# silencht/SG-SLAM

Hardware: AMD Instinct MI355X
Metric: tracked frames/sec (640x480 RGB-D) (higher is better)
Workload: dtype u8/f32(bf16x3 matrix products)/f64

## Files before the change

### include/sgx.h

```cpp
#ifndef SGX_H
#define SGX_H
#include <stdint.h>
#include <stddef.h>
#ifdef __cplusplus
extern "C" {
#endif

typedef enum sgx_status {
    SGX_OK = 0,
    SGX_ERR_INVALID = -1,
    SGX_ERR_UNSUPPORTED = -2,
    SGX_ERR_NOMEM = -3,
    SGX_ERR_DEVICE = -4,
    SGX_ERR_OVERFLOW = -5
} sgx_status;

const char *sgx_version(void);
const char *sgx_status_string(int status);

typedef struct sgx_keypoint {
    float x, y;
    float size;
    float angle;
    float response;
    int32_t octave;
    int32_t class_id;
} sgx_keypoint;

typedef struct sgx_orb_config {
    int32_t nfeatures;
    float scale_factor;
    int32_t nlevels;
    int32_t ini_th_fast;
    int32_t min_th_fast;
    int32_t width, height;
    int32_t max_batch;
} sgx_orb_config;

typedef struct sgx_orb sgx_orb;

int sgx_orb_create(const sgx_orb_config *cfg, sgx_orb **out);
void sgx_orb_destroy(sgx_orb *h);
int sgx_orb_keypoint_capacity(const sgx_orb *h);
int sgx_orb_get_tables(const sgx_orb *h, float *scale, float *inv_scale, float *sigma2, float *inv_sigma2,
                       int32_t *features_per_level);
int sgx_orb_extract_batch_dev(sgx_orb *h, const uint8_t *d_gray, int pitch, int batch,
                              sgx_keypoint *d_kps, uint8_t *d_desc, int32_t *d_count, int cap, void *stream);
int sgx_orb_extract(sgx_orb *h, const uint8_t *gray, int stride, sgx_keypoint *kps, uint8_t *desc, int cap, int *n);
int sgx_orb_last_status(sgx_orb *h, void *stream);

typedef struct sgx_camera {
    float fx, fy, cx, cy, bf;
    float min_x, max_x, min_y, max_y;
} sgx_camera;

int sgx_match_project_frame_batch_dev(
    int batch, int cap,
    const sgx_keypoint *d_ckeys, const uint8_t *d_cdesc, const float *d_curight, const int32_t *d_cn, const float *d_cTcw,
    const sgx_keypoint *d_lkeys, const int32_t *d_ln, const uint8_t *d_l_has_mp, const uint8_t *d_l_outlier, const float *d_l_xw,
    const int32_t *d_l_obs, const uint8_t *d_l_mpdesc, const float *d_lTcw,
    const sgx_camera *cam, const float *scale_factors, int nlevels, float th, int b_mono, int check_orientation,
    int32_t *d_cur_match, int32_t *d_nmatches, void *stream);
int sgx_match_project_frame(
    int nc, const sgx_keypoint *ckeys, const uint8_t *cdesc, const float *curight, const float *cTcw,
    int nl, const sgx_keypoint *lkeys, const uint8_t *l_has_mp, const uint8_t *l_outlier, const float *l_xw,
    const int32_t *l_obs, const uint8_t *l_mpdesc, const float *lTcw,
    const sgx_camera *cam, const float *scale_factors, int nlevels, float th, int b_mono, int check_orientation,
    int32_t *cur_match, int32_t *nmatches);

int sgx_match_project_local_batch_dev(
    int batch, int cap, const sgx_keypoint *d_ckeys, const uint8_t *d_cdesc, const float *d_curight, const int32_t *d_cn, const float *d_cTcw, const int32_t *d_cur_mp_obs,
    int mcap, const int32_t *d_mn, const float *d_m_xw, const float *d_m_normal, const float *d_m_min_dist, const float *d_m_max_dist, const uint8_t *d_m_desc,
    const int32_t *d_m_obs, const uint8_t *d_m_skip,
    const sgx_camera *cam, const float *scale_factors, int nlevels, float log_scale_factor, float th, float nnratio, float viewing_cos_limit,
    int32_t *d_cur_match, int32_t *d_nmatches, uint8_t *d_in_view, void *stream);

int sgx_match_project_local(
    int nc, const sgx_keypoint *ckeys, const uint8_t *cdesc, const float *curight, const float *cTcw, const int32_t *cur_mp_obs,
    int nm, const float *m_xw, const float *m_normal, const float *m_min_dist, const float *m_max_dist, const uint8_t *m_desc, const int32_t *m_obs, const uint8_t *m_skip,
    const sgx_camera *cam, const float *scale_factors, int nlevels, float log_scale_factor, float th, float nnratio, float viewing_cos_limit,
    int32_t *cur_match, int32_t *nmatches, uint8_t *in_view);

int sgx_hamming_matrix(const uint8_t *desc_a, int na, const uint8_t *desc_b, int nb, uint16_t *out);
int sgx_hamming_matrix_dev(const uint8_t *d_desc_a, int na, const uint8_t *d_desc_b, int nb, uint16_t *d_out, void *stream);
int sgx_match_search_for_triangulation(
    int n1, const sgx_keypoint *keys1_un, const uint8_t *desc1, const float *uright1, const uint8_t *has_mp1, const int32_t *feat_node1, const float *cam_center1,
    int n2, const sgx_keypoint *keys2_un, const uint8_t *desc2, const float *uright2, const uint8_t *has_mp2, const int32_t *feat_node2, const float *Tcw2,
    const float *F12, const sgx_camera *cam2, const float *scale_factors2, const float *level_sigma2_2, int nlevels, int only_stereo, int check_orientation,
    int32_t *pairs, int32_t *npairs);
int sgx_match_search_by_bow(
    int nk, const sgx_keypoint *keys_kf_un, const uint8_t *desc_kf, const uint8_t *kf_good_mp, const int32_t *feat_node_kf,
    int nf, const sgx_keypoint *keys_f_un, const uint8_t *desc_f, const int32_t *feat_node_f, float nnratio, int check_orientation,
    int32_t *match_f, int32_t *nmatches);
int sgx_match_search_by_bow_kf(
    int n1, const sgx_keypoint *keys1_un, const uint8_t *desc1, const uint8_t *good1, const int32_t *feat_node1,
    int n2, const sgx_keypoint *keys2_un, const uint8_t *desc2, const uint8_t *good2, const int32_t *feat_node2, float nnratio, int check_orientation,
    int32_t *match12, int32_t *nmatches);
int sgx_match_fuse_search(
    int nk, const sgx_keypoint *keys_un, const uint8_t *desc, const float *uright, const float *Tcw,
    int nm, const float *m_xw, const float *m_normal, const float *m_min_dist, const float *m_max_dist, const uint8_t *m_desc, const uint8_t *m_skip,
    const sgx_camera *cam, const float *scale_factors, const float *inv_level_sigma2, int nlevels, float log_scale_factor, float th,
    int32_t *best_idx, int32_t *best_dist, int32_t *nfused);

int sgx_match_project_keyframe(
    int nc, const sgx_keypoint *ckeys_un, const uint8_t *cdesc, const uint8_t *c_has_mp, const float *cTcw,
    int nk, const sgx_keypoint *kf_keys_un, const uint8_t *kf_ok, const float *m_xw, const float *m_min_dist, const float *m_max_dist, const uint8_t *m_desc,
    const sgx_camera *cam, const float *scale_factors, int nlevels, float log_scale_factor, float th, int orb_dist, int check_orientation,
    int32_t *cur_match, int32_t *nmatches);

int sgx_match_fuse_search_sim3(
    int nk, const sgx_keypoint *keys_un, const uint8_t *desc, const float *Scw,
    int nm, const float *m_xw, const float *m_normal, const float *m_min_dist, const float *m_max_dist, const uint8_t *m_desc, const uint8_t *m_skip,
    const sgx_camera *cam, const float *scale_factors, int nlevels, float log_scale_factor, float th,
    int32_t *best_idx, int32_t *best_dist, int32_t *nfused);
int sgx_match_project_sim3(
    int nk, const sgx_keypoint *keys_un, const uint8_t *desc, const uint8_t *matched_in, const float *Scw,
    int nm, const float *m_xw, const float *m_normal, const float *m_min_dist, const float *m_max_dist, const uint8_t *m_desc, const uint8_t *m_skip,
    const sgx_camera *cam, const float *scale_factors, int nlevels, float log_scale_factor, int th,
    int32_t *matched_out, int32_t *nmatches);
int sgx_match_search_by_sim3(
    int n1, const sgx_keypoint *keys1_un, const uint8_t *desc1, const float *Tcw1, const uint8_t *mp_ok1, const float *m_xw1, const float *m_min_dist1, const float *m_max_dist1, const uint8_t *m_desc1,
    int n2, const sgx_keypoint *keys2_un, const uint8_t *desc2, const float *Tcw2, const uint8_t *mp_ok2, const float *m_xw2, const float *m_min_dist2, const float *m_max_dist2, const uint8_t *m_desc2,
    const sgx_camera *cam, const float *scale_factors, int nlevels, float log_scale_factor, float s12, const float *R12, const float *t12, float th,
    int32_t *match12, int32_t *nfound);

int sgx_match_search_for_initialization(
    int n1, const sgx_keypoint *keys1_un, const uint8_t *desc1, int n2, const sgx_keypoint *keys2_un, const uint8_t *desc2,
    float *prev_matched, int window_size, float nnratio, int check_orientation, const sgx_camera *cam, int32_t *matches12, int32_t *nmatches);

int sgx_triangulate_new_map_points(
// ... 84 lines not shown
int sgx_voc_transform(sgx_voc *v, int n, const uint8_t *desc, int levelsup, int32_t *bow_ids, double *bow_weights, int32_t *nbow, int32_t *feat_node, int32_t *feat_word);
int sgx_voc_transform_batch_dev(sgx_voc *v, const uint8_t *d_desc, size_t desc_pitch, const int32_t *d_n, int batch, int cap, int levelsup,
                                int32_t *d_word_id, double *d_weight, int32_t *d_feat_node, void *stream);
int sgx_voc_score(const sgx_voc *v, int n1, const int32_t *ids1, const double *w1, int n2, const int32_t *ids2, const double *w2, double *score);

int sgx_frame_gray_from_color_batch_dev(int batch, int width, int height, const uint8_t *d_src, int src_pitch, int channels, int blue_first,
                                        uint8_t *d_gray, int gray_pitch, void *stream);
int sgx_frame_stereo_from_rgbd_batch_dev(int batch, int cap, const sgx_keypoint *d_keys, const int32_t *d_n,
                                         const uint16_t *d_depth, int width, int height, float depth_map_factor,
                                         float bf, float *d_uright, float *d_zdepth, void *stream);
int sgx_undistort_points(int n, const float *pts, const float *K4, const float *dist, int ndist, float *out);
int sgx_frame_undistort_stereo_rgbd_batch_dev(int batch, int cap, const sgx_keypoint *d_keys, const int32_t *d_n, const float *dist, int ndist,
                                              const sgx_camera *cam, const uint16_t *d_depth, int width, int height, float depth_map_factor,
                                              sgx_keypoint *d_keys_un, float *d_uright, float *d_zdepth, void *stream);
int sgx_frame_image_bounds(int width, int height, const float *K4, const float *dist, int ndist, sgx_camera *cam);

int sgx_frame_unproject_batch_dev(int batch, int cap, const sgx_keypoint *d_keys, const int32_t *d_n, const float *d_zdepth,
                                  const float *d_Tcw, const sgx_camera *cam, float *d_xw, uint8_t *d_has, void *stream);

int sgx_frame_motion_model_batch_dev(int batch, const float *d_Tcw_cur, const float *d_Tcw_prev, const uint8_t *d_valid,
                                     float *d_Tcw_pred, void *stream);

int sgx_frame_make_map_points_batch_dev(int batch, int cap, int half, const sgx_keypoint *d_keys, const int32_t *d_n, const float *d_xw, const uint8_t *d_has,
                                        const uint8_t *d_desc, const float *d_Tcw, const float *scale_factors, int nlevels,
                                        float *d_m_xw, float *d_m_normal, float *d_m_min_dist, float *d_m_max_dist, uint8_t *d_m_desc, uint8_t *d_m_skip, void *stream);
int sgx_frame_merge_matches_batch_dev(int batch, int cap, const int32_t *d_n, const int32_t *d_match_last, const uint8_t *d_outlier_last, const int32_t *d_match_local,
                                      const float *d_xw_last, const float *d_m_xw, int32_t *d_merged, int32_t *d_cur_mp_obs, float *d_xw_all, void *stream);

int sgx_pose_optimization_batch_dev(int batch, int cap, const sgx_keypoint *d_keys_un, const float *d_uright, const int32_t *d_n,
                                    const int32_t *d_mp_index, const uint8_t *d_has_mp, const float *d_mp_xw, int xw_pitch,
                                    const float *inv_level_sigma2, int nlevels, const sgx_camera *cam,
                                    float *d_Tcw, uint8_t *d_outlier, int32_t *d_n_inliers, void *stream);
int sgx_pose_optimization(int n, const sgx_keypoint *keys_un, const float *uright, const uint8_t *has_mp, const float *mp_xw,
                          const float *inv_level_sigma2, int nlevels, const sgx_camera *cam,
                          float *Tcw, uint8_t *outlier, int32_t *n_inliers);

typedef struct sgx_ba_problem {
    int32_t n_poses, n_points, n_edges;
    float *poses;
    const uint8_t *pose_fixed;
    float *points;
    const int32_t *edge_pose;
    const int32_t *edge_point;
    const float *edge_obs;
    const float *edge_info;
} sgx_ba_problem;
typedef struct sgx_ba_stats { int32_t iterations_first, iterations_second, free_poses, reserved; double chi2_first, chi2_second; } sgx_ba_stats;
int sgx_local_bundle_adjustment(const sgx_ba_problem *problem, const sgx_camera *cam, const volatile int32_t *stop_flag,
                                uint8_t *edge_erase, sgx_ba_stats *stats);
int sgx_bundle_adjustment(const sgx_ba_problem *problem, const sgx_camera *cam, int n_iterations, const volatile int32_t *stop_flag, int robust, sgx_ba_stats *stats);

int sgx_optimize_sim3(int n, const float *p1c, const float *p2c, const float *obs1, const float *obs2, const float *info1, const float *info2,
                      const float *K1, const float *K2, double *S12, float th2, int fix_scale, uint8_t *inlier, int32_t *iterations, int32_t *n_inliers);

int sgx_optimize_essential_graph(int nv, const double *S_in, const uint8_t *fixed, int ne, const int32_t *e_i, const int32_t *e_j, const double *e_meas,
                                 int fix_scale, int iterations, double *S_out, double *stats);
int sgx_correct_map_points(int n, const float *xw, const int32_t *ref, int nv, const double *Srw, const double *corrected_Swr, float *xw_out);

#define SGX_DET_MAX 100
typedef struct sgx_detection { float label, score, xmin, ymin, xmax, ymax; } sgx_detection;
typedef struct sgx_object2d { int32_t id; float prob, x, y, w, h; } sgx_object2d;
typedef struct sgx_det_result {
    int32_t n_raw; sgx_detection raw[SGX_DET_MAX];
    int32_t n_objects; sgx_object2d objects[SGX_DET_MAX];
    int32_t have_dynamic_for_mapping, have_dynamic_for_rm_feature;
    int32_t n_map_boxes; sgx_object2d map_boxes[SGX_DET_MAX];
    int32_t n_rm_boxes; sgx_object2d rm_boxes[SGX_DET_MAX];
} sgx_det_result;
typedef struct sgx_det sgx_det;
int sgx_det_create(const char *param_text, const void *bin, size_t bin_bytes, int width, int height, int max_batch,
                   float detection_confidence_threshold, float dynamic_detection_confidence_threshold, sgx_det **out);
void sgx_det_destroy(sgx_det *h);
int sgx_det_info(const sgx_det *h, int32_t *num_priors, int32_t *num_class, int32_t *num_kernels, double *gmac);
int sgx_det_detect(sgx_det *h, const uint8_t *images, int pitch, int batch, sgx_det_result *results);
int sgx_det_detect_batch_dev(sgx_det *h, const uint8_t *d_img, int pitch, int batch, sgx_det_result *d_results,
                             float *d_boxes, int32_t *d_nboxes, int max_boxes, int32_t *d_have_dynamic, void *stream);
int sgx_det_forward_batch_dev(sgx_det *h, const uint8_t *d_img, int pitch, int batch, const float **d_loc, const float **d_conf, void *stream);
int sgx_det_gemm_mode(const sgx_det *h);
int sgx_det_plan_step(const sgx_det *h, int i, char *buf, int cap);
int sgx_dynamic_mask_batch_dev(int batch, int cap, const sgx_keypoint *d_keys, const int32_t *d_n, const float *d_prev_xy, const double *d_F,
                               const float *d_boxes, const int32_t *d_nboxes, int max_boxes, uint8_t *d_keep, void *stream);
int sgx_frame_compact_keys_batch_dev(int batch, int cap, const sgx_keypoint *d_keys, const uint8_t *d_desc, const int32_t *d_n, const uint8_t *d_keep,
                                     const int32_t *d_have_dynamic, int nfeatures, sgx_keypoint *d_keys_out, uint8_t *d_desc_out, int32_t *d_n_out, void *stream);


typedef struct sgx_flow_config {
    int32_t width, height, max_batch;
    int32_t win_size;
    int32_t max_level;
    int32_t max_count;
    double epsilon;
} sgx_flow_config;
typedef struct sgx_flow sgx_flow;
int sgx_flow_create(const sgx_flow_config *cfg, sgx_flow **out);
void sgx_flow_destroy(sgx_flow *h);
int sgx_flow_reset(sgx_flow *h);
int sgx_flow_levels(const sgx_flow *h);
int sgx_flow_lk_batch_dev(sgx_flow *h, const uint8_t *d_gray, int pitch, int batch, const sgx_keypoint *d_keys, const int32_t *d_n, int cap,
                          float *d_prev_xy, uint8_t *d_status, int32_t *have_prev, void *stream);
int sgx_flow_lk(sgx_flow *h, const uint8_t *gray_from, const uint8_t *gray_to, int stride, const float *pts, int n, float *next_pts, uint8_t *status);
int sgx_fundamental_ransac_batch_dev(int batch, int cap, const sgx_keypoint *d_keys, const int32_t *d_n, const float *d_prev_xy,
                                     const int32_t *d_pre_have_dynamic, const float *d_pre_boxes, const int32_t *d_pre_nboxes, int max_boxes,
                                     double threshold, double confidence, double *d_F, int32_t *d_ok, int32_t *d_stats, void *stream);
int sgx_find_fundamental_mat(const float *pts1, const float *pts2, int n, double threshold, double confidence, double *F, int32_t *ok, int32_t *stats);

typedef struct sgx_tracker_config {
    int32_t streams, width, height;
    int32_t nfeatures; float scale_factor; int32_t nlevels, ini_th_fast, min_th_fast;
    sgx_camera cam; float depth_map_factor;
    float th_projection;
    int32_t local_map;
    int32_t dynamic_mask;
    int32_t max_boxes;
    int32_t pipelined;
} sgx_tracker_config;
typedef struct sgx_tracker sgx_tracker;
int sgx_tracker_create(const sgx_tracker_config *cfg, sgx_det *detector , sgx_tracker **out);
void sgx_tracker_destroy(sgx_tracker *t);
int sgx_tracker_keypoint_capacity(const sgx_tracker *t);
int sgx_tracker_record_bytes(const sgx_tracker *t);
int sgx_tracker_set_initial_pose(sgx_tracker *t, const float *Tcw );
int sgx_tracker_set_distortion(sgx_tracker *t, const float *dist, int ndist, sgx_camera *out_cam);
int sgx_tracker_step_dev(sgx_tracker *t, const uint8_t *d_gray, int gray_pitch, const uint16_t *d_depth, const uint8_t *d_bgr, int bgr_pitch, void *caller_stream);
int sgx_tracker_host_buffers(sgx_tracker *t, int slot, uint8_t **bgr, int *bgr_pitch, uint16_t **depth);
int sgx_tracker_step_host(sgx_tracker *t, int slot, int rgb_order);
int sgx_tracker_wait_inputs(sgx_tracker *t, int steps_back);
int sgx_tracker_sync(sgx_tracker *t);
int sgx_tracker_read(sgx_tracker *t, float *Tcw, int32_t *nkeys, int32_t *nmatches, int32_t *ninliers, int32_t *nmatches_local, int32_t *ninliers2, int32_t *nkeys_raw,
                     int32_t *f_ok, int32_t *f_stats);
int sgx_tracker_snapshot_pose_dev(sgx_tracker *t, float *d_out );
int sgx_tracker_snapshot_boxes_dev(sgx_tracker *t, int stream_index, float *d_boxes , int32_t *d_nboxes);
int sgx_tracker_pack_records_dev(sgx_tracker *t, uint8_t *d_records, void *stream);
typedef struct sgx_dist sgx_dist;
int sgx_dist_unique_id(void *id128 );
int sgx_dist_create(const void *id128, int world, int rank, sgx_dist **out);
void sgx_dist_destroy(sgx_dist *d);
int sgx_dist_world(const sgx_dist *d, int32_t *world, int32_t *rank);
int sgx_dist_gather_records(sgx_dist *d, const void *d_send, size_t bytes_per_rank, void *d_recv, int root, void *stream);
int sgx_tracker_frame_dev(sgx_tracker *t, const int32_t **d_n, const sgx_keypoint **d_keys, const uint8_t **d_desc, const float **d_Tcw, const float **d_xw, const uint8_t **d_has);
int sgx_tracker_frame_keys_un_dev(sgx_tracker *t, const sgx_keypoint **d_keys_un);
sgx_orb *sgx_tracker_extractor(sgx_tracker *t);

int sgx_profile_enable(int on);
int sgx_profile_num_classes(void);
const char *sgx_profile_class_name(int k);
int sgx_profile_read(float *ms, int32_t *launches, int reset);

#ifdef __cplusplus
}
#endif
#endif
```

### include/sgx_debug.h

```cpp
#ifndef SGX_DEBUG_H
#define SGX_DEBUG_H
#include "sgx.h"
#ifdef __cplusplus
extern "C" {
#endif

int sgx_orb_debug_level_geometry(const sgx_orb *h, int level, int32_t *w, int32_t *hgt, int32_t *stride);
int sgx_orb_debug_set_unfused_pyramid(int on);
int sgx_orb_debug_read_level(sgx_orb *h, int frame, int level, uint8_t *dst );
int sgx_orb_debug_read_candidates(sgx_orb *h, int frame, int level, int32_t *x, int32_t *y, int32_t *score, int cap, int *n);
int sgx_debug_flow_affine_batch_dev(int batch, int cap, const sgx_keypoint *d_keys, const int32_t *d_n, const float *d_A, const float *d_shift, const float *d_boxes,
                                    int max_boxes, float *d_prev_xy, void *stream);
int sgx_pose_opt_debug_set_threads(int threads_per_frame);
int sgx_ba_debug_last_plan(int32_t plan[4]);
int sgx_ba_debug_set_init(int mode);
int sgx_ba_debug_set_jobs(int host);
int sgx_ba_debug_set_solver(int mode);
int sgx_det_debug_read_blob(sgx_det *h, const char *blob_name, int image, float *dst, int cap, int *n);
int sgx_flow_debug_read_level(sgx_flow *h, int slot, int frame, int level, uint8_t *img);
int sgx_flow_debug_read_slot(sgx_flow *h, int slot, int frame, int level, uint8_t *img, int32_t *pitch);
int sgx_flow_debug_level_size(const sgx_flow *h, int level, int32_t *w, int32_t *hgt);
int sgx_pnp_debug_betas(int which, const double *L, const double *rho, double *betas);
int sgx_obj3d_debug_read(sgx_obj3d *h, int job, uint8_t *kept, int32_t *labels, int cap, int *n);
int sgx_debug_corun_bf16(int blocks, int iters, int launches, void *stream);
int sgx_det_debug_detection_output(sgx_det *h, const float *loc, const float *conf, int batch, sgx_det_result *results);
int sgx_det_debug_continued(sgx_det *h, int *count);
int sgx_det_debug_set_fusion(int on);
int sgx_det_debug_set_irb(int on);
int sgx_det_debug_set_block_fusion(int on);
int sgx_det_debug_set_gemm(int mode);
int sgx_det_debug_set_legacy_kernels(int on);
int sgx_det_debug_time_ops(sgx_det *h, const uint8_t *d_img, int pitch, int batch, int reps, float *ms, int cap, int *nops);
int sgx_det_debug_run_step(sgx_det *h, const uint8_t *d_img, int pitch, int batch, int step, int reps, void *stream);
int sgx_orb_debug_run_octree(sgx_orb *h, int level, const uint32_t *packed, int n, uint32_t *out_sel, int cap, int *nsel);

#ifdef __cplusplus
}
#endif
#endif
```

### sg_slam_amd/capi.py

```python
import ctypes as C
import numpy as np

KP_DTYPE = np.dtype([('x', 'f4'), ('y', 'f4'), ('size', 'f4'), ('angle', 'f4'), ('response', 'f4'),
                     ('octave', 'i4'), ('class_id', 'i4')])


class SgxError(RuntimeError):
    pass


class Camera(C.Structure):
    _fields_ = [('fx', C.c_float), ('fy', C.c_float), ('cx', C.c_float), ('cy', C.c_float), ('bf', C.c_float),
                ('min_x', C.c_float), ('max_x', C.c_float), ('min_y', C.c_float), ('max_y', C.c_float)]


class BaProblem(C.Structure):
    _fields_ = [('n_poses', C.c_int32), ('n_points', C.c_int32), ('n_edges', C.c_int32), ('poses', C.c_void_p), ('pose_fixed', C.c_void_p),
                ('points', C.c_void_p), ('edge_pose', C.c_void_p), ('edge_point', C.c_void_p), ('edge_obs', C.c_void_p), ('edge_info', C.c_void_p)]


class BaStats(C.Structure):
    _fields_ = [('iterations_first', C.c_int32), ('iterations_second', C.c_int32), ('free_poses', C.c_int32), ('reserved', C.c_int32),
                ('chi2_first', C.c_double), ('chi2_second', C.c_double)]

# ... 2 lines not shown


class Detection(C.Structure):
    _fields_ = [(k, C.c_float) for k in ('label', 'score', 'xmin', 'ymin', 'xmax', 'ymax')]


class Object2D(C.Structure):
    _fields_ = [('id', C.c_int32)] + [(k, C.c_float) for k in ('prob', 'x', 'y', 'w', 'h')]


class DetResult(C.Structure):
    _fields_ = [('n_raw', C.c_int32), ('raw', Detection * SGX_DET_MAX), ('n_objects', C.c_int32), ('objects', Object2D * SGX_DET_MAX),
                ('have_dynamic_for_mapping', C.c_int32), ('have_dynamic_for_rm_feature', C.c_int32),
                ('n_map_boxes', C.c_int32), ('map_boxes', Object2D * SGX_DET_MAX), ('n_rm_boxes', C.c_int32), ('rm_boxes', Object2D * SGX_DET_MAX)]


class FlowConfig(C.Structure):
    _fields_ = [('width', C.c_int32), ('height', C.c_int32), ('max_batch', C.c_int32), ('win_size', C.c_int32), ('max_level', C.c_int32),
                ('max_count', C.c_int32), ('epsilon', C.c_double)]


class TrackerConfig(C.Structure):
    _fields_ = [('streams', C.c_int32), ('width', C.c_int32), ('height', C.c_int32), ('nfeatures', C.c_int32), ('scale_factor', C.c_float), ('nlevels', C.c_int32),
                ('ini_th_fast', C.c_int32), ('min_th_fast', C.c_int32), ('cam', Camera), ('depth_map_factor', C.c_float), ('th_projection', C.c_float),
                ('local_map', C.c_int32), ('dynamic_mask', C.c_int32), ('max_boxes', C.c_int32), ('pipelined', C.c_int32)]


class Obj3dParams(C.Structure):
    _fields_ = [('sor_stddev_mul', C.c_double), ('sor_mean_k', C.c_int32), ('cluster_min_size', C.c_int32), ('cluster_max_size', C.c_int32),
                ('voxel_leaf_size', C.c_float), ('cluster_tolerance', C.c_float), ('similar_compare_ratio', C.c_float),
                ('camera_valid_depth_min', C.c_float), ('camera_valid_depth_max', C.c_float)]


class Obj3dJob(C.Structure):
    _fields_ = [('image', C.c_int32), ('class_id', C.c_int32)] + [(k, C.c_float) for k in ('prob', 'x', 'y', 'w', 'h')]


OBJ3D_RESULT_DTYPE = np.dtype([('found', 'i4'), ('class_id', 'i4'), ('prob', 'f4'), ('centroid', 'f4', 3), ('size', 'f4', 3), ('crop_points', 'i4'), ('kept_points', 'i4'),
                               ('components', 'i4'), ('clusters', 'i4'), ('best_cluster_size', 'i4'), ('larger_window_points', 'i4'), ('best_similar1', 'f4'),
                               ('best_similar2', 'f4'), ('best_roi', 'f4', 4)])


class SemanticObjectRecord(C.Structure):
    _fields_ = [('class_id', C.c_int32), ('object_id', C.c_int32), ('prob', C.c_float), ('centroid', C.c_float * 3), ('size', C.c_float * 3)]


class InitReport(C.Structure):
    _fields_ = [('SH', C.c_float), ('SF', C.c_float), ('RH', C.c_float), ('model', C.c_int32), ('n_matches', C.c_int32), ('n_inliers_h', C.c_int32),
                ('n_inliers_f', C.c_int32), ('n_hyp', C.c_int32), ('best_hyp', C.c_int32), ('n_good', C.c_int32 * 8), ('cos_parallax', C.c_float * 8),
                ('parallax', C.c_float * 8), ('H21', C.c_float * 9), ('F21', C.c_float * 9)]


class OrbConfig(C.Structure):
    _fields_ = [('nfeatures', C.c_int32), ('scale_factor', C.c_float), ('nlevels', C.c_int32),
                ('ini_th_fast', C.c_int32), ('min_th_fast', C.c_int32), ('width', C.c_int32),
                ('height', C.c_int32), ('max_batch', C.c_int32)]


SYMBOLS = [
    'sgx_version', 'sgx_status_string', 'sgx_orb_create', 'sgx_orb_destroy', 'sgx_orb_keypoint_capacity', 'sgx_orb_get_tables',
    'sgx_orb_extract_batch_dev', 'sgx_orb_extract', 'sgx_orb_last_status', 'sgx_profile_enable', 'sgx_profile_num_classes', 'sgx_profile_class_name',
    'sgx_profile_read', 'sgx_match_project_frame_batch_dev', 'sgx_match_project_frame', 'sgx_match_project_local_batch_dev',
    'sgx_match_project_local', 'sgx_frame_stereo_from_rgbd_batch_dev', 'sgx_frame_unproject_batch_dev', 'sgx_frame_make_map_points_batch_dev',
    'sgx_frame_merge_matches_batch_dev', 'sgx_pose_optimization_batch_dev', 'sgx_pose_optimization', 'sgx_frame_motion_model_batch_dev',
    'sgx_local_bundle_adjustment', 'sgx_bundle_adjustment', 'sgx_det_create', 'sgx_det_destroy', 'sgx_det_info', 'sgx_det_detect',
    'sgx_det_detect_batch_dev', 'sgx_det_forward_batch_dev', 'sgx_frame_compact_keys_batch_dev', 'sgx_frame_gray_from_color_batch_dev',
    'sgx_det_gemm_mode', 'sgx_det_plan_step', 'sgx_dynamic_mask_batch_dev', 'sgx_tracker_create', 'sgx_tracker_destroy',
    'sgx_tracker_keypoint_capacity', 'sgx_tracker_record_bytes', 'sgx_tracker_set_initial_pose', 'sgx_tracker_step_dev', 'sgx_tracker_host_buffers',
    'sgx_tracker_step_host', 'sgx_tracker_wait_inputs', 'sgx_tracker_sync', 'sgx_tracker_read', 'sgx_tracker_snapshot_pose_dev',
    'sgx_tracker_snapshot_boxes_dev', 'sgx_tracker_pack_records_dev', 'sgx_tracker_frame_dev', 'sgx_tracker_extractor', 'sgx_flow_create',
    'sgx_dist_unique_id', 'sgx_dist_create', 'sgx_dist_destroy', 'sgx_dist_world', 'sgx_dist_gather_records',
    'sgx_flow_destroy', 'sgx_flow_reset', 'sgx_flow_levels', 'sgx_flow_lk_batch_dev', 'sgx_flow_lk', 'sgx_fundamental_ransac_batch_dev',
    'sgx_find_fundamental_mat', 'sgx_hamming_matrix', 'sgx_hamming_matrix_dev', 'sgx_match_search_for_triangulation', 'sgx_match_search_by_bow',
    'sgx_match_search_by_bow_kf', 'sgx_match_fuse_search', 'sgx_match_project_keyframe', 'sgx_match_fuse_search_sim3',
    'sgx_triangulate_new_map_points', 'sgx_mappoint_update_normal_and_depth', 'sgx_mappoint_distinctive_descriptors', 'sgx_sim3_solver_create',
    'sgx_sim3_solver_set_ransac_parameters', 'sgx_sim3_solver_iterate', 'sgx_sim3_solver_get_estimate', 'sgx_sim3_solver_destroy',
    'sgx_match_search_for_initialization', 'sgx_voc_load', 'sgx_voc_create', 'sgx_voc_info', 'sgx_voc_destroy', 'sgx_voc_transform',
    'sgx_voc_transform_batch_dev', 'sgx_voc_score', 'sgx_match_project_sim3', 'sgx_match_search_by_sim3', 'sgx_optimize_sim3',
    'sgx_optimize_essential_graph', 'sgx_correct_map_points', 'sgx_undistort_points', 'sgx_frame_undistort_stereo_rgbd_batch_dev', 'sgx_frame_image_bounds',
    'sgx_tracker_set_distortion', 'sgx_tracker_frame_keys_un_dev', 'sgx_pnp_solver_create', 'sgx_pnp_solver_set_ransac_parameters', 'sgx_pnp_solver_iterate',
    'sgx_pnp_solver_get_estimate', 'sgx_pnp_solver_destroy', 'sgx_pnp_batch_create', 'sgx_pnp_batch_set_dev', 'sgx_pnp_batch_iterate_dev', 'sgx_pnp_batch_destroy',
    'sgx_obj3d_create', 'sgx_obj3d_destroy', 'sgx_obj3d_detect_batch_dev', 'sgx_obj3d_detect', 'sgx_objdb_create', 'sgx_objdb_destroy', 'sgx_objdb_add', 'sgx_objdb_size',
    'sgx_objdb_get', 'sgx_initializer_create', 'sgx_initializer_initialize', 'sgx_initializer_destroy', 'sgx_init_batch_create', 'sgx_init_batch_run_dev',
    'sgx_init_batch_destroy',
]
TAP_SYMBOLS = [
    'sgx_orb_debug_level_geometry', 'sgx_orb_debug_set_unfused_pyramid', 'sgx_orb_debug_read_level', 'sgx_orb_debug_read_candidates',
    'sgx_orb_debug_run_octree', 'sgx_pose_opt_debug_set_threads', 'sgx_ba_debug_set_solver', 'sgx_ba_debug_set_jobs', 'sgx_ba_debug_set_init', 'sgx_ba_debug_last_plan', 'sgx_det_debug_read_blob',
    'sgx_det_debug_detection_output', 'sgx_det_debug_continued', 'sgx_debug_flow_affine_batch_dev', 'sgx_det_debug_set_fusion', 'sgx_det_debug_set_legacy_kernels',
    'sgx_det_debug_set_block_fusion', 'sgx_det_debug_set_irb', 'sgx_det_debug_set_gemm', 'sgx_det_debug_time_ops', 'sgx_det_debug_run_step', 'sgx_flow_debug_read_level',
    'sgx_flow_debug_level_size', 'sgx_flow_debug_read_slot', 'sgx_debug_corun_bf16', 'sgx_pnp_debug_betas', 'sgx_obj3d_debug_read',
]


def _vp(x):
    if x is None:
        return None
    if isinstance(x, int):
        return C.c_void_p(x)
    if hasattr(x, 'data_ptr'):
        return C.c_void_p(x.data_ptr())
    return x.ctypes.data_as(C.c_void_p)


class SgxLib:
    def __init__(self, path):
        self.path = path
        self.dll = C.CDLL(path)
        d = self.dll
        d.sgx_version.restype = C.c_char_p
        d.sgx_status_string.restype = C.c_char_p
        d.sgx_status_string.argtypes = [C.c_int]
        d.sgx_orb_create.argtypes = [C.POINTER(OrbConfig), C.POINTER(C.c_void_p)]
        d.sgx_orb_destroy.argtypes = [C.c_void_p]
        d.sgx_orb_destroy.restype = None
        d.sgx_orb_keypoint_capacity.argtypes = [C.c_void_p]
        d.sgx_orb_get_tables.argtypes = [C.c_void_p] + [C.c_void_p] * 5
        d.sgx_orb_extract_batch_dev.argtypes = [C.c_void_p, C.c_void_p, C.c_int, C.c_int, C.c_void_p, C.c_void_p,
                                                C.c_void_p, C.c_int, C.c_void_p]
        d.sgx_orb_extract.argtypes = [C.c_void_p, C.c_void_p, C.c_int, C.c_void_p, C.c_void_p, C.c_int, C.POINTER(C.c_int)]
        d.sgx_orb_last_status.argtypes = [C.c_void_p, C.c_void_p]

        d.sgx_profile_enable.argtypes = [C.c_int]
        d.sgx_profile_class_name.restype = C.c_char_p
        d.sgx_profile_class_name.argtypes = [C.c_int]
        d.sgx_profile_read.argtypes = [C.c_void_p, C.c_void_p, C.c_int]

        vp = C.c_void_p
        d.sgx_match_project_frame_batch_dev.argtypes = [C.c_int, C.c_int] + [vp] * 13 + [C.POINTER(Camera), vp, C.c_int, C.c_float, C.c_int, C.c_int, vp, vp, vp]
        d.sgx_match_project_frame.argtypes = [C.c_int] + [vp] * 4 + [C.c_int] + [vp] * 7 + [C.POINTER(Camera), vp, C.c_int, C.c_float, C.c_int, C.c_int, vp, vp]
        d.sgx_frame_stereo_from_rgbd_batch_dev.argtypes = [C.c_int, C.c_int, vp, vp, vp, C.c_int, C.c_int, C.c_float, C.c_float, vp, vp, vp]
        d.sgx_frame_unproject_batch_dev.argtypes = [C.c_int, C.c_int, vp, vp, vp, vp, C.POINTER(Camera), vp, vp, vp]
        d.sgx_pose_optimization_batch_dev.argtypes = [C.c_int, C.c_int, vp, vp, vp, vp, vp, vp, C.c_int, vp, C.c_int, C.POINTER(Camera), vp, vp, vp, vp]
        d.sgx_pose_optimization.argtypes = [C.c_int, vp, vp, vp, vp, vp, C.c_int, C.POINTER(Camera), vp, vp, vp]
        d.sgx_frame_motion_model_batch_dev.argtypes = [C.c_int, vp, vp, vp, vp, vp]
        d.sgx_local_bundle_adjustment.argtypes = [C.POINTER(BaProblem), C.POINTER(Camera), vp, vp, C.POINTER(BaStats)]
        d.sgx_bundle_adjustment.argtypes = [C.POINTER(BaProblem), C.POINTER(Camera), C.c_int, vp, C.c_int, C.POINTER(BaStats)]
        d.sgx_det_create.argtypes = [C.c_char_p, vp, C.c_size_t, C.c_int, C.c_int, C.c_int, C.c_float, C.c_float, C.POINTER(vp)]
        d.sgx_det_destroy.argtypes = [vp]; d.sgx_det_destroy.restype = None
        d.sgx_det_info.argtypes = [vp, C.POINTER(C.c_int32), C.POINTER(C.c_int32), C.POINTER(C.c_int32), C.POINTER(C.c_double)]
        d.sgx_det_detect.argtypes = [vp, vp, C.c_int, C.c_int, C.POINTER(DetResult)]
        d.sgx_det_detect_batch_dev.argtypes = [vp, vp, C.c_int, C.c_int, vp, vp, vp, C.c_int, vp, vp]
        d.sgx_det_forward_batch_dev.argtypes = [vp, vp, C.c_int, C.c_int, C.POINTER(vp), C.POINTER(vp), vp]
        d.sgx_det_gemm_mode.argtypes = [vp]
        d.sgx_tracker_create.argtypes = [C.POINTER(TrackerConfig), vp, C.POINTER(vp)]
        d.sgx_tracker_destroy.argtypes = [vp]; d.sgx_tracker_destroy.restype = None
        d.sgx_tracker_keypoint_capacity.argtypes = [vp]
        d.sgx_tracker_record_bytes.argtypes = [vp]
        d.sgx_tracker_set_initial_pose.argtypes = [vp, vp]
        d.sgx_tracker_step_dev.argtypes = [vp, vp, C.c_int, vp, vp, C.c_int, vp]
        d.sgx_tracker_host_buffers.argtypes = [vp, C.c_int, C.POINTER(vp), C.POINTER(C.c_int), C.POINTER(vp)]
        d.sgx_tracker_step_host.argtypes = [vp, C.c_int, C.c_int]
        d.sgx_tracker_sync.argtypes = [vp]
        d.sgx_tracker_wait_inputs.argtypes = [vp, C.c_int]
        d.sgx_tracker_read.argtypes = [vp] * 10
        d.sgx_tracker_snapshot_pose_dev.argtypes = [vp, vp]
        d.sgx_tracker_snapshot_boxes_dev.argtypes = [vp, C.c_int, vp, vp]
        d.sgx_tracker_pack_records_dev.argtypes = [vp, vp, vp]
        d.sgx_dist_unique_id.argtypes = [vp]
        d.sgx_dist_create.argtypes = [vp, C.c_int, C.c_int, C.POINTER(vp)]
        d.sgx_dist_destroy.argtypes = [vp]; d.sgx_dist_destroy.restype = None
        d.sgx_dist_world.argtypes = [vp, C.POINTER(C.c_int32), C.POINTER(C.c_int32)]
        d.sgx_dist_gather_records.argtypes = [vp, vp, C.c_size_t, vp, C.c_int, vp]
        d.sgx_tracker_frame_dev.argtypes = [vp] + [C.POINTER(vp)] * 6
        d.sgx_tracker_extractor.argtypes = [vp]; d.sgx_tracker_extractor.restype = vp
        d.sgx_det_plan_step.argtypes = [vp, C.c_int, C.c_char_p, C.c_int]
        d.sgx_dynamic_mask_batch_dev.argtypes = [C.c_int, C.c_int, vp, vp, vp, vp, vp, vp, C.c_int, vp, vp]
        d.sgx_frame_gray_from_color_batch_dev.argtypes = [C.c_int, C.c_int, C.c_int, vp, C.c_int, C.c_int, C.c_int, vp, C.c_int, vp]
        d.sgx_frame_compact_keys_batch_dev.argtypes = [C.c_int, C.c_int, vp, vp, vp, vp, vp, C.c_int, vp, vp, vp, vp]
        d.sgx_match_project_local.argtypes = [C.c_int] + [vp] * 5 + [C.c_int] + [vp] * 7 + [C.POINTER(Camera), vp, C.c_int, C.c_float, C.c_float, C.c_float, C.c_float, vp, vp, vp]
        d.sgx_match_project_local_batch_dev.argtypes = [C.c_int, C.c_int] + [vp] * 6 + [C.c_int] + [vp] * 8 + [C.POINTER(Camera), vp, C.c_int, C.c_float, C.c_float, C.c_float, C.c_float, vp, vp, vp, vp]
        d.sgx_undistort_points.argtypes = [C.c_int, vp, vp, vp, C.c_int, vp]
        d.sgx_frame_undistort_stereo_rgbd_batch_dev.argtypes = [C.c_int, C.c_int, vp, vp, vp, C.c_int, C.POINTER(Camera), vp, C.c_int, C.c_int, C.c_float, vp, vp, vp, vp]
        d.sgx_frame_image_bounds.argtypes = [C.c_int, C.c_int, vp, vp, C.c_int, C.POINTER(Camera)]
        d.sgx_tracker_set_distortion.argtypes = [vp, vp, C.c_int, C.POINTER(Camera)]
        d.sgx_tracker_frame_keys_un_dev.argtypes = [vp, C.POINTER(vp)]
        d.sgx_frame_make_map_points_batch_dev.argtypes = [C.c_int, C.c_int, C.c_int] + [vp] * 7 + [C.c_int] + [vp] * 7
        d.sgx_frame_merge_matches_batch_dev.argtypes = [C.c_int, C.c_int] + [vp] * 10
        d.sgx_flow_create.argtypes = [C.POINTER(FlowConfig), C.POINTER(vp)]
        d.sgx_flow_destroy.argtypes = [vp]; d.sgx_flow_destroy.restype = None
        d.sgx_flow_reset.argtypes = [vp]
        d.sgx_flow_levels.argtypes = [vp]
        d.sgx_flow_lk_batch_dev.argtypes = [vp, vp, C.c_int, C.c_int, vp, vp, C.c_int, vp, vp, C.POINTER(C.c_int32), vp]
        d.sgx_flow_lk.argtypes = [vp, vp, vp, C.c_int, vp, C.c_int, vp, vp]
        d.sgx_fundamental_ransac_batch_dev.argtypes = [C.c_int, C.c_int] + [vp] * 6 + [C.c_int, C.c_double, C.c_double, vp, vp, vp, vp]
        d.sgx_find_fundamental_mat.argtypes = [vp, vp, C.c_int, C.c_double, C.c_double, vp, vp, vp]
        d.sgx_hamming_matrix.argtypes = [vp, C.c_int, vp, C.c_int, vp]
        d.sgx_optimize_essential_graph.argtypes = [C.c_int, vp, vp, C.c_int, vp, vp, vp, C.c_int, C.c_int, vp, vp]
        d.sgx_correct_map_points.argtypes = [C.c_int, vp, vp, C.c_int, vp, vp, vp]
        d.sgx_optimize_sim3.argtypes = [C.c_int] + [vp] * 9 + [C.c_float, C.c_int, vp, vp, vp]
        d.sgx_match_project_keyframe.argtypes = [C.c_int] + [vp] * 4 + [C.c_int] + [vp] * 6 + [C.POINTER(Camera), vp, C.c_int, C.c_float, C.c_float, C.c_int, C.c_int, vp, vp]
        d.sgx_match_search_by_bow.argtypes = [C.c_int] + [vp] * 4 + [C.c_int] + [vp] * 3 + [C.c_float, C.c_int, vp, vp]
        d.sgx_match_fuse_search_sim3.argtypes = [C.c_int, vp, vp, vp, C.c_int] + [vp] * 6 + [vp, vp, C.c_int, C.c_float, C.c_float, vp, vp, vp]
        d.sgx_match_project_sim3.argtypes = [C.c_int, vp, vp, vp, vp, C.c_int] + [vp] * 6 + [vp, vp, C.c_int, C.c_float, C.c_int, vp, vp]
        d.sgx_match_search_by_sim3.argtypes = ([C.c_int] + [vp] * 8) * 2 + [vp, vp, C.c_int, C.c_float, C.c_float, vp, vp, C.c_float, vp, vp]
        d.sgx_match_search_for_initialization.argtypes = [C.c_int, vp, vp, C.c_int, vp, vp, vp, C.c_int, C.c_float, C.c_int, vp, vp, vp]
        d.sgx_sim3_solver_create.argtypes = [C.c_int] + [vp] * 6 + [C.c_int, C.c_uint, vp]
        d.sgx_sim3_solver_set_ransac_parameters.argtypes = [vp, C.c_double, C.c_int, C.c_int]
        d.sgx_sim3_solver_iterate.argtypes = [vp, C.c_int] + [vp] * 7
        d.sgx_sim3_solver_get_estimate.argtypes = [vp] * 5
        d.sgx_sim3_solver_destroy.argtypes = [vp]; d.sgx_sim3_solver_destroy.restype = None
        d.sgx_pnp_solver_create.argtypes = [C.c_int] + [vp] * 4 + [C.c_uint, vp]
        d.sgx_pnp_solver_set_ransac_parameters.argtypes = [vp, C.c_double, C.c_int, C.c_int, C.c_int, C.c_float, C.c_float]
        d.sgx_pnp_solver_iterate.argtypes = [vp, C.c_int] + [vp] * 7
        d.sgx_pnp_solver_get_estimate.argtypes = [vp] * 6
        d.sgx_pnp_solver_destroy.argtypes = [vp]; d.sgx_pnp_solver_destroy.restype = None
        d.sgx_pnp_batch_create.argtypes = [C.c_int, C.c_int, vp]
        d.sgx_pnp_batch_set_dev.argtypes = [vp, C.c_int] + [vp] * 8
        d.sgx_pnp_batch_iterate_dev.argtypes = [vp, C.c_int, vp, C.c_int, vp, vp, vp, vp]
        d.sgx_pnp_batch_destroy.argtypes = [vp]; d.sgx_pnp_batch_destroy.restype = None
        d.sgx_initializer_create.argtypes = [C.c_int, vp, vp, C.c_float, C.c_int, C.c_uint, vp]
        d.sgx_initializer_initialize.argtypes = [vp, C.c_int] + [vp] * 10
        d.sgx_initializer_destroy.argtypes = [vp]; d.sgx_initializer_destroy.restype = None
        d.sgx_init_batch_create.argtypes = [C.c_int] * 4 + [vp]
        d.sgx_init_batch_run_dev.argtypes = [vp, C.c_int] + [vp] * 9 + [C.c_int] + [vp] * 8
        d.sgx_init_batch_destroy.argtypes = [vp]; d.sgx_init_batch_destroy.restype = None
        d.sgx_obj3d_create.argtypes = [C.c_int] * 5 + [C.POINTER(Obj3dParams), C.POINTER(vp)]
        d.sgx_obj3d_destroy.argtypes = [vp]; d.sgx_obj3d_destroy.restype = None
        d.sgx_obj3d_detect_batch_dev.argtypes = [vp, vp, C.c_int, C.c_int, vp, vp, vp, C.c_int, vp, vp]
        d.sgx_obj3d_detect.argtypes = [vp, vp, vp, vp, C.POINTER(Obj3dJob), vp]
        d.sgx_objdb_create.argtypes = [C.POINTER(vp)]
        d.sgx_objdb_destroy.argtypes = [vp]; d.sgx_objdb_destroy.restype = None
        d.sgx_objdb_add.argtypes = [vp, C.POINTER(SemanticObjectRecord), C.POINTER(C.c_int32), C.POINTER(C.c_int32)]
        d.sgx_objdb_size.argtypes = [vp]
        d.sgx_objdb_get.argtypes = [vp, C.c_int, C.POINTER(SemanticObjectRecord)]
        d.sgx_mappoint_update_normal_and_depth.argtypes = [C.c_int] + [vp] * 6 + [C.c_int, vp, vp, vp]
        d.sgx_mappoint_distinctive_descriptors.argtypes = [C.c_int, vp, vp, vp, vp]
        d.sgx_triangulate_new_map_points.argtypes = [C.c_int, vp] + [C.c_int] + [vp] * 5 + [C.c_int] + [vp] * 5 + [vp, vp, vp, C.c_int, vp, vp, vp]
        d.sgx_voc_load.argtypes = [C.c_char_p, vp]
        d.sgx_voc_create.argtypes = [C.c_int] * 5 + [vp] * 5
        d.sgx_voc_info.argtypes = [vp] * 7
        d.sgx_voc_destroy.argtypes = [vp]; d.sgx_voc_destroy.restype = None
        d.sgx_voc_transform.argtypes = [vp, C.c_int, vp, C.c_int, vp, vp, vp, vp, vp]
        d.sgx_voc_transform_batch_dev.argtypes = [vp, vp, C.c_size_t, vp, C.c_int, C.c_int, C.c_int, vp, vp, vp, vp]
        d.sgx_voc_score.argtypes = [vp, C.c_int, vp, vp, C.c_int, vp, vp, vp]
        d.sgx_match_search_by_bow_kf.argtypes = [C.c_int] + [vp] * 4 + [C.c_int] + [vp] * 4 + [C.c_float, C.c_int, vp, vp]
        d.sgx_match_fuse_search.argtypes = [C.c_int] + [vp] * 4 + [C.c_int] + [vp] * 6 + [C.POINTER(Camera), vp, vp, C.c_int, C.c_float, C.c_float, vp, vp, vp]
        d.sgx_hamming_matrix_dev.argtypes = [vp, C.c_int, vp, C.c_int, vp, vp]
        d.sgx_match_search_for_triangulation.argtypes = [C.c_int] + [vp] * 6 + [C.c_int] + [vp] * 6 + [vp, C.POINTER(Camera), vp, vp, C.c_int, C.c_int, C.c_int, vp, vp]

        self.has_taps = hasattr(d, 'sgx_det_debug_read_blob')
        if self.has_taps:
            d.sgx_orb_debug_level_geometry.argtypes = [C.c_void_p, C.c_int] + [C.POINTER(C.c_int32)] * 3
            d.sgx_orb_debug_read_level.argtypes = [C.c_void_p, C.c_int, C.c_int, C.c_void_p]
            d.sgx_orb_debug_read_candidates.argtypes = [C.c_void_p, C.c_int, C.c_int, C.c_void_p, C.c_void_p, C.c_void_p, C.c_int, C.POINTER(C.c_int)]
            d.sgx_orb_debug_run_octree.argtypes = [C.c_void_p, C.c_int, C.c_void_p, C.c_int, C.c_void_p, C.c_int, C.POINTER(C.c_int)]
            d.sgx_orb_debug_set_unfused_pyramid.argtypes = [C.c_int]
            d.sgx_pose_opt_debug_set_threads.argtypes = [C.c_int]
            d.sgx_ba_debug_set_solver.argtypes = [C.c_int]
            d.sgx_ba_debug_set_jobs.argtypes = [C.c_int]
            d.sgx_ba_debug_set_init.argtypes = [C.c_int]
            d.sgx_ba_debug_last_plan.argtypes = [C.c_void_p]
            d.sgx_det_debug_detection_output.argtypes = [vp, vp, vp, C.c_int, C.POINTER(DetResult)]
            d.sgx_det_debug_continued.argtypes = [vp, C.POINTER(C.c_int)]
            d.sgx_det_debug_read_blob.argtypes = [vp, C.c_char_p, C.c_int, vp, C.c_int, C.POINTER(C.c_int)]
            for nm in ('fusion', 'legacy_kernels', 'block_fusion', 'irb', 'gemm'):
                getattr(d, 'sgx_det_debug_set_' + nm).argtypes = [C.c_int]
            d.sgx_det_debug_time_ops.argtypes = [vp, vp, C.c_int, C.c_int, C.c_int, vp, C.c_int, C.POINTER(C.c_int)]
            d.sgx_det_debug_run_step.argtypes = [vp, vp, C.c_int, C.c_int, C.c_int, C.c_int, vp]
            d.sgx_debug_flow_affine_batch_dev.argtypes = [C.c_int, C.c_int, vp, vp, vp, vp, vp, C.c_int, vp, vp]
            d.sgx_flow_debug_read_level.argtypes = [vp, C.c_int, C.c_int, C.c_int, vp]
            d.sgx_debug_corun_bf16.argtypes = [C.c_int, C.c_int, C.c_int, vp]
            d.sgx_pnp_debug_betas.argtypes = [C.c_int, vp, vp, vp]
            d.sgx_obj3d_debug_read.argtypes = [vp, C.c_int, vp, vp, C.c_int, C.POINTER(C.c_int)]
            d.sgx_flow_debug_level_size.argtypes = [vp, C.c_int, C.POINTER(C.c_int32), C.POINTER(C.c_int32)]
            d.sgx_flow_debug_read_slot.argtypes = [vp, C.c_int, C.c_int, C.c_int, vp, C.POINTER(C.c_int32)]

    def tap(self, name):
        if not self.has_taps:
            raise SgxError(f'{name}: {self.path} is the product build and has no test taps; use tests/taps/libsgx_taps.so (make -C sg_slam_amd/csrc taps)')
        return getattr(self.dll, name)

    def version(self):
        return self.dll.sgx_version().decode()

    def check(self, rc, what=''):
        if rc != 0:
            raise SgxError(f'{what}: {self.dll.sgx_status_string(rc).decode()} ({rc})')

    def profile_enable(self, on=True):
        self.check(self.dll.sgx_profile_enable(int(on)))

    def profile_read(self, reset=True):
        n = self.dll.sgx_profile_num_classes()
        ms = np.zeros(n, 'f4'); cnt = np.zeros(n, 'i4')
        self.check(self.dll.sgx_profile_read(_vp(ms), _vp(cnt), int(reset)), 'sgx_profile_read')
        return {self.dll.sgx_profile_class_name(k).decode(): (float(ms[k]), int(cnt[k])) for k in range(n)}
```

### sg_slam_amd/csrc/sgx_det.cpp

```cpp
#include "sgx_block.h"
#include "sgx_det_block.h"
#include "sgx_det_irb.h"
#include "sgx_det_bf16.h"
#include "sgx_det_hrb.h"
#include "sgx_prof.h"
#include "../../include/sgx.h"
#ifdef SGX_DEBUG_TAPS
#include "../../include/sgx_debug.h"
#endif
#include <math.h>
#include <stdio.h>
#include <stdlib.h>
#include <string.h>
#include <algorithm>
#include <map>
#include <memory>
#include <sstream>
#include <string>
#include <vector>


namespace {
struct Layer {
    std::string type, name;
// ... 1206 lines not shown
                                        float *d_boxes, int32_t *d_nboxes, int max_boxes, int32_t *d_have_dynamic, void *stream_)
{
    if (!h || !d_results || ((d_boxes != nullptr) != (d_nboxes != nullptr)) || (d_boxes && max_boxes < 1)) return SGX_ERR_INVALID;
    const float *dl = nullptr, *dc = nullptr;
    int rc = sgx_det_forward_batch_dev(h, d_img, pitch, batch, &dl, &dc, stream_);
    if (rc != SGX_OK) return rc;
    return run_detection_output(h, batch, d_results, d_boxes, d_nboxes, max_boxes, d_have_dynamic, (sgx_stream_t)stream_);
}

static int run_detection_output(sgx_det *h, int batch, sgx_det_result *d_results, float *d_boxes, int32_t *d_nboxes, int max_boxes, int32_t *d_have_dynamic, sgx_stream_t st)
{
    SgxDetOut P; P.n = h->num_priors; P.nc = h->num_class; P.nms_top_k = h->nms_top_k; P.keep_top_k = h->keep_top_k; P.nms_th = h->nms_th; P.conf_th = h->conf_th;
    P.var0 = h->dvar[0]; P.var1 = h->dvar[1]; P.var2 = h->dvar[2]; P.var3 = h->dvar[3];
    if (h->sw.skip_output) return SGX_OK;
    sgx_prof_begin(SGX_K_DET_OUT, st);
    const dim3 grid(h->num_class - 1, batch);
    const size_t lds_full = (size_t)std::max(h->num_priors, 7 * SGX_DO_TOPK) * 4 + 16, lds_first = (size_t)std::max(h->num_priors, 7 * (SGX_DO_FIRST + 1)) * 4 + 16;
    const float *loc = h->blobs[h->loc_blob].d, *conf = h->blobs[h->conf_blob].d;
    const int *no_cont = nullptr; const uint32_t *no_sstar = nullptr; int *no_ncut = nullptr; uint32_t *no_next = nullptr;
    if (h->sw.out_single) {
        SGX_LAUNCH_DYN(k_det_class_nms<0>, grid, dim3(256), lds_full, st, P, loc, conf, h->d_priors, h->d_cls_rows, h->d_cls_count, no_ncut, no_next, no_cont, no_sstar);
    } else {
        SGX_LAUNCH_DYN(k_det_class_nms<SGX_DO_FIRST>, grid, dim3(256), lds_first, st, P, loc, conf, h->d_priors, h->d_cls_rows, h->d_cls_count, h->d_cls_ncut, h->d_cls_next, no_cont, no_sstar);
        SGX_LAUNCH(k_det_cut, dim3(batch), dim3(256), st, P, h->d_cls_rows, h->d_cls_count, h->d_cls_ncut, h->d_cls_next, h->d_sstar, h->d_cls_cont);
        SGX_LAUNCH_DYN(k_det_class_nms<0>, grid, dim3(256), lds_full, st, P, loc, conf, h->d_priors, h->d_cls_rows, h->d_cls_count, no_ncut, no_next, h->d_cls_cont, h->d_sstar);
    }
    h->last_out_batch = h->sw.out_single ? 0 : batch;
    SGX_LAUNCH(k_det_merge, dim3(batch), dim3(256), st, P, h->d_cls_rows, h->d_cls_count, h->det_th, h->dyn_th, h->W, h->H, h->T, d_results, d_boxes, d_nboxes, max_boxes, d_have_dynamic);
    sgx_prof_end(SGX_K_DET_OUT, st);
    SGX_CHECK_HIP(hipGetLastError());
    return SGX_OK;
}

SGX_TAP int sgx_det_debug_detection_output(sgx_det *h, const float *loc, const float *conf, int batch, sgx_det_result *results)
{
    if (!h || !loc || !conf || !results || batch < 1 || batch > h->max_batch) return SGX_ERR_INVALID;
    SGX_CHECK_HIP(hipMemcpy(h->blobs[h->loc_blob].d, loc, sizeof(float) * 4 * (size_t)h->num_priors * batch, hipMemcpyHostToDevice));
    SGX_CHECK_HIP(hipMemcpy(h->blobs[h->conf_blob].d, conf, sizeof(float) * (size_t)h->num_priors * h->num_class * batch, hipMemcpyHostToDevice));
    int rc = run_detection_output(h, batch, h->d_results, nullptr, nullptr, 0, nullptr, (sgx_stream_t)0);
    if (rc != SGX_OK) return rc;
    SGX_CHECK_HIP(hipMemcpy(results, h->d_results, sizeof(sgx_det_result) * batch, hipMemcpyDeviceToHost));
    return SGX_OK;
}

SGX_TAP int sgx_det_debug_continued(sgx_det *h, int *count)
{
    if (!h || !count) return SGX_ERR_INVALID;
    std::vector<int> cont((size_t)h->last_out_batch * (h->num_class - 1));
    if (!cont.empty()) SGX_CHECK_HIP(hipMemcpy(cont.data(), h->d_cls_cont, cont.size() * sizeof(int), hipMemcpyDeviceToHost));
    *count = 0; for (int v : cont) *count += v;
    return SGX_OK;
}

extern "C" int sgx_det_detect(sgx_det *h, const uint8_t *images, int pitch, int batch, sgx_det_result *results)
{
    if (!h || !images || !results || batch < 1 || batch > h->max_batch || pitch < 3 * h->W) return SGX_ERR_INVALID;
    const int ipitch = (3 * h->W + 3) & ~3;
    for (int b = 0; b < batch; b++)
        for (int y = 0; y < h->H; y++)
            SGX_CHECK_HIP(hipMemcpyAsync(h->d_img + ((size_t)b * h->H + y) * ipitch, images + ((size_t)b * h->H + y) * pitch, (size_t)3 * h->W, hipMemcpyHostToDevice, 0));
    int rc = sgx_det_detect_batch_dev(h, h->d_img, ipitch, batch, h->d_results, nullptr, nullptr, 0, nullptr, nullptr);
    if (rc != SGX_OK) return rc;
    SGX_CHECK_HIP(hipMemcpy(results, h->d_results, sizeof(sgx_det_result) * batch, hipMemcpyDeviceToHost));
    return SGX_OK;
}

extern "C" int sgx_dynamic_mask_batch_dev(int batch, int cap, const sgx_keypoint *d_keys, const int32_t *d_n, const float *d_prev_xy, const double *d_F,
                                          const float *d_boxes, const int32_t *d_nboxes, int max_boxes, uint8_t *d_keep, void *stream)
{
    if (batch < 1 || cap < 1 || !d_keys || !d_n || !d_prev_xy || !d_F || !d_boxes || !d_nboxes || !d_keep || max_boxes < 0) return SGX_ERR_INVALID;
    sgx_prof_begin(SGX_K_MASK, (sgx_stream_t)stream);
    SGX_LAUNCH(k_dynamic_mask, dim3((cap + 255) / 256, batch), dim3(256), (sgx_stream_t)stream, cap, (const uint8_t *)d_keys, d_n, d_prev_xy, d_F, d_boxes, d_nboxes, max_boxes, d_keep);
    sgx_prof_end(SGX_K_MASK, (sgx_stream_t)stream);
    SGX_CHECK_HIP(hipGetLastError());
    return SGX_OK;
}

extern "C" int sgx_frame_compact_keys_batch_dev(int batch, int cap, const sgx_keypoint *d_keys, const uint8_t *d_desc, const int32_t *d_n, const uint8_t *d_keep,
                                                const int32_t *d_have_dynamic, int nfeatures, sgx_keypoint *d_keys_out, uint8_t *d_desc_out, int32_t *d_n_out, void *stream)
{
    if (batch < 1 || cap < 1 || !d_keys || !d_desc || !d_n || !d_keep || !d_keys_out || !d_desc_out || !d_n_out || (const void *)d_keys == (const void *)d_keys_out) return SGX_ERR_INVALID;
    sgx_prof_begin(SGX_K_MASK, (sgx_stream_t)stream);
    SGX_LAUNCH(k_compact_keys, dim3(batch), dim3(256), (sgx_stream_t)stream, cap, (const uint8_t *)d_keys, d_desc, d_n, d_keep, d_have_dynamic, (float)nfeatures * 0.1f,
               (uint8_t *)d_keys_out, d_desc_out, d_n_out);
    sgx_prof_end(SGX_K_MASK, (sgx_stream_t)stream);
    SGX_CHECK_HIP(hipGetLastError());
    return SGX_OK;
}
```

### sg_slam_amd/csrc/sgx_det_kernels.h

```cpp
#pragma once
#include "sgx_rt.h"
#include "../../include/sgx.h"
#ifdef SGX_DEBUG_TAPS
#include "../../include/sgx_debug.h"
#endif

#ifndef SGX_EMU
__device__ int sgx_det_xcd_order = 1;
#else
static int sgx_det_xcd_order = 1;
#endif
SGX_DEV void sgx_xcd_order(int id, int per_frame, int batch, int *frame, int *item)
{
    const int b8 = batch & ~7;
    if (sgx_det_xcd_order && id < b8 * per_frame) {
        const int x = id & 7, i = id >> 3, q = i / per_frame;
        *item = i - q * per_frame; *frame = q * 8 + x;
    } else { const int f = id / per_frame; *frame = f; *item = id - f * per_frame; }
}

#define SGX_ACT_NONE 0
#define SGX_ACT_RELU 1
#define SGX_ACT_CLIP 2

// ... 800 lines not shown
    SGX_THREADS_END
}

SGX_KERNEL(256) k_unary(size_t n, int act, float lo, float hi, const float *a, float *out)
{
    SGX_THREADS_BEGIN(tid)
    for (size_t i = (size_t)blockIdx.x * 256 + tid; i < n; i += (size_t)gridDim.x * 256) out[i] = sgx_act(a[i], act, lo, hi);
    SGX_THREADS_END
}

SGX_KERNEL(256) k_permute_hwc_into(int C, int HW, const float *src, size_t src_pitch, float *dst, size_t dst_pitch, int off)
{
    SGX_THREADS_BEGIN(tid)
    const int idx = (int)blockIdx.x * 256 + tid, b = (int)blockIdx.y;
    if (idx < C * HW) { const int hw = idx / C, c = idx - hw * C; dst[(size_t)b * dst_pitch + off + idx] = src[(size_t)b * src_pitch + (size_t)c * HW + hw]; }
    SGX_THREADS_END
}

SGX_KERNEL(256) k_copy_into(int n, const float *src, size_t src_pitch, float *dst, size_t dst_pitch, int off)
{
    SGX_THREADS_BEGIN(tid)
    const int idx = (int)blockIdx.x * 256 + tid, b = (int)blockIdx.y;
    if (idx < n) dst[(size_t)b * dst_pitch + off + idx] = src[(size_t)b * src_pitch + idx];
    SGX_THREADS_END
}

#define SGX_SOFTMAX_MAXC 32
SGX_KERNEL(256) k_softmax_rows(int rows, int C, const float *in, size_t in_pitch, float *out, size_t out_pitch)
{
    SGX_LDS float buf[256 * SGX_SOFTMAX_MAXC + 1];
    const int r0 = (int)blockIdx.x * 256, b = (int)blockIdx.y;
    const int nr = min(256, rows - r0), tot = nr * C;
    const float *src = in + (size_t)b * in_pitch + (size_t)r0 * C;
    float *dst = out + (size_t)b * out_pitch + (size_t)r0 * C;
    SGX_THREADS_BEGIN(tid)
    for (int t = tid; t < tot; t += 256) buf[t] = src[t];
    SGX_THREADS_END
    SGX_SYNC();
    SGX_THREADS_BEGIN(tid)
    if (tid < nr) {
        float *x = buf + tid * C;
        float m = x[0];
        for (int c = 1; c < C; c++) m = fmaxf(m, x[c]);
        float s = 0.f;
        for (int c = 0; c < C; c++) { const float e = expf(x[c] - m); x[c] = e; s += e; }
        for (int c = 0; c < C; c++) x[c] = x[c] / s;
    }
    SGX_THREADS_END
    SGX_SYNC();
    SGX_THREADS_BEGIN(tid)
    for (int t = tid; t < tot; t += 256) dst[t] = buf[t];
    SGX_THREADS_END
}

SGX_KERNEL(256) k_dynamic_mask(int cap, const uint8_t *keys_raw, const int *n, const float *prev_xy, const double *F, const float *boxes, const int *nboxes,
                               int max_boxes, uint8_t *keep)
{
    SGX_THREADS_BEGIN(tid)
    const int f = (int)blockIdx.y, i = (int)blockIdx.x * 256 + tid;
    if (i < cap) {
        uint8_t k = 0;
        if (i < n[f]) {
            const float *kp = (const float *)(keys_raw + ((size_t)f * cap + i) * 28);
            const float x = kp[0], y = kp[1];
            const double *Fm = F + 9 * (size_t)f;
            const double a = x * Fm[0] + y * Fm[1] + Fm[2], b = x * Fm[3] + y * Fm[4] + Fm[5], c = x * Fm[6] + y * Fm[7] + Fm[8];
            const float px = prev_xy[2 * ((size_t)f * cap + i)], py = prev_xy[2 * ((size_t)f * cap + i) + 1];
            const double dist = fabs(a * px + b * py + c) / sqrt(a * a + b * b);
            const bool noF = Fm[0] == 0. && Fm[1] == 0. && Fm[2] == 0. && Fm[3] == 0. && Fm[4] == 0. && Fm[5] == 0. && Fm[6] == 0. && Fm[7] == 0. && Fm[8] == 0.;
            bool inbox = false;
            const int nb = nboxes[f];
            for (int q = 0; q < nb && q < max_boxes; q++) {
                const float *r = boxes + 4 * ((size_t)f * max_boxes + q);
                if (x > r[0] && x < r[0] + r[2] && y > r[1] && y < r[1] + r[3]) { inbox = true; break; }
            }
            k = (noF || dist < (inbox ? 0.2 : 1.0)) ? 1 : 0;
        }
        keep[(size_t)f * cap + i] = k;
    }
    SGX_THREADS_END
}

SGX_KERNEL(256) k_compact_keys(int cap, const uint8_t *keys, const uint8_t *desc, const int *n, const uint8_t *keep, const int *have_dynamic, float restore_below,
                               uint8_t *keys_out, uint8_t *desc_out, int *n_out)
{
    SGX_LDS int scan[256];
    SGX_LDS int s_total;
    const int f = (int)blockIdx.x, N = min(n[f], cap), CH = (N + 255) / 256;
    SGX_THREADS_BEGIN(tid)
    int c = 0;
    for (int i = tid * CH; i < min(N, (tid + 1) * CH); i++) c += keep[(size_t)f * cap + i] ? 1 : 0;
    scan[tid] = c;
    SGX_THREADS_END
    SGX_SYNC();
    SGX_THREADS_BEGIN(tid)
    sgx_block_exclusive_scan_i32(scan, 256, &s_total, tid);
    SGX_THREADS_END
    SGX_SYNC();
    const bool restore = (have_dynamic && have_dynamic[f]) && (float)s_total < restore_below;
    SGX_THREADS_BEGIN(tid)
    int pos = restore ? tid * CH : scan[tid];
    for (int i = tid * CH; i < min(N, (tid + 1) * CH); i++) {
        if (!restore && !keep[(size_t)f * cap + i]) continue;
        const uint32_t *ks = (const uint32_t *)(keys + ((size_t)f * cap + i) * 28), *ds = (const uint32_t *)(desc + ((size_t)f * cap + i) * 32);
        uint32_t *kd = (uint32_t *)(keys_out + ((size_t)f * cap + pos) * 28), *dd = (uint32_t *)(desc_out + ((size_t)f * cap + pos) * 32);
#pragma unroll
        for (int w = 0; w < 7; w++) kd[w] = ks[w];
#pragma unroll
        for (int w = 0; w < 8; w++) dd[w] = ds[w];
        pos++;
    }
    if (tid == 0) n_out[f] = restore ? N : s_total;
    SGX_THREADS_END
}

#define SGX_DO_SORT 4096
#define SGX_DO_TOPK 320
#define SGX_DO_WORDS (SGX_DO_TOPK / 64)
#define SGX_DO_MERGE 8192
#define SGX_DO_FIRST 64
struct SgxDetOut { int n, nc, nms_top_k, keep_top_k; float nms_th, conf_th, var0, var1, var2, var3; };

#define SGX_BITONIC_DESC(keys, size, NT)                                                                             \
    for (int k_ = 2; k_ <= (size); k_ <<= 1)                                                                         \
        for (int j_ = k_ >> 1; j_ > 0; j_ >>= 1) {                                                                   \
            SGX_THREADS_BEGIN(tid)                                                                                   \
            for (int t_ = tid; t_ < (size) / 2; t_ += (NT)) {                                                        \
                const int lo_ = ((t_ & ~(j_ - 1)) << 1) | (t_ & (j_ - 1)), hi_ = lo_ | j_;                           \
                const unsigned long long a_ = keys[lo_], b_ = keys[hi_];                                             \
                const bool desc_ = (lo_ & k_) == 0;                                                                  \
                if (desc_ ? a_ < b_ : a_ > b_) { keys[lo_] = b_; keys[hi_] = a_; }                                   \
            }                                                                                                        \
            SGX_THREADS_END                                                                                          \
            SGX_SYNC();                                                                                              \
        }

#define SGX_TOPK_SELECT(keys, size, K, hist, cum, sel, s_tot)                                                        \
    SGX_THREADS_BEGIN(tid) if (tid == 0) { sel[0] = 0; sel[1] = (K); sel[2] = 0; sel[3] = 0; } SGX_THREADS_END       \
    SGX_SYNC();                                                                                                      \
    for (int sh_ = 24; sh_ >= 0; sh_ -= 8) {                                                                         \
        SGX_THREADS_BEGIN(tid) hist[tid] = 0; SGX_THREADS_END                                                        \
        SGX_SYNC();                                                                                                  \
        SGX_THREADS_BEGIN(tid)                                                                                       \
        const uint32_t pre_ = (uint32_t)sel[0];                                                                      \
        for (int i_ = tid; i_ < (size); i_ += 256) {                                                                 \
            const unsigned long long k_ = keys[i_]; const uint32_t h_ = (uint32_t)(k_ >> 32);                        \
            if (k_ != 0 && (sh_ == 24 || ((h_ ^ pre_) >> ((sh_ + 8) & 31)) == 0)) sgx_atomic_add(&hist[255 - (int)((h_ >> sh_) & 255u)], 1); \
        }                                                                                                            \
        SGX_THREADS_END                                                                                              \
        SGX_SYNC();                                                                                                  \
        SGX_THREADS_BEGIN(tid) cum[tid] = hist[tid]; SGX_THREADS_END                                                 \
        SGX_SYNC();                                                                                                  \
        SGX_THREADS_BEGIN(tid) sgx_block_exclusive_scan_i32(cum, 256, &s_tot, tid); SGX_THREADS_END                  \
        SGX_SYNC();                                                                                                  \
        SGX_THREADS_BEGIN(tid) { const int need_ = sel[1]; if (cum[tid] < need_ && need_ <= cum[tid] + hist[tid]) sel[2] = tid; } SGX_THREADS_END \
        SGX_SYNC();                                                                                                  \
        SGX_THREADS_BEGIN(tid) if (tid == 0) { const int b_ = sel[2]; sel[1] -= cum[b_]; sel[3] = hist[b_]; sel[0] = (int)((uint32_t)sel[0] | ((uint32_t)(255 - b_) << sh_)); } SGX_THREADS_END \
        SGX_SYNC();                                                                                                  \
    }

#define SGX_RANK_SORT_DESC(src, n, dst)                                                                              \
    SGX_THREADS_BEGIN(tid)                                                                                           \
    for (int r_ = tid; r_ < (n); r_ += 256) {                                                                        \
        const unsigned long long k_ = src[r_]; int rank_ = 0;                                                        \
        _Pragma("unroll 8")                                                                                          \
        for (int q_ = 0; q_ < (n); q_++) rank_ += src[q_] > k_ ? 1 : 0;                                              \
        dst[rank_] = k_;                                                                                             \
    }                                                                                                                \
    SGX_THREADS_END                                                                                                  \
    SGX_SYNC();

#ifdef SGX_EMU
SGX_DEV void sgx_topk_resolve(int *hist, int *sel, int sh, int tid)
{
    if (tid != 0) return;
    int run = 0; const int need = sel[1];
    for (int rb = 0; rb < 256; rb++) {
        const int hcur = hist[rb];
        if (run < need && need <= run + hcur) { sel[1] = need - run; sel[3] = hcur; sel[0] = (int)((uint32_t)sel[0] | ((uint32_t)(255 - rb) << sh)); }
        run += hcur;
    }
    for (int rb = 0; rb < 256; rb++) hist[rb] = 0;
}
#else
SGX_DEV void sgx_topk_resolve(int *hist, int *sel, int sh, int tid)
{
    if (tid >= 64) return;
    const int need = sel[1]; const uint32_t pre = (uint32_t)sel[0];
    int hv[4]; int sum = 0;
#pragma unroll
    for (int j = 0; j < 4; j++) { hv[j] = hist[4 * tid + j]; sum += hv[j]; }
    int inc = sum;
// ... 332 lines not shown
```

### sg_slam_amd/csrc/sgx_orb.cpp

```cpp
#include "sgx_orb_kernels.h"
#include "sgx_prof.h"
#include "../../include/sgx.h"
#ifdef SGX_DEBUG_TAPS
#include "../../include/sgx_debug.h"
#endif
#include "../../include/sgx_orb_pattern.h"
#include <math.h>
#include <stdio.h>
#include <stdlib.h>
#include <string.h>
#include <vector>

#ifdef SGX_EMU
thread_local sgx_dim3 blockIdx, blockDim, gridDim;
#endif


struct sgx_orb {
    sgx_orb_config cfg;
    SgxOrbGeom g;
    float scale[SGX_MAX_LEVELS], inv_scale[SGX_MAX_LEVELS], sigma2[SGX_MAX_LEVELS], inv_sigma2[SGX_MAX_LEVELS];
    int umax_h[16];
    SgxCell *d_cells = nullptr;
    SgxXTab *d_xt[SGX_MAX_LEVELS] = {};
    SgxYTab *d_yt[SGX_MAX_LEVELS] = {};
    SgxXGroup *d_xg_all = nullptr; SgxYTab *d_yt_all = nullptr; SgxPyrRect *d_pyr_rects = nullptr; SgxPyrTabs pyr_tabs; int pyr_tiles = 0, pyr_lds = 0;
    int *d_umax = nullptr;
    signed char *d_pattern = nullptr;
    uint8_t *d_pyr = nullptr;
    uint8_t *d_blur = nullptr; SgxBlurTile *d_blur_tiles = nullptr;
    uint32_t *d_cand = nullptr;
    int *d_cand_count = nullptr;
    uint16_t *d_node_scratch = nullptr;
    uint32_t *d_sel = nullptr;
    int *d_sel_count = nullptr;
    uint32_t *d_status = nullptr;
    uint8_t *d_gray1 = nullptr; uint8_t *d_kps1 = nullptr; uint8_t *d_desc1 = nullptr; int *d_count1 = nullptr;
    int last_batch = 0;
    int oct_maxlim = 0;
};

static thread_local int g_orb_unfused_pyramid = 0;
SGX_TAP int sgx_orb_debug_set_unfused_pyramid(int on) { g_orb_unfused_pyramid = on ? 1 : 0; return SGX_OK; }

static inline int cvround_f(float v) { return (int)lrintf(v); }
static inline int cvround_d(double v) { return (int)lrint(v); }

static void build_tables(sgx_orb *h)
{
    const sgx_orb_config &c = h->cfg;
    const double sf = (double)c.scale_factor;
    const int nl = c.nlevels;
    h->scale[0] = 1.0f; h->sigma2[0] = 1.0f;
    for (int i = 1; i < nl; i++) { h->scale[i] = (float)((double)h->scale[i - 1] * sf); h->sigma2[i] = h->scale[i] * h->scale[i]; }
    for (int i = 0; i < nl; i++) { h->inv_scale[i] = 1.0f / h->scale[i]; h->inv_sigma2[i] = 1.0f / h->sigma2[i]; }
    const float factor = (float)(1.0f / sf);
    float want = c.nfeatures * (1 - factor) / (1 - (float)pow((double)factor, (double)nl));
    int sum = 0;
    for (int l = 0; l < nl - 1; l++) { h->g.lv[l].quota = cvround_f(want); sum += h->g.lv[l].quota; want *= factor; }
    h->g.lv[nl - 1].quota = c.nfeatures - sum > 0 ? c.nfeatures - sum : 0;
    int umax[17] = {0};
    const int HP = 15;
    const int vmax = (int)floor(HP * sqrtf(2.f) / 2 + 1), vmin = (int)ceil(HP * sqrtf(2.f) / 2);
    for (int v = 0; v <= vmax; ++v) umax[v] = cvround_d(sqrt((double)HP * HP - v * v));
    for (int v = HP, v0 = 0; v >= vmin; --v) { while (umax[v0] == umax[v0 + 1]) ++v0; umax[v] = v0; ++v0; }
    for (int i = 0; i < 16; i++) h->umax_h[i] = umax[i];
}

static void build_resize_tables(int sw, int sh, int dw, int dh, std::vector<SgxXTab> &xt, std::vector<SgxYTab> &yt)
{
    const double scale_x = 1. / ((double)dw / sw), scale_y = 1. / ((double)dh / sh);
    xt.resize(dw); yt.resize(dh);
    for (int dx = 0; dx < dw; dx++) {
        float fx = (float)((dx + 0.5) * scale_x - 0.5);
        int sx = (int)floorf(fx);
        fx -= sx;
        if (sx < 0) { fx = 0; sx = 0; }
        if (sx >= sw - 1) { fx = 0; sx = sw - 1; }
        xt[dx].sx = (short)sx; xt[dx].sx1 = (short)(sx + 1 < sw ? sx + 1 : sx);
        xt[dx].a0 = (short)cvround_f((1.f - fx) * 2048); xt[dx].a1 = (short)cvround_f(fx * 2048);
    }
    for (int dy = 0; dy < dh; dy++) {
        float fy = (float)((dy + 0.5) * scale_y - 0.5);
        int sy = (int)floorf(fy);
        fy -= sy;
        int r0 = sy, r1 = sy + 1;
        if (r0 < 0) r0 = 0; if (r0 > sh - 1) r0 = sh - 1;
        if (r1 < 0) r1 = 0; if (r1 > sh - 1) r1 = sh - 1;
        yt[dy].sy0 = (short)r0; yt[dy].sy1 = (short)r1;
        yt[dy].b0 = (short)cvround_f((1.f - fy) * 2048); yt[dy].b1 = (short)cvround_f(fy * 2048);
    }
}

extern "C" const char *sgx_version(void) {
#ifdef SGX_EMU
    return "sgx 0.1 (EMULATOR - tests only)";
#else
    return "sgx 0.1 (gfx950)";
#endif
}

extern "C" const char *sgx_status_string(int s)
{
    switch (s) {
    case SGX_OK: return "ok";
    case SGX_ERR_INVALID: return "invalid argument";
    case SGX_ERR_UNSUPPORTED: return "unsupported geometry";
    case SGX_ERR_NOMEM: return "out of memory";
    case SGX_ERR_DEVICE: return "HIP runtime error";
    case SGX_ERR_OVERFLOW: return "device buffer overflow";
    default: return "unknown";
    }
}

extern "C" void sgx_orb_destroy(sgx_orb *h)
{
    if (!h) return;
    (void)hipFree(h->d_cells); (void)hipFree(h->d_umax); (void)hipFree(h->d_pattern); (void)hipFree(h->d_pyr); (void)hipFree(h->d_cand);
    (void)hipFree(h->d_cand_count); (void)hipFree(h->d_node_scratch); (void)hipFree(h->d_sel); (void)hipFree(h->d_sel_count); (void)hipFree(h->d_status);
    (void)hipFree(h->d_gray1); (void)hipFree(h->d_kps1); (void)hipFree(h->d_desc1); (void)hipFree(h->d_count1);
    for (int l = 0; l < SGX_MAX_LEVELS; l++) { (void)hipFree(h->d_xt[l]); (void)hipFree(h->d_yt[l]); }
// ... 142 lines not shown
                    G.a01[i] = (uint32_t)t.a0 | ((uint32_t)t.a1 << 16);
                }
                xall.push_back(G);
            }
        }
        const int T = 32, ntx = (g.lv[nl - 1].w + T - 1) / T, nty = (g.lv[nl - 1].h + T - 1) / T;
        std::vector<SgxPyrRect> rects((size_t)ntx * nty * nl);
        int max_a = 0, max_b = 0, max_y = 0;
        for (int j = 0; j < nty; j++) for (int i = 0; i < ntx; i++) {
            SgxPyrRect *R = &rects[((size_t)j * ntx + i) * nl];
            int nx0 = 0, nx1 = 0, ny0 = 0, ny1 = 0;
            for (int l = nl - 1; l >= 0; l--) {
                const int Wl = g.lv[l].w, Hl = g.lv[l].h;
                int ax0 = Wl, ax1 = 0, ay0 = Hl, ay1 = 0;
                if (l >= 1) {
                    ax0 = i == 0 ? 0 : (int)(((long)i * Wl / ntx) & ~3L); ax1 = i == ntx - 1 ? Wl : (int)(((long)(i + 1) * Wl / ntx) & ~3L);
                    ay0 = (int)((long)j * Hl / nty); ay1 = j == nty - 1 ? Hl : (int)((long)(j + 1) * Hl / nty);
                }
                SgxPyrRect &r = R[l];
                r.ox0 = (short)ax0; r.ox1 = (short)ax1; r.oy0 = (short)ay0; r.oy1 = (short)ay1;
                if (l < nl - 1) {
                    for (int x = nx0; x < std::min(nx1, g.lv[l + 1].w); x++) { ax0 = std::min(ax0, (int)xts[l + 1][x].sx); ax1 = std::max(ax1, (int)xts[l + 1][x].sx1 + 1); }
                    for (int y = ny0; y < ny1; y++) { ay0 = std::min(ay0, (int)yts[l + 1][y].sy0); ay1 = std::max(ay1, (int)yts[l + 1][y].sy1 + 1); }
                }
                ax0 &= ~3; ax1 = (ax1 + 3) & ~3;
                r.nx0 = (short)ax0; r.ny0 = (short)ay0; r.nw = (short)(ax1 - ax0); r.nh = (short)(ay1 - ay0);
                const int q = r.nw / 4; r.qmagic = q <= 1 ? 0u : (unsigned)((0x100000000ull + (unsigned)q - 1) / (unsigned)q); r.pad0 = r.pad1 = 0;
                const int bytes = (int)r.nw * r.nh;
                if (l & 1) max_b = std::max(max_b, bytes); else max_a = std::max(max_a, bytes);
                nx0 = ax0; nx1 = ax1; ny0 = ay0; ny1 = ay1;
            }
            int yo = 0;
            for (int l = 1; l < nl; l++) { R[l].yo = yo; yo += R[l].nh; }
            R[0].yo = 0;
            max_y = std::max(max_y, yo);
        }
        h->pyr_tabs.lds_a = (max_a + SGX_PYR_SPAN + 15) & ~15; h->pyr_tabs.lds_b = (max_b + SGX_PYR_SPAN + 15) & ~15;
        h->pyr_lds = h->pyr_tabs.lds_a + h->pyr_tabs.lds_b + max_y * (int)sizeof(SgxYTab);
        h->pyr_tiles = ntx * nty;
        if (h->pyr_lds > 64 * 1024 || !span_ok) h->pyr_tiles = 0;
        SGX_ALLOC(h->d_xg_all, xall.size() * sizeof(SgxXGroup)); SGX_ALLOC(h->d_yt_all, yall.size() * sizeof(SgxYTab)); SGX_ALLOC(h->d_pyr_rects, rects.size() * sizeof(SgxPyrRect));
        SGX_CHECK_HIP(hipMemcpy(h->d_xg_all, xall.data(), xall.size() * sizeof(SgxXGroup), hipMemcpyHostToDevice));
        SGX_CHECK_HIP(hipMemcpy(h->d_yt_all, yall.data(), yall.size() * sizeof(SgxYTab), hipMemcpyHostToDevice));
        SGX_CHECK_HIP(hipMemcpy(h->d_pyr_rects, rects.data(), rects.size() * sizeof(SgxPyrRect), hipMemcpyHostToDevice));
    }
#undef SGX_ALLOC
    *out = h;
    return SGX_OK;
}

extern "C" int sgx_orb_keypoint_capacity(const sgx_orb *h) { return h ? h->g.kp_cap : SGX_ERR_INVALID; }

extern "C" int sgx_orb_get_tables(const sgx_orb *h, float *scale, float *inv_scale, float *sigma2, float *inv_sigma2, int32_t *per_level)
{
    if (!h) return SGX_ERR_INVALID;
    for (int l = 0; l < h->g.nlevels; l++) {
        if (scale) scale[l] = h->scale[l];
        if (inv_scale) inv_scale[l] = h->inv_scale[l];
        if (sigma2) sigma2[l] = h->sigma2[l];
        if (inv_sigma2) inv_sigma2[l] = h->inv_sigma2[l];
        if (per_level) per_level[l] = h->g.lv[l].quota;
    }
    return SGX_OK;
}

static void launch_octree(sgx_orb *h, int batch, sgx_stream_t stream)
{
    const SgxOrbGeom &g = h->g; const int nl = g.nlevels;
    static const int oct_threads = sgx_getenv("SGX_TUNE_OCT_THREADS") ? atoi(sgx_getenv("SGX_TUNE_OCT_THREADS")) : SGX_OCT_THREADS;
    static const bool frame_fast = sgx_getenv("SGX_TUNE_OCT_FRAME_FAST") != nullptr;
    const dim3 ogrid = frame_fast ? dim3(batch, nl) : dim3(nl, batch);
    if (h->oct_maxlim <= 256) {
        auto ka = k_octree<true, 256, 2048>; auto kb = k_octree<true, 256, SGX_CAND_LDS>; auto kc = k_octree<false, 256, 1>;
        SGX_LAUNCH(ka, ogrid, dim3(oct_threads), stream, g, h->d_cand, h->d_cand_count, h->d_node_scratch, h->d_sel, h->d_sel_count, h->d_status, -1);
        SGX_LAUNCH(kb, ogrid, dim3(oct_threads), stream, g, h->d_cand, h->d_cand_count, h->d_node_scratch, h->d_sel, h->d_sel_count, h->d_status, 2048);
        SGX_LAUNCH(kc, ogrid, dim3(oct_threads), stream, g, h->d_cand, h->d_cand_count, h->d_node_scratch, h->d_sel, h->d_sel_count, h->d_status, SGX_CAND_LDS);
    } else {
        auto kb = k_octree<true, SGX_OCT_MAXN, SGX_CAND_LDS>; auto kc = k_octree<false, SGX_OCT_MAXN, 1>;
        SGX_LAUNCH(kb, ogrid, dim3(oct_threads), stream, g, h->d_cand, h->d_cand_count, h->d_node_scratch, h->d_sel, h->d_sel_count, h->d_status, -1);
        SGX_LAUNCH(kc, ogrid, dim3(oct_threads), stream, g, h->d_cand, h->d_cand_count, h->d_node_scratch, h->d_sel, h->d_sel_count, h->d_status, SGX_CAND_LDS);
    }
}

extern "C" int sgx_orb_extract_batch_dev(sgx_orb *h, const uint8_t *d_gray, int pitch, int batch,
                                         sgx_keypoint *d_kps, uint8_t *d_desc, int32_t *d_count, int cap, void *stream_)
{
    if (!h || !d_gray || !d_kps || !d_desc || !d_count) return SGX_ERR_INVALID;
    if (batch < 1 || batch > h->cfg.max_batch || pitch < h->g.W || (pitch & 3) || ((uintptr_t)d_gray & 3) || cap < h->g.kp_cap) return SGX_ERR_INVALID;
    sgx_stream_t stream = (sgx_stream_t)stream_;
    const SgxOrbGeom &g = h->g;
    const int nl = g.nlevels;
    h->last_batch = batch;
    SGX_CHECK_HIP(hipMemsetAsync(h->d_cand_count, 0, (size_t)batch * nl * 4, stream));
    sgx_prof_begin(SGX_K_RESIZE, stream);
    static const int pyr_threads = sgx_getenv("SGX_TUNE_PYR_THREADS") ? atoi(sgx_getenv("SGX_TUNE_PYR_THREADS")) : 512;
    if (h->pyr_tiles > 0 && !g_orb_unfused_pyramid)
        SGX_LAUNCH_DYN(k_pyramid, dim3(h->pyr_tiles, batch), dim3(pyr_threads), h->pyr_lds, stream, g, h->pyr_tabs, d_gray, pitch, h->d_pyr, h->d_xg_all, h->d_yt_all, h->d_pyr_rects);
    else
        for (int l = 1; l < nl; l++) {
            dim3 grid((g.lv[l].w + 255) / 256, (g.lv[l].h + 3) / 4, batch);
            SGX_LAUNCH(k_resize, grid, dim3(256), stream, g, l, d_gray, pitch, h->d_pyr, h->d_xt[l], h->d_yt[l]);
        }
    sgx_prof_end(SGX_K_RESIZE, stream);
    sgx_prof_begin(SGX_K_FAST, stream);
    static const int fast_threads = sgx_getenv("SGX_TUNE_FAST_THREADS") ? atoi(sgx_getenv("SGX_TUNE_FAST_THREADS")) : 128;
    static const int e_extra = sgx_getenv("SGX_TUNE_E_EXTRA_LDS") ? atoi(sgx_getenv("SGX_TUNE_E_EXTRA_LDS")) : 0;
    SGX_LAUNCH_DYN(k_fast_cells, dim3(g.ncells * batch), dim3(fast_threads), g.fast_lds_bytes + e_extra, stream, g, h->d_cells, d_gray, pitch, h->d_pyr, batch,
               h->d_cand, h->d_cand_count, h->d_status);
    sgx_prof_end(SGX_K_FAST, stream);
    sgx_prof_begin(SGX_K_OCTREE, stream);
    launch_octree(h, batch, stream);
    sgx_prof_end(SGX_K_OCTREE, stream);
    sgx_prof_begin(SGX_K_ORIENT_DESC, stream);
    unsigned long long umax_packed = 0;
    for (int i = 0; i < 16; i++) umax_packed |= (unsigned long long)(h->umax_h[i] & 15) << (4 * i);
#ifdef SGX_DEBUG_TAPS
    static const bool patch_blur = sgx_getenv("SGX_TUNE_ORB_PATCH_BLUR") != nullptr;
    if (patch_blur) {
        SGX_LAUNCH_DYN(k_orient_desc, dim3(g.kp_cap * batch), dim3(64), e_extra / 2, stream, g, d_gray, pitch, h->d_pyr, h->d_sel, h->d_sel_count,
                       umax_packed, h->d_pattern, (uint8_t *)d_kps, d_desc, d_count, cap, batch, h->d_status);
    } else
#endif
    {
        static const int blur_threads = sgx_getenv("SGX_TUNE_BLUR_THREADS") ? atoi(sgx_getenv("SGX_TUNE_BLUR_THREADS")) : 256;
        {
            const int blur_grid = sgx_getenv("SGX_TUNE_ORB_BLUR_GRID") ? atoi(sgx_getenv("SGX_TUNE_ORB_BLUR_GRID")) : 4096;
            const int parts = std::min(g.nblur_tiles, std::max(1, blur_grid / batch));
            SGX_LAUNCH(k_blur_levels, dim3(parts * batch), dim3(std::min(512, std::max(256, blur_threads))), stream, g, h->d_blur_tiles, d_gray, pitch, h->d_pyr, h->d_blur, batch);
        }
#ifdef SGX_DEBUG_TAPS
        static const bool one_per_wave = sgx_getenv("SGX_TUNE_ORB_DESC_ONE_PER_WAVE") != nullptr;
        if (one_per_wave)
            SGX_LAUNCH(k_orient_desc2, dim3(g.kp_cap * batch), dim3(64), stream, g, d_gray, pitch, h->d_pyr, h->d_blur, h->d_sel, h->d_sel_count,
                       umax_packed, h->d_pattern, (uint8_t *)d_kps, d_desc, d_count, cap, batch, h->d_status);
        else
#endif
            SGX_LAUNCH(k_orient_desc4, dim3(((g.kp_cap + 3) / 4) * batch), dim3(64), stream, g, d_gray, pitch, h->d_pyr, h->d_blur, h->d_sel, h->d_sel_count,
                       umax_packed, h->d_pattern, (uint8_t *)d_kps, d_desc, d_count, cap, batch, h->d_status);
    }
    sgx_prof_end(SGX_K_ORIENT_DESC, stream);
    SGX_CHECK_HIP(hipGetLastError());
    return SGX_OK;
}

extern "C" int sgx_orb_last_status(sgx_orb *h, void *stream_)
{
    if (!h) return SGX_ERR_INVALID;
    uint32_t st = 0;
    SGX_CHECK_HIP(hipMemcpyAsync(&st, h->d_status, 4, hipMemcpyDeviceToHost, (sgx_stream_t)stream_));
    SGX_CHECK_HIP(hipStreamSynchronize((sgx_stream_t)stream_));
    if (st) { SGX_CHECK_HIP(hipMemsetAsync(h->d_status, 0, 4, (sgx_stream_t)stream_)); return SGX_ERR_OVERFLOW; }
    return SGX_OK;
}

extern "C" int sgx_orb_extract(sgx_orb *h, const uint8_t *gray, int stride, sgx_keypoint *kps, uint8_t *desc, int cap, int *n)
{
    if (!h || !gray || !kps || !desc || !n || stride < h->g.W || cap < 0) return SGX_ERR_INVALID;
    const int W = h->g.W, H = h->g.H, kc = h->g.kp_cap, P = (W + 3) & ~3;
    if (stride == P) SGX_CHECK_HIP(hipMemcpyAsync(h->d_gray1, gray, (size_t)P * (H - 1) + W, hipMemcpyHostToDevice, 0));
    else for (int y = 0; y < H; y++)
        SGX_CHECK_HIP(hipMemcpyAsync(h->d_gray1 + (size_t)y * P, gray + (size_t)y * stride, W, hipMemcpyHostToDevice, 0));
    int rc = sgx_orb_extract_batch_dev(h, h->d_gray1, P, 1, (sgx_keypoint *)h->d_kps1, h->d_desc1, h->d_count1, kc, 0);
    if (rc != SGX_OK) return rc;
    int cnt = 0;
    SGX_CHECK_HIP(hipMemcpyAsync(&cnt, h->d_count1, 4, hipMemcpyDeviceToHost, 0));
    SGX_CHECK_HIP(hipStreamSynchronize(0));
    rc = sgx_orb_last_status(h, 0);
    if (rc != SGX_OK) return rc;
    if (cnt > cap) return SGX_ERR_OVERFLOW;
    SGX_CHECK_HIP(hipMemcpyAsync(kps, h->d_kps1, (size_t)cnt * 28, hipMemcpyDeviceToHost, 0));
    SGX_CHECK_HIP(hipMemcpyAsync(desc, h->d_desc1, (size_t)cnt * 32, hipMemcpyDeviceToHost, 0));
    SGX_CHECK_HIP(hipStreamSynchronize(0));
    *n = cnt;
    return SGX_OK;
}

SGX_TAP int sgx_orb_debug_level_geometry(const sgx_orb *h, int level, int32_t *w, int32_t *hgt, int32_t *stride)
{
    if (!h || level < 0 || level >= h->g.nlevels) return SGX_ERR_INVALID;
    if (w) *w = h->g.lv[level].w; if (hgt) *hgt = h->g.lv[level].h; if (stride) *stride = h->g.lv[level].stride;
    return SGX_OK;
}

SGX_TAP int sgx_orb_debug_read_level(sgx_orb *h, int frame, int level, uint8_t *dst)
{
    if (!h || !dst || level < 1 || level >= h->g.nlevels || frame < 0 || frame >= h->cfg.max_batch) return SGX_ERR_INVALID;
    const SgxLevel &L = h->g.lv[level];
    for (int y = 0; y < L.h; y++)
        SGX_CHECK_HIP(hipMemcpyAsync(dst + (size_t)y * L.w, h->d_pyr + (size_t)frame * h->g.pyr_pitch + L.off + (size_t)y * L.stride, L.w, hipMemcpyDeviceToHost, 0));
    SGX_CHECK_HIP(hipStreamSynchronize(0));
    return SGX_OK;
}

SGX_TAP int sgx_orb_debug_read_candidates(sgx_orb *h, int frame, int level, int32_t *x, int32_t *y, int32_t *score, int cap, int *n)
{
    if (!h || !n || level < 0 || level >= h->g.nlevels || frame < 0 || frame >= h->cfg.max_batch) return SGX_ERR_INVALID;
    int cnt = 0;
    SGX_CHECK_HIP(hipMemcpyAsync(&cnt, h->d_cand_count + frame * h->g.nlevels + level, 4, hipMemcpyDeviceToHost, 0));
    SGX_CHECK_HIP(hipStreamSynchronize(0));
    if (cnt > h->g.lv[level].cand_cap) cnt = h->g.lv[level].cand_cap;
    std::vector<uint32_t> buf(cnt > 0 ? cnt : 1);
    SGX_CHECK_HIP(hipMemcpyAsync(buf.data(), h->d_cand + (size_t)frame * h->g.cand_pitch + h->g.lv[level].cand_off, (size_t)cnt * 4, hipMemcpyDeviceToHost, 0));
    SGX_CHECK_HIP(hipStreamSynchronize(0));
    for (int i = 0; i < cnt && i < cap; i++) { x[i] = buf[i] & 0xFFF; y[i] = (buf[i] >> 12) & 0xFFF; score[i] = buf[i] >> 24; }
    *n = cnt;
    return SGX_OK;
}

SGX_TAP int sgx_orb_debug_run_octree(sgx_orb *h, int level, const uint32_t *packed, int n, uint32_t *out_sel, int cap, int *nsel)
{
    if (!h || !packed || !out_sel || !nsel || level < 0 || level >= h->g.nlevels || n < 0 || n > h->g.lv[level].cand_cap) return SGX_ERR_INVALID;
    const int nl = h->g.nlevels;
    std::vector<int> cnt(nl, 0); cnt[level] = n;
    SGX_CHECK_HIP(hipMemcpyAsync(h->d_cand_count, cnt.data(), nl * 4, hipMemcpyHostToDevice, 0));
    SGX_CHECK_HIP(hipMemcpyAsync(h->d_cand + h->g.lv[level].cand_off, packed, (size_t)n * 4, hipMemcpyHostToDevice, 0));
    launch_octree(h, 1, (sgx_stream_t)0);
    int ns = 0;
    SGX_CHECK_HIP(hipMemcpyAsync(&ns, h->d_sel_count + level, 4, hipMemcpyDeviceToHost, 0));
    SGX_CHECK_HIP(hipStreamSynchronize(0));
    if (ns > cap) return SGX_ERR_OVERFLOW;
    SGX_CHECK_HIP(hipMemcpyAsync(out_sel, h->d_sel + (size_t)level * SGX_OCT_MAXN, (size_t)ns * 4, hipMemcpyDeviceToHost, 0));
    SGX_CHECK_HIP(hipStreamSynchronize(0));
// ... 4 lines not shown
```

### sg_slam_amd/csrc/sgx_orb_kernels.h

```cpp
#pragma once
#include "sgx_rt.h"
#include "sgx_block.h"
#include "sgx_lane.h"

#define SGX_MAX_LEVELS 12
#define SGX_EDGE 19
#define SGX_BORDER 16
#define SGX_TILE_MAX 68
#define SGX_TILE_STRIDE 72
#define SGX_CAND_LDS 8192
#define SGX_OCT_MAXN 1280
#define SGX_OCT_THREADS 512

struct SgxLevel {
    int w, h, stride;
    int off;
    int quota;
    int ncols, nrows, wcell, hcell;
    int cell0;
    int patch_size;
    int cand_off, cand_cap;
    int boff, bstride;
    float scale;
};
// ... 954 lines not shown
        else { frame = n / kc; slot = n % kc; }
    }
    int level = -1, base = 0, total = 0;
    for (int l = 0; l < g.nlevels; l++) {
        const int n = sel_count[frame * g.nlevels + l];
        if (level < 0 && slot < total + n) { level = l; base = total; }
        total += n;
    }
    if (slot == 0) {
        SGX_THREADS_BEGIN(tid)
        if (tid == 0) { count[frame] = total < cap ? total : cap; if (total > cap) sgx_atomic_or(status, SGX_ST_KP_OVERFLOW); }
        SGX_THREADS_END
    }
    if (level < 0 || slot >= cap) return;
    const SgxLevel L = g.lv[level];
    const uint32_t e = sel[((size_t)frame * g.nlevels + level) * SGX_OCT_MAXN + (slot - base)];
    const int kx = (int)(e & 0xFFF) + SGX_BORDER, ky = (int)((e >> 12) & 0xFFF) + SGX_BORDER;
    int stride;
    const uint8_t *img = sgx_level_ptr(g, gray, gray_pitch, pyr, frame, level, &stride);
    const int px0 = kx - 15, py0 = ky - 15, lead = px0 & 3, xa = px0 - lead;
    SGX_THREADS_BEGIN(tid)
    if (tid == 0) { s_m01 = 0; s_m10 = 0; }
#pragma unroll
    for (int it_ = 0; it_ < (31 * (SGX_MS / 4) + 63) / 64; it_++) { const int i = tid + 64 * it_; if (i >= 31 * (SGX_MS / 4)) break;
        const int r = i / (SGX_MS / 4), q = i - r * (SGX_MS / 4);
        patch_dw[i] = *(const uint32_t *)(img + (size_t)(py0 + r) * stride + xa + 4 * q);
    }
    SGX_THREADS_END
    SGX_SYNC();
    SGX_THREADS_BEGIN(tid)
    int m10 = 0, m01 = 0;
#pragma unroll
    for (int it_ = 0; it_ < (31 * 31 + 63) / 64; it_++) { const int i = tid + 64 * it_; if (i >= 31 * 31) break;
        const int v = i / 31 - 15, u = i - (v + 15) * 31 - 15;
        const int av = v < 0 ? -v : v, au = u < 0 ? -u : u;
        if (au <= (int)((umax_packed >> (4 * av)) & 15ull)) {
            const int I = patch[(15 + v) * SGX_MS + lead + 15 + u];
            m10 += u * I; m01 += v * I;
        }
    }
    sgx_atomic_add(&s_m10, m10); sgx_atomic_add(&s_m01, m01);
    SGX_THREADS_END
    SGX_SYNC();
    SGX_THREADS_BEGIN(tid)
    if (tid == 0) {
        const float angle = sgx_fast_atan2((float)s_m01, (float)s_m10);
        const float factorPI = (float)(3.1415926535897932384626433832795 / 180.f);
        float sn, cs;
        sgx_sincosf(angle * factorPI, &sn, &cs);
        s_a = cs; s_b = sn;
        float *kp = (float *)(kps_raw + ((size_t)frame * cap + slot) * 28);
        float fx = (float)kx, fy = (float)ky;
        if (level != 0) { fx = fx * L.scale; fy = fy * L.scale; }
        kp[0] = fx; kp[1] = fy; kp[2] = (float)L.patch_size; kp[3] = angle; kp[4] = (float)(e >> 24);
        ((int *)kp)[5] = level; ((int *)kp)[6] = -1;
    }
    SGX_THREADS_END
    SGX_SYNC();
    SGX_THREADS_BEGIN(tid)
    const float a = s_a, b = s_b;
    const uint8_t *bl = blur + (size_t)frame * g.blur_pitch + L.boff + (size_t)ky * L.bstride + kx;
#pragma unroll
    for (int it_ = 0; it_ < 4; it_++) { const int t = tid + 64 * it_;
        const uint32_t pw = *(const uint32_t *)(pattern + 4 * t);
        const float x0 = (float)(signed char)(pw & 255u), y0 = (float)(signed char)((pw >> 8) & 255u), x1 = (float)(signed char)((pw >> 16) & 255u), y1 = (float)(signed char)(pw >> 24);
        const int r0 = sgx_cvround(x0 * b + y0 * a), c0 = sgx_cvround(x0 * a - y0 * b);
        const int r1 = sgx_cvround(x1 * b + y1 * a), c1 = sgx_cvround(x1 * a - y1 * b);
        const int t0 = bl[r0 * L.bstride + c0], t1 = bl[r1 * L.bstride + c1];
        bits[t] = (uint8_t)(t0 < t1);
    }
    SGX_THREADS_END
    SGX_SYNC();
    SGX_THREADS_BEGIN(tid)
    if (tid < 32) {
        int v = 0;
#pragma unroll
        for (int j = 0; j < 8; j++) v |= bits[8 * tid + j] << j;
        desc[((size_t)frame * cap + slot) * 32 + tid] = (uint8_t)v;
    }
    SGX_THREADS_END
}
#endif

SGX_KERNEL(64) k_orient_desc4(SgxOrbGeom g, const uint8_t *gray, int gray_pitch, const uint8_t *pyr, const uint8_t *blur,
                              const uint32_t *sel, const int *sel_count, unsigned long long umax_packed, const signed char *pattern,
                              uint8_t *kps_raw, uint8_t *desc, int *count, int cap, int batch, uint32_t *status)
{
    SGX_LDS uint32_t patch_dw[4][31 * SGX_MS / 4];
    SGX_LDS uint8_t bits[4][256];
    SGX_LDS int s_m01[4], s_m10[4];
    SGX_LDS float s_a[4], s_b[4];
    int slot4, frame;
    {
        const int n = (int)blockIdx.x, kc = (g.kp_cap + 3) >> 2;
        if ((batch & 7) == 0) { const int xcd = n & 7, j = n >> 3; frame = xcd + 8 * (j / kc); slot4 = j % kc; }
        else { frame = n / kc; slot4 = n % kc; }
    }
    int total = 0;
    for (int l = 0; l < g.nlevels; l++) total += sel_count[frame * g.nlevels + l];
    if (slot4 == 0) {
        SGX_THREADS_BEGIN(tid)
        if (tid == 0) { count[frame] = total < cap ? total : cap; if (total > cap) sgx_atomic_or(status, SGX_ST_KP_OVERFLOW); }
        SGX_THREADS_END
    }
    if (4 * slot4 >= total || 4 * slot4 >= cap) return;

    SGX_THREADS_BEGIN(tid)
    if (tid < 4) { s_m01[tid] = 0; s_m10[tid] = 0; }
    const int grp = tid >> 4, l16 = tid & 15, slot = 4 * slot4 + grp;
    int level = -1, base = 0, acc_ = 0;
    for (int l = 0; l < g.nlevels; l++) {
        const int n = sel_count[frame * g.nlevels + l];
        if (level < 0 && slot < acc_ + n) { level = l; base = acc_; }
        acc_ += n;
    }
    if (level >= 0 && slot < cap) {
        const uint32_t e = sel[((size_t)frame * g.nlevels + level) * SGX_OCT_MAXN + (slot - base)];
        const int kx = (int)(e & 0xFFF) + SGX_BORDER, ky = (int)((e >> 12) & 0xFFF) + SGX_BORDER;
        int stride;
        const uint8_t *img = sgx_level_ptr(g, gray, gray_pitch, pyr, frame, level, &stride);
        const int px0 = kx - 15, py0 = ky - 15, lead = px0 & 3, xa = px0 - lead;
        for (int i = l16; i < 31 * (SGX_MS / 4); i += 16) {
            const int r = i / (SGX_MS / 4), q = i - r * (SGX_MS / 4);
            patch_dw[grp][i] = *(const uint32_t *)(img + (size_t)(py0 + r) * stride + xa + 4 * q);
        }
    }
    SGX_THREADS_END
    SGX_SYNC();
    SGX_THREADS_BEGIN(tid)
    const int grp = tid >> 4, l16 = tid & 15, slot = 4 * slot4 + grp;
    int level = -1, base = 0, acc_ = 0;
    for (int l = 0; l < g.nlevels; l++) {
        const int n = sel_count[frame * g.nlevels + l];
        if (level < 0 && slot < acc_ + n) { level = l; base = acc_; }
        acc_ += n;
    }
    if (level >= 0 && slot < cap) {
        const uint32_t e = sel[((size_t)frame * g.nlevels + level) * SGX_OCT_MAXN + (slot - base)];
        const int lead = ((int)(e & 0xFFF) + SGX_BORDER - 15) & 3;
        int m10 = 0, m01 = 0;
        for (int i = l16; i < 31 * (SGX_MS / 4); i += 16) {
            const int r = i / (SGX_MS / 4), q = i - r * (SGX_MS / 4);
            const int v = r - 15, av = v < 0 ? -v : v, um = (int)((umax_packed >> (4 * av)) & 15ull);
            const uint32_t w = patch_dw[grp][i];
            int rowsum = 0;
#pragma unroll
            for (int j = 0; j < 4; j++) {
                const int u = 4 * q + j - lead - 15, au = u < 0 ? -u : u;
                const int I = au <= um ? (int)((w >> (8 * j)) & 255u) : 0;
                m10 += u * I; rowsum += I;
            }
            m01 += v * rowsum;
        }
        sgx_atomic_add(&s_m10[grp], m10); sgx_atomic_add(&s_m01[grp], m01);
    }
    SGX_THREADS_END
    SGX_SYNC();
    SGX_THREADS_BEGIN(tid)
    const int grp = tid >> 4, l16 = tid & 15, slot = 4 * slot4 + grp;
    int level = -1, base = 0, acc_ = 0;
    for (int l = 0; l < g.nlevels; l++) {
        const int n = sel_count[frame * g.nlevels + l];
        if (level < 0 && slot < acc_ + n) { level = l; base = acc_; }
        acc_ += n;
    }
    if (level >= 0 && slot < cap && l16 == 0) {
        const SgxLevel L = g.lv[level];
        const uint32_t e = sel[((size_t)frame * g.nlevels + level) * SGX_OCT_MAXN + (slot - base)];
        const int kx = (int)(e & 0xFFF) + SGX_BORDER, ky = (int)((e >> 12) & 0xFFF) + SGX_BORDER;
        const float angle = sgx_fast_atan2((float)s_m01[grp], (float)s_m10[grp]);
        const float factorPI = (float)(3.1415926535897932384626433832795 / 180.f);
        float sn, cs;
        sgx_sincosf(angle * factorPI, &sn, &cs);
        s_a[grp] = cs; s_b[grp] = sn;
        float *kp = (float *)(kps_raw + ((size_t)frame * cap + slot) * 28);
        float fx = (float)kx, fy = (float)ky;
        if (level != 0) { fx = fx * L.scale; fy = fy * L.scale; }
        kp[0] = fx; kp[1] = fy; kp[2] = (float)L.patch_size; kp[3] = angle; kp[4] = (float)(e >> 24);
        ((int *)kp)[5] = level; ((int *)kp)[6] = -1;
    }
    SGX_THREADS_END
    SGX_SYNC();
    SGX_THREADS_BEGIN(tid)
    const int grp = tid >> 4, l16 = tid & 15, slot = 4 * slot4 + grp;
    int level = -1, base = 0, acc_ = 0;
    for (int l = 0; l < g.nlevels; l++) {
        const int n = sel_count[frame * g.nlevels + l];
        if (level < 0 && slot < acc_ + n) { level = l; base = acc_; }
        acc_ += n;
    }
    if (level >= 0 && slot < cap) {
        const SgxLevel L = g.lv[level];
        const uint32_t e = sel[((size_t)frame * g.nlevels + level) * SGX_OCT_MAXN + (slot - base)];
        const int kx = (int)(e & 0xFFF) + SGX_BORDER, ky = (int)((e >> 12) & 0xFFF) + SGX_BORDER;
        const float a = s_a[grp], b = s_b[grp];
        const uint8_t *bl = blur + (size_t)frame * g.blur_pitch + L.boff + (size_t)ky * L.bstride + kx;
#pragma unroll 4
        for (int it_ = 0; it_ < 16; it_++) { const int t = l16 + 16 * it_;
            const uint32_t pw = *(const uint32_t *)(pattern + 4 * t);
            const float x0 = (float)(signed char)(pw & 255u), y0 = (float)(signed char)((pw >> 8) & 255u), x1 = (float)(signed char)((pw >> 16) & 255u), y1 = (float)(signed char)(pw >> 24);
            const int r0 = sgx_cvround(x0 * b + y0 * a), c0 = sgx_cvround(x0 * a - y0 * b);
            const int r1 = sgx_cvround(x1 * b + y1 * a), c1 = sgx_cvround(x1 * a - y1 * b);
            const int t0 = bl[r0 * L.bstride + c0], t1 = bl[r1 * L.bstride + c1];
            bits[grp][t] = (uint8_t)(t0 < t1);
        }
    }
    SGX_THREADS_END
    SGX_SYNC();
    SGX_THREADS_BEGIN(tid)
    const int grp = tid >> 4, l16 = tid & 15, slot = 4 * slot4 + grp;
    if (slot < total && slot < cap) {
#pragma unroll
        for (int h2 = 0; h2 < 2; h2++) {
            const int byte = 2 * l16 + h2;
            int v = 0;
#pragma unroll
            for (int j = 0; j < 8; j++) v |= bits[grp][8 * byte + j] << j;
            desc[((size_t)frame * cap + slot) * 32 + byte] = (uint8_t)v;
        }
    }
    SGX_THREADS_END
}
```

### sg_slam_amd/csrc/sgx_tracker.cpp

```cpp
#include "sgx_rt.h"
#include "../../include/sgx.h"
#ifdef SGX_DEBUG_TAPS
#include "../../include/sgx_debug.h"
#endif
#include <math.h>
#include <stdio.h>
#include <string.h>
#include <stdlib.h>
#include <vector>

#ifndef SGX_EMU
typedef hipEvent_t sgx_ev;
typedef hipStream_t sgx_st;
static int ev_create(sgx_ev *e) { return hipEventCreateWithFlags(e, hipEventDisableTiming) == hipSuccess ? 0 : 1; }
static void ev_destroy(sgx_ev e) { if (e) (void)hipEventDestroy(e); }
static void ev_record(sgx_ev e, sgx_st s) { (void)hipEventRecord(e, s); }
static void st_wait(sgx_st s, sgx_ev e) { (void)hipStreamWaitEvent(s, e, 0); }
static int st_create(sgx_st *s, int high_priority)
{
    if (high_priority) { int lo = 0, hi = 0; (void)hipDeviceGetStreamPriorityRange(&lo, &hi); return hipStreamCreateWithPriority(s, hipStreamNonBlocking, hi) == hipSuccess ? 0 : 1; }
    return hipStreamCreateWithFlags(s, hipStreamNonBlocking) == hipSuccess ? 0 : 1;
}
static void st_destroy(sgx_st s) { if (s) (void)hipStreamDestroy(s); }
static void st_sync(sgx_st s) { if (s) (void)hipStreamSynchronize(s); }
static void ev_sync(sgx_ev e) { if (e) (void)hipEventSynchronize(e); }
static void *host_alloc(size_t n) { void *p = nullptr; return hipHostMalloc(&p, n, hipHostMallocDefault) == hipSuccess ? p : nullptr; }
static void host_free(void *p) { (void)hipHostFree(p); }
#else
typedef int sgx_ev;
typedef void *sgx_st;
static int ev_create(sgx_ev *e) { *e = 0; return 0; }
static void ev_destroy(sgx_ev) {}
static void ev_record(sgx_ev, sgx_st) {}
static void st_wait(sgx_st, sgx_ev) {}
static int st_create(sgx_st *s, int) { *s = nullptr; return 0; }
static void st_destroy(sgx_st) {}
static void st_sync(sgx_st) {}
static void ev_sync(sgx_ev) {}
static void *host_alloc(size_t n) { return calloc(1, n ? n : 1); }
static void host_free(void *p) { free(p); }
#endif

#define TRK_CHECK(expr) do { const int _rc = (expr); if (_rc != SGX_OK) return _rc; } while (0)
#define TRK_HIP(expr) do { if ((expr) != hipSuccess) return SGX_ERR_DEVICE; } while (0)

SGX_KERNEL(256) k_pack_frame_records(int cap, const int32_t *n, const uint32_t *keys, const uint32_t *desc, const uint32_t *Tcw, uint32_t *rec, int rec_words)
{
    SGX_THREADS_BEGIN(tid)
    const int f = (int)blockIdx.x;
    uint32_t *r = rec + (size_t)f * rec_words;
    const uint32_t *k = keys + (size_t)f * cap * 7, *d = desc + (size_t)f * cap * 8, *T = Tcw + (size_t)f * 16;
    if (tid < 4) r[tid] = tid == 0 ? (uint32_t)n[f] : 0u;
    for (int i = tid; i < cap * 7; i += 256) r[4 + i] = k[i];
    for (int i = tid; i < cap * 8; i += 256) r[4 + cap * 7 + i] = d[i];
    if (tid < 16) r[4 + cap * 15 + tid] = T[tid];
    SGX_THREADS_END
}

struct sgx_tracker {
    sgx_tracker_config cfg;
    int S = 0, cap = 0, nlevels = 0, MB = 0;
    sgx_orb *ex = nullptr; sgx_flow *flow = nullptr; sgx_det *det = nullptr;
    float scale[16], inv_sigma2[16]; float log_scale = 0.f;
    std::vector<void *> dev, pinned;
    sgx_keypoint *keys[3]; uint8_t *desc[3]; int32_t *n[3]; float *uright[3], *zdepth[3], *xw[3]; uint8_t *has[3];
    float *Tcw[3];
    sgx_keypoint *keys_un[3] = { nullptr, nullptr, nullptr }; float dist[8] = {}; int ndist = 0; bool undistort = false;
    int32_t *match, *nmatch, *ninl, *zero_i4; uint8_t *outlier, *zero_u8, *vel_valid;
    float *lm_xw, *lm_normal, *lm_min, *lm_max; uint8_t *lm_desc, *lm_skip; int32_t *lm_obs, *lm_n;
    int32_t *match_local, *nmatch_local, *merged, *cur_mp_obs, *ninl2; uint8_t *in_view, *outlier2; float *xw_all;
    sgx_keypoint *rkeys; uint8_t *rdesc, *keep, *lk_status; int32_t *rn; float *prev_xy; double *F; int32_t *f_ok, *f_stats;
    float *pre_boxes; int32_t *pre_nboxes, *pre_have;
    float *no_boxes; int32_t *no_nboxes, *no_have;
    sgx_det_result *det_res[2]; float *det_boxes[2]; int32_t *det_nb[2], *det_have[2];
    uint8_t *h_bgr[2] = { nullptr, nullptr }; uint16_t *h_depth[2] = { nullptr, nullptr };
    uint8_t *d_bgr[2] = { nullptr, nullptr }, *d_gray[2] = { nullptr, nullptr }; uint16_t *d_depth[2] = { nullptr, nullptr };
    int bgr_pitch = 0;
    sgx_st sE = nullptr, sT = nullptr, sD = nullptr, sU = nullptr;
    sgx_ev ev_extract[3] = {}, ev_track[3] = {}, ev_pack[3] = {}, ev_det[2] = {}, ev_up[2] = {}, ev_in = {};
    sgx_ev ev_consumed[3] = {}, ev_det_read[3] = {}, ev_step = {};
    bool consumed_valid[3] = { false, false, false }, det_read_valid[3] = { false, false, false }, up_pending[2] = { false, false };
    sgx_st last_stream = nullptr;
    bool pack_pending[3] = { false, false, false };
    int frame_idx = 0, cur = 0;
    bool pipelined = false, shared_T = false;

    template <class Tp> int alloc(Tp **p, size_t count)
    {
        void *q = nullptr;
        if (hipMalloc(&q, (count ? count : 1) * sizeof(Tp)) != hipSuccess) return SGX_ERR_NOMEM;
        if (hipMemset(q, 0, (count ? count : 1) * sizeof(Tp)) != hipSuccess) return SGX_ERR_DEVICE;
        dev.push_back(q); *p = (Tp *)q; return SGX_OK;
    }
};

extern "C" void sgx_tracker_destroy(sgx_tracker *t)
{
    if (!t) return;
    st_sync(t->sE); st_sync(t->sT); st_sync(t->sD); st_sync(t->sU);
    (void)hipDeviceSynchronize();
    if (t->ex) sgx_orb_destroy(t->ex);
    if (t->flow) sgx_flow_destroy(t->flow);
    for (void *p : t->dev) (void)hipFree(p);
    for (void *p : t->pinned) host_free(p);
    for (int i = 0; i < 3; i++) { ev_destroy(t->ev_extract[i]); ev_destroy(t->ev_track[i]); ev_destroy(t->ev_pack[i]); ev_destroy(t->ev_consumed[i]); ev_destroy(t->ev_det_read[i]); }
    ev_destroy(t->ev_step);
    for (int i = 0; i < 2; i++) { ev_destroy(t->ev_det[i]); ev_destroy(t->ev_up[i]); }
    ev_destroy(t->ev_in);
    st_destroy(t->sE); if (!t->shared_T) st_destroy(t->sT); st_destroy(t->sD); st_destroy(t->sU);
    delete t;
}

extern "C" int sgx_tracker_create(const sgx_tracker_config *cfg, sgx_det *detector, sgx_tracker **out)
{
    if (!cfg || !out || cfg->streams < 1 || cfg->width < 32 || cfg->height < 32 || cfg->nfeatures < 1 || cfg->max_boxes < 1 || cfg->max_boxes > SGX_DET_MAX) return SGX_ERR_INVALID;
    sgx_tracker *t = new sgx_tracker();
    t->cfg = *cfg; t->S = cfg->streams; t->MB = cfg->max_boxes; t->det = detector;
    sgx_orb_config oc; memset(&oc, 0, sizeof oc);
    oc.nfeatures = cfg->nfeatures; oc.scale_factor = cfg->scale_factor; oc.nlevels = cfg->nlevels; oc.ini_th_fast = cfg->ini_th_fast; oc.min_th_fast = cfg->min_th_fast;
    oc.width = cfg->width; oc.height = cfg->height; oc.max_batch = cfg->streams;
#define FAIL(rc_) do { const int _r = (rc_); sgx_tracker_destroy(t); return _r; } while (0)
    int rc = sgx_orb_create(&oc, &t->ex); if (rc != SGX_OK) FAIL(rc);
    t->cap = sgx_orb_keypoint_capacity(t->ex); t->nlevels = cfg->nlevels;
    if (t->nlevels > 16) FAIL(SGX_ERR_INVALID);
    {
        rc = sgx_orb_get_tables(t->ex, t->scale, nullptr, nullptr, t->inv_sigma2, nullptr); if (rc != SGX_OK) FAIL(rc);
        t->log_scale = logf(t->scale[1]);
    }
    const int S = t->S, cap = t->cap, MB = t->MB;
    for (int i = 0; i < 3; i++) {
        if (t->alloc(&t->keys[i], (size_t)S * cap) || t->alloc(&t->desc[i], (size_t)S * cap * 32) || t->alloc(&t->n[i], S) || t->alloc(&t->uright[i], (size_t)S * cap) ||
            t->alloc(&t->zdepth[i], (size_t)S * cap) || t->alloc(&t->xw[i], (size_t)S * cap * 3) || t->alloc(&t->has[i], (size_t)S * cap) || t->alloc(&t->Tcw[i], (size_t)S * 16)) FAIL(SGX_ERR_NOMEM);
    }
    if (t->alloc(&t->match, (size_t)S * cap) || t->alloc(&t->nmatch, S) || t->alloc(&t->ninl, S) || t->alloc(&t->zero_i4, (size_t)S * cap) || t->alloc(&t->outlier, (size_t)S * cap) ||
        t->alloc(&t->zero_u8, (size_t)S * cap) || t->alloc(&t->vel_valid, S)) FAIL(SGX_ERR_NOMEM);
    if (t->alloc(&t->lm_xw, (size_t)S * 2 * cap * 3) || t->alloc(&t->lm_normal, (size_t)S * 2 * cap * 3) || t->alloc(&t->lm_min, (size_t)S * 2 * cap) || t->alloc(&t->lm_max, (size_t)S * 2 * cap) ||
        t->alloc(&t->lm_desc, (size_t)S * 2 * cap * 32) || t->alloc(&t->lm_skip, (size_t)S * 2 * cap) || t->alloc(&t->lm_obs, (size_t)S * 2 * cap) || t->alloc(&t->lm_n, S) ||
        t->alloc(&t->match_local, (size_t)S * cap) || t->alloc(&t->nmatch_local, S) || t->alloc(&t->merged, (size_t)S * cap) || t->alloc(&t->cur_mp_obs, (size_t)S * cap) ||
        t->alloc(&t->ninl2, S) || t->alloc(&t->in_view, (size_t)S * 2 * cap) || t->alloc(&t->outlier2, (size_t)S * cap) || t->alloc(&t->xw_all, (size_t)S * 3 * cap * 3)) FAIL(SGX_ERR_NOMEM);
    {
        std::vector<uint8_t> ones((size_t)S * 2 * cap, 1); std::vector<int32_t> one((size_t)S * 2 * cap, 1), full(S, 2 * cap);
        if (hipMemcpy(t->lm_skip, ones.data(), ones.size(), hipMemcpyHostToDevice) != hipSuccess || hipMemcpy(t->lm_obs, one.data(), one.size() * 4, hipMemcpyHostToDevice) != hipSuccess ||
            hipMemcpy(t->lm_n, full.data(), full.size() * 4, hipMemcpyHostToDevice) != hipSuccess) FAIL(SGX_ERR_DEVICE);
    }
    if (t->alloc(&t->rkeys, (size_t)S * cap) || t->alloc(&t->rdesc, (size_t)S * cap * 32) || t->alloc(&t->keep, (size_t)S * cap) || t->alloc(&t->lk_status, (size_t)S * cap) ||
        t->alloc(&t->rn, S) || t->alloc(&t->prev_xy, (size_t)S * cap * 2) || t->alloc(&t->F, (size_t)S * 9) || t->alloc(&t->f_ok, S) || t->alloc(&t->f_stats, (size_t)S * 4) ||
        t->alloc(&t->pre_boxes, (size_t)S * MB * 4) || t->alloc(&t->pre_nboxes, S) || t->alloc(&t->pre_have, S) || t->alloc(&t->no_boxes, (size_t)S * MB * 4) ||
        t->alloc(&t->no_nboxes, S) || t->alloc(&t->no_have, S)) FAIL(SGX_ERR_NOMEM);
    for (int i = 0; i < 2; i++)
        if (t->alloc(&t->det_res[i], S) || t->alloc(&t->det_boxes[i], (size_t)S * MB * 4) || t->alloc(&t->det_nb[i], S) || t->alloc(&t->det_have[i], S)) FAIL(SGX_ERR_NOMEM);
    if (cfg->dynamic_mask) {
        sgx_flow_config fc; memset(&fc, 0, sizeof fc);
        fc.width = cfg->width; fc.height = cfg->height; fc.max_batch = S; fc.win_size = 21; fc.max_level = 3; fc.max_count = 30; fc.epsilon = 0.01;
        rc = sgx_flow_create(&fc, &t->flow); if (rc != SGX_OK) FAIL(rc);
    }
    t->pipelined = cfg->pipelined != 0;
    if (t->pipelined) {
        static const int prio = sgx_getenv("SGX_TRK_PRIO") ? atoi(sgx_getenv("SGX_TRK_PRIO")) : 0;
        static const int share = sgx_getenv("SGX_TRK_SHARE") ? atoi(sgx_getenv("SGX_TRK_SHARE")) : 0;
        if (st_create(&t->sE, prio & 1) || st_create(&t->sD, (prio >> 2) & 1)) FAIL(SGX_ERR_DEVICE);
        if (share == 1) { t->sT = t->sD; t->shared_T = true; } else if (share == 2) { t->sT = t->sE; t->shared_T = true; }
        else if (st_create(&t->sT, (prio >> 1) & 1)) FAIL(SGX_ERR_DEVICE);
        for (int i = 0; i < 3; i++) if (ev_create(&t->ev_extract[i]) || ev_create(&t->ev_track[i]) || ev_create(&t->ev_pack[i]) || ev_create(&t->ev_consumed[i]) || ev_create(&t->ev_det_read[i])) FAIL(SGX_ERR_DEVICE);
        for (int i = 0; i < 2; i++) if (ev_create(&t->ev_det[i])) FAIL(SGX_ERR_DEVICE);
        if (ev_create(&t->ev_in)) FAIL(SGX_ERR_DEVICE);
    } else if (ev_create(&t->ev_step)) FAIL(SGX_ERR_DEVICE);
    for (int i = 0; i < 2; i++) if (ev_create(&t->ev_up[i])) FAIL(SGX_ERR_DEVICE);
#undef FAIL
    (void)hipDeviceSynchronize();
    *out = t;
    return SGX_OK;
}

extern "C" int sgx_tracker_keypoint_capacity(const sgx_tracker *t) { return t ? t->cap : 0; }
extern "C" int sgx_tracker_record_bytes(const sgx_tracker *t) { return t ? 16 + t->cap * 28 + t->cap * 32 + 64 : 0; }

extern "C" int sgx_tracker_set_initial_pose(sgx_tracker *t, const float *Tcw)
{
    if (!t || !Tcw) return SGX_ERR_INVALID;
    for (int i = 0; i < 3; i++) TRK_HIP(hipMemcpy(t->Tcw[i], Tcw, (size_t)t->S * 16 * 4, hipMemcpyHostToDevice));
    return SGX_OK;
}

extern "C" int sgx_tracker_set_distortion(sgx_tracker *t, const float *dist, int ndist, sgx_camera *out_cam)
{
    if (!t || !dist || (ndist != 4 && ndist != 5 && ndist != 8) || t->frame_idx > 0) return SGX_ERR_INVALID;
    if (dist[0] != 0.0f) {
        const float K4[4] = { t->cfg.cam.fx, t->cfg.cam.fy, t->cfg.cam.cx, t->cfg.cam.cy };
        sgx_camera cam = t->cfg.cam;
        TRK_CHECK(sgx_frame_image_bounds(t->cfg.width, t->cfg.height, K4, dist, ndist, &cam));
        if (!t->keys_un[0]) {
            for (int i = 0; i < 3; i++) TRK_CHECK(t->alloc(&t->keys_un[i], (size_t)t->S * t->cap));
            TRK_HIP(hipDeviceSynchronize());
        }
        t->cfg.cam = cam;
        memcpy(t->dist, dist, (size_t)ndist * sizeof(float)); t->ndist = ndist; t->undistort = true;
    }
    if (out_cam) *out_cam = t->cfg.cam;
    return SGX_OK;
}

extern "C" int sgx_tracker_step_dev(sgx_tracker *t, const uint8_t *d_gray, int gray_pitch, const uint16_t *d_depth, const uint8_t *d_bgr, int bgr_pitch, void *caller_stream)
{
    if (!t || !d_gray || !d_depth || gray_pitch < t->cfg.width) return SGX_ERR_INVALID;
    const int S = t->S, cap = t->cap, MB = t->MB, i = t->frame_idx, c = i % 3, l = (i + 2) % 3;
    const sgx_tracker_config &cf = t->cfg;
    float *Tc = t->Tcw[0], *Tl = t->Tcw[1], *Tll = t->Tcw[2];
    sgx_st sE = t->pipelined ? t->sE : (sgx_st)caller_stream, sT = t->pipelined ? t->sT : (sgx_st)caller_stream, sD = t->pipelined ? t->sD : (sgx_st)caller_stream;
    if (t->pipelined) {
        ev_record(t->ev_in, (sgx_st)caller_stream);
        st_wait(sE, t->ev_in); st_wait(sD, t->ev_in);
        if (i == 0) st_wait(sT, t->ev_in);
        if (t->consumed_valid[c]) st_wait((sgx_st)caller_stream, t->ev_consumed[c]);
        if (t->det_read_valid[c]) { st_wait((sgx_st)caller_stream, t->ev_det_read[c]); t->det_read_valid[c] = false; }
        if (i >= 2) st_wait(sE, t->ev_track[(i - 2) % 3]);
        if (t->pack_pending[c]) { st_wait(sE, t->ev_pack[c]); t->pack_pending[c] = false; }
    }
    const bool with_det = t->det != nullptr && d_bgr != nullptr;
    const int b = i & 1;
    if (with_det) {
        if (t->pipelined && i >= 2) st_wait(sD, t->ev_extract[(i - 2) % 3]);
        TRK_CHECK(sgx_det_detect_batch_dev(t->det, d_bgr, bgr_pitch, S, t->det_res[b], t->det_boxes[b], t->det_nb[b], MB, t->det_have[b], sD));
        if (t->pipelined) { ev_record(t->ev_det[b], sD); ev_record(t->ev_det_read[c], sD); t->det_read_valid[c] = true; }
    }
    const float *boxes = with_det ? t->det_boxes[b] : t->no_boxes; const int32_t *nboxes = with_det ? t->det_nb[b] : t->no_nboxes, *have = with_det ? t->det_have[b] : t->no_have;
    if (cf.dynamic_mask) {
        if (i == 0) {
            TRK_CHECK(sgx_orb_extract_batch_dev(t->ex, d_gray, gray_pitch, S, t->keys[c], t->desc[c], t->n[c], cap, sE));
            TRK_CHECK(sgx_flow_lk_batch_dev(t->flow, d_gray, gray_pitch, S, nullptr, nullptr, cap, nullptr, nullptr, nullptr, sE));
        } else {
            TRK_CHECK(sgx_orb_extract_batch_dev(t->ex, d_gray, gray_pitch, S, t->rkeys, t->rdesc, t->rn, cap, sE));
            TRK_CHECK(sgx_flow_lk_batch_dev(t->flow, d_gray, gray_pitch, S, t->rkeys, t->rn, cap, t->prev_xy, t->lk_status, nullptr, sE));
            TRK_CHECK(sgx_fundamental_ransac_batch_dev(S, cap, t->rkeys, t->rn, t->prev_xy, t->pre_have, t->pre_boxes, t->pre_nboxes, MB, 1.0, 0.99, t->F, t->f_ok, t->f_stats, sE));
            if (with_det && t->pipelined) st_wait(sE, t->ev_det[b]);
            TRK_CHECK(sgx_dynamic_mask_batch_dev(S, cap, t->rkeys, t->rn, t->prev_xy, t->F, boxes, nboxes, MB, t->keep, sE));
            TRK_CHECK(sgx_frame_compact_keys_batch_dev(S, cap, t->rkeys, t->rdesc, t->rn, t->keep, have, cf.nfeatures, t->keys[c], t->desc[c], t->n[c], sE));
            TRK_HIP(hipMemcpyAsync(t->pre_boxes, boxes, (size_t)S * MB * 16, hipMemcpyDeviceToDevice, sE));
            TRK_HIP(hipMemcpyAsync(t->pre_nboxes, nboxes, (size_t)S * 4, hipMemcpyDeviceToDevice, sE));
            TRK_HIP(hipMemcpyAsync(t->pre_have, have, (size_t)S * 4, hipMemcpyDeviceToDevice, sE));
        }
    } else
        TRK_CHECK(sgx_orb_extract_batch_dev(t->ex, d_gray, gray_pitch, S, t->keys[c], t->desc[c], t->n[c], cap, sE));
    if (t->undistort)
        TRK_CHECK(sgx_frame_undistort_stereo_rgbd_batch_dev(S, cap, t->keys[c], t->n[c], t->dist, t->ndist, &cf.cam, d_depth, cf.width, cf.height, cf.depth_map_factor,
                                                            t->keys_un[c], t->uright[c], t->zdepth[c], sE));
    else
        TRK_CHECK(sgx_frame_stereo_from_rgbd_batch_dev(S, cap, t->keys[c], t->n[c], d_depth, cf.width, cf.height, cf.depth_map_factor, cf.cam.bf, t->uright[c], t->zdepth[c], sE));
    const sgx_keypoint *ku_c = t->undistort ? t->keys_un[c] : t->keys[c], *ku_l = t->undistort ? t->keys_un[l] : t->keys[l];
    if (t->pipelined) {
        ev_record(t->ev_extract[c], sE); st_wait(sT, t->ev_extract[c]);
        ev_record(t->ev_consumed[c], sE); t->consumed_valid[c] = true;
    }
    if (i > 0) {
        TRK_CHECK(sgx_frame_motion_model_batch_dev(S, Tl, Tll, t->vel_valid, Tc, sT));
        TRK_CHECK(sgx_match_project_frame_batch_dev(S, cap, ku_c, t->desc[c], t->uright[c], t->n[c], Tc, ku_l, t->n[l], t->has[l], t->zero_u8, t->xw[l], t->zero_i4,
                                                    t->desc[l], Tl, &cf.cam, t->scale, t->nlevels, cf.th_projection, 0, 1, t->match, t->nmatch, sT));
        TRK_CHECK(sgx_pose_optimization_batch_dev(S, cap, ku_c, t->uright[c], t->n[c], t->match, nullptr, t->xw[l], cap, t->inv_sigma2, t->nlevels, &cf.cam, Tc, t->outlier, t->ninl, sT));
        if (i == 1) TRK_HIP(hipMemsetAsync(t->vel_valid, 1, (size_t)S, sT));
    }
    if (i > 0 && cf.local_map) {
        TRK_CHECK(sgx_frame_merge_matches_batch_dev(S, cap, t->n[c], t->match, t->outlier, nullptr, nullptr, nullptr, nullptr, t->cur_mp_obs, nullptr, sT));
        TRK_CHECK(sgx_match_project_local_batch_dev(S, cap, ku_c, t->desc[c], t->uright[c], t->n[c], Tc, t->cur_mp_obs, 2 * cap, t->lm_n, t->lm_xw, t->lm_normal, t->lm_min, t->lm_max,
                                                    t->lm_desc, t->lm_obs, t->lm_skip, &cf.cam, t->scale, t->nlevels, t->log_scale, 3.0f, 0.8f, 0.5f, t->match_local, t->nmatch_local, t->in_view, sT));
        TRK_CHECK(sgx_frame_merge_matches_batch_dev(S, cap, t->n[c], t->match, t->outlier, t->match_local, t->xw[l], t->lm_xw, t->merged, nullptr, t->xw_all, sT));
        TRK_CHECK(sgx_pose_optimization_batch_dev(S, cap, ku_c, t->uright[c], t->n[c], t->merged, nullptr, t->xw_all, 3 * cap, t->inv_sigma2, t->nlevels, &cf.cam, Tc, t->outlier2, t->ninl2, sT));
    }
    TRK_CHECK(sgx_frame_unproject_batch_dev(S, cap, ku_c, t->n[c], t->zdepth[c], Tc, &cf.cam, t->xw[c], t->has[c], sT));
    if (i > 0 && cf.local_map)
        TRK_CHECK(sgx_frame_make_map_points_batch_dev(S, cap, (i - 1) % 2, ku_l, t->n[l], t->xw[l], t->has[l], t->desc[l], Tl, t->scale, t->nlevels, t->lm_xw, t->lm_normal, t->lm_min,
                                                      t->lm_max, t->lm_desc, t->lm_skip, sT));
    if (t->pipelined) ev_record(t->ev_track[c], sT);
    else { t->last_stream = (sgx_st)caller_stream; ev_record(t->ev_step, t->last_stream); }
    t->Tcw[0] = Tll; t->Tcw[1] = Tc; t->Tcw[2] = Tl;
    t->cur = c; t->frame_idx = i + 1;
    return SGX_OK;
}

extern "C" int sgx_tracker_host_buffers(sgx_tracker *t, int slot, uint8_t **bgr, int *bgr_pitch, uint16_t **depth)
{
    if (!t || slot < 0 || slot > 1) return SGX_ERR_INVALID;
    const int S = t->S, W = t->cfg.width, H = t->cfg.height;
    if (!t->h_bgr[0]) {
        t->bgr_pitch = (3 * W + 3) & ~3;
        for (int i = 0; i < 2; i++) {
            t->h_bgr[i] = (uint8_t *)host_alloc((size_t)S * H * t->bgr_pitch); t->h_depth[i] = (uint16_t *)host_alloc((size_t)S * H * W * 2);
            if (!t->h_bgr[i] || !t->h_depth[i]) return SGX_ERR_NOMEM;
            t->pinned.push_back(t->h_bgr[i]); t->pinned.push_back(t->h_depth[i]);
            if (t->alloc(&t->d_bgr[i], (size_t)S * H * t->bgr_pitch) || t->alloc(&t->d_gray[i], (size_t)S * H * W) || t->alloc(&t->d_depth[i], (size_t)S * H * W)) return SGX_ERR_NOMEM;
        }
        if (t->pipelined && st_create(&t->sU, 0)) return SGX_ERR_DEVICE;
        (void)hipDeviceSynchronize();
    }
    if (t->up_pending[slot]) { ev_sync(t->ev_up[slot]); t->up_pending[slot] = false; }
    if (bgr) *bgr = t->h_bgr[slot]; if (bgr_pitch) *bgr_pitch = t->bgr_pitch; if (depth) *depth = t->h_depth[slot];
    return SGX_OK;
}

extern "C" int sgx_tracker_step_host(sgx_tracker *t, int slot, int rgb_order)
{
    if (!t || slot < 0 || slot > 1 || !t->h_bgr[0]) return SGX_ERR_INVALID;
    const int S = t->S, W = t->cfg.width, H = t->cfg.height;
    sgx_st sU = t->pipelined ? t->sU : (sgx_st) nullptr;
    if (t->pipelined && t->frame_idx >= 2) { const int p = (t->frame_idx - 2) % 3; st_wait(sU, t->ev_consumed[p]); if (t->det_read_valid[p]) st_wait(sU, t->ev_det_read[p]); }
    TRK_HIP(hipMemcpyAsync(t->d_bgr[slot], t->h_bgr[slot], (size_t)S * H * t->bgr_pitch, hipMemcpyHostToDevice, sU));
    TRK_HIP(hipMemcpyAsync(t->d_depth[slot], t->h_depth[slot], (size_t)S * H * W * 2, hipMemcpyHostToDevice, sU));
    ev_record(t->ev_up[slot], sU); t->up_pending[slot] = true;
    TRK_CHECK(sgx_frame_gray_from_color_batch_dev(S, W, H, t->d_bgr[slot], t->bgr_pitch, 3, rgb_order ? 0 : 1, t->d_gray[slot], W, sU));
    return sgx_tracker_step_dev(t, t->d_gray[slot], W, t->d_depth[slot], t->det ? t->d_bgr[slot] : nullptr, t->bgr_pitch, sU);
}

extern "C" int sgx_tracker_wait_inputs(sgx_tracker *t, int steps_back)
{
    if (!t || steps_back < 0 || steps_back > 2) return SGX_ERR_INVALID;
    if (t->frame_idx - 1 - steps_back < 0) return SGX_OK;
    if (!t->pipelined) { TRK_HIP(hipDeviceSynchronize()); return SGX_OK; }
    const int c = (t->frame_idx - 1 - steps_back) % 3;
    if (t->consumed_valid[c]) ev_sync(t->ev_consumed[c]);
    if (t->det_read_valid[c]) ev_sync(t->ev_det_read[c]);
    return SGX_OK;
}

extern "C" int sgx_tracker_sync(sgx_tracker *t)
{
    if (!t) return SGX_ERR_INVALID;
    if (t->pipelined) { st_sync(t->sE); st_sync(t->sT); st_sync(t->sD); if (t->sU) st_sync(t->sU); }
    else TRK_HIP(hipDeviceSynchronize());
    t->up_pending[0] = t->up_pending[1] = false;
    return SGX_OK;
}

extern "C" int sgx_tracker_read(sgx_tracker *t, float *Tcw, int32_t *nkeys, int32_t *nmatches, int32_t *ninliers, int32_t *nmatches_local, int32_t *ninliers2, int32_t *nkeys_raw,
                                int32_t *f_ok, int32_t *f_stats)
{
    if (!t) return SGX_ERR_INVALID;
    TRK_CHECK(sgx_tracker_sync(t));
    const size_t S = (size_t)t->S;
    if (Tcw) TRK_HIP(hipMemcpy(Tcw, t->Tcw[1], S * 64, hipMemcpyDeviceToHost));
    if (nkeys) TRK_HIP(hipMemcpy(nkeys, t->n[t->cur], S * 4, hipMemcpyDeviceToHost));
    if (nmatches) TRK_HIP(hipMemcpy(nmatches, t->nmatch, S * 4, hipMemcpyDeviceToHost));
    if (ninliers) TRK_HIP(hipMemcpy(ninliers, t->ninl, S * 4, hipMemcpyDeviceToHost));
    if (nmatches_local) TRK_HIP(hipMemcpy(nmatches_local, t->nmatch_local, S * 4, hipMemcpyDeviceToHost));
    if (ninliers2) TRK_HIP(hipMemcpy(ninliers2, t->ninl2, S * 4, hipMemcpyDeviceToHost));
    if (nkeys_raw) TRK_HIP(hipMemcpy(nkeys_raw, t->rn, S * 4, hipMemcpyDeviceToHost));
    if (f_ok) TRK_HIP(hipMemcpy(f_ok, t->f_ok, S * 4, hipMemcpyDeviceToHost));
    if (f_stats) TRK_HIP(hipMemcpy(f_stats, t->f_stats, S * 16, hipMemcpyDeviceToHost));
    return SGX_OK;
}

extern "C" int sgx_tracker_snapshot_pose_dev(sgx_tracker *t, float *d_out)
{
    if (!t || !d_out) return SGX_ERR_INVALID;
    TRK_HIP(hipMemcpyAsync(d_out, t->Tcw[1], (size_t)t->S * 64, hipMemcpyDeviceToDevice, t->pipelined ? t->sT : t->last_stream));
    return SGX_OK;
}

extern "C" int sgx_tracker_snapshot_boxes_dev(sgx_tracker *t, int stream_index, float *d_boxes, int32_t *d_nboxes)
{
    if (!t || !d_boxes || !d_nboxes || stream_index < 0 || stream_index >= t->S || t->frame_idx < 1) return SGX_ERR_INVALID;
    const int b = (t->frame_idx - 1) & 1;
    sgx_st sD = t->pipelined ? t->sD : t->last_stream;
    TRK_HIP(hipMemcpyAsync(d_boxes, t->det_boxes[b] + (size_t)stream_index * t->MB * 4, (size_t)t->MB * 16, hipMemcpyDeviceToDevice, sD));
    TRK_HIP(hipMemcpyAsync(d_nboxes, t->det_nb[b] + stream_index, 4, hipMemcpyDeviceToDevice, sD));
    return SGX_OK;
}

extern "C" int sgx_tracker_pack_records_dev(sgx_tracker *t, uint8_t *d_records, void *stream)
{
    if (!t || !d_records || t->frame_idx < 1 || ((uintptr_t)d_records & 3)) return SGX_ERR_INVALID;
    const int c = t->cur, words = sgx_tracker_record_bytes(t) / 4;
    sgx_st st = (sgx_st)stream;
    if (t->pipelined) st_wait(st, t->ev_track[c]);
    else if (st != t->last_stream) st_wait(st, t->ev_step);
    SGX_LAUNCH(k_pack_frame_records, dim3(t->S), dim3(256), st, t->cap, t->n[c], (const uint32_t *)t->keys[c], (const uint32_t *)t->desc[c], (const uint32_t *)t->Tcw[1], (uint32_t *)d_records, words);
    TRK_HIP(hipGetLastError());
    if (t->pipelined) { ev_record(t->ev_pack[c], st); t->pack_pending[c] = true; }
    return SGX_OK;
}

extern "C" int sgx_tracker_frame_dev(sgx_tracker *t, const int32_t **d_n, const sgx_keypoint **d_keys, const uint8_t **d_desc, const float **d_Tcw, const float **d_xw, const uint8_t **d_has)
{
    if (!t || t->frame_idx < 1) return SGX_ERR_INVALID;
    const int c = t->cur;
    if (d_n) *d_n = t->n[c]; if (d_keys) *d_keys = t->keys[c]; if (d_desc) *d_desc = t->desc[c]; if (d_Tcw) *d_Tcw = t->Tcw[1]; if (d_xw) *d_xw = t->xw[c]; if (d_has) *d_has = t->has[c];
    return SGX_OK;
}

extern "C" int sgx_tracker_frame_keys_un_dev(sgx_tracker *t, const sgx_keypoint **d_keys_un)
{
    if (!t || !d_keys_un || t->frame_idx < 1) return SGX_ERR_INVALID;
    *d_keys_un = t->undistort ? t->keys_un[t->cur] : t->keys[t->cur];
    return SGX_OK;
}

extern "C" sgx_orb *sgx_tracker_extractor(sgx_tracker *t) { return t ? t->ex : nullptr; }
```

### sg_slam_amd/frame.py

```python
import ctypes as C
from .capi import _vp
from .matcher import camera_struct


def stereo_from_rgbd_batch(lib, batch, cap, d_keys, d_n, d_depth_u16, width, height, depth_map_factor, bf, d_uright, d_zdepth, stream=None):
    lib.check(lib.dll.sgx_frame_stereo_from_rgbd_batch_dev(batch, cap, _vp(d_keys), _vp(d_n), _vp(d_depth_u16), width, height,
                                                           float(depth_map_factor), float(bf), _vp(d_uright), _vp(d_zdepth), _vp(stream)),
              'sgx_frame_stereo_from_rgbd_batch_dev')


def unproject_batch(lib, batch, cap, d_keys, d_n, d_zdepth, d_Tcw, cam, d_xw, d_has, stream=None):
    cs = camera_struct(cam)
    lib.check(lib.dll.sgx_frame_unproject_batch_dev(batch, cap, _vp(d_keys), _vp(d_n), _vp(d_zdepth), _vp(d_Tcw), C.byref(cs), _vp(d_xw),
                                                    _vp(d_has), _vp(stream)), 'sgx_frame_unproject_batch_dev')


def make_map_points_batch(lib, batch, cap, half, d_keys, d_n, d_xw, d_has, d_desc, d_Tcw, scale_factors, d_m_xw, d_m_normal, d_m_min, d_m_max,
                          d_m_desc, d_m_skip, stream=None):
    import numpy as np
    sf = np.ascontiguousarray(scale_factors, 'f4')
    lib.check(lib.dll.sgx_frame_make_map_points_batch_dev(batch, cap, int(half), _vp(d_keys), _vp(d_n), _vp(d_xw), _vp(d_has), _vp(d_desc), _vp(d_Tcw),
                                                          _vp(sf), len(sf), _vp(d_m_xw), _vp(d_m_normal), _vp(d_m_min), _vp(d_m_max), _vp(d_m_desc),
                                                          _vp(d_m_skip), _vp(stream)), 'sgx_frame_make_map_points_batch_dev')


def merge_matches_batch(lib, batch, cap, d_n, d_match_last, d_outlier_last, d_match_local=None, d_xw_last=None, d_m_xw=None, d_merged=None,
                        d_cur_mp_obs=None, d_xw_all=None, stream=None):
    lib.check(lib.dll.sgx_frame_merge_matches_batch_dev(batch, cap, _vp(d_n), _vp(d_match_last), _vp(d_outlier_last), _vp(d_match_local), _vp(d_xw_last),
                                                        _vp(d_m_xw), _vp(d_merged), _vp(d_cur_mp_obs), _vp(d_xw_all), _vp(stream)),
              'sgx_frame_merge_matches_batch_dev')


def compact_keys_batch(lib, batch, cap, d_keys, d_desc, d_n, d_keep, d_have_dynamic, nfeatures, d_keys_out, d_desc_out, d_n_out, stream=None):
    lib.check(lib.dll.sgx_frame_compact_keys_batch_dev(batch, cap, _vp(d_keys), _vp(d_desc), _vp(d_n), _vp(d_keep), _vp(d_have_dynamic), int(nfeatures),
                                                       _vp(d_keys_out), _vp(d_desc_out), _vp(d_n_out), _vp(stream)), 'sgx_frame_compact_keys_batch_dev')


def gray_from_color_batch(lib, batch, width, height, d_src, src_pitch, channels, blue_first, d_gray, gray_pitch, stream=None):
    lib.check(lib.dll.sgx_frame_gray_from_color_batch_dev(batch, width, height, _vp(d_src), src_pitch, channels, 1 if blue_first else 0, _vp(d_gray), gray_pitch, _vp(stream)),
              'sgx_frame_gray_from_color_batch_dev')


def _dist_array(dist):
    import numpy as np
    return np.ascontiguousarray(dist, 'f4').reshape(-1)


def undistort_points(lib, pts, cam, dist):
    import numpy as np
    p = np.ascontiguousarray(pts, 'f4').reshape(-1, 2)
    out = np.zeros_like(p)
    K4 = np.array([cam['fx'], cam['fy'], cam['cx'], cam['cy']], 'f4'); d = _dist_array(dist)
    lib.check(lib.dll.sgx_undistort_points(len(p), _vp(p), _vp(K4), _vp(d), len(d), _vp(out)), 'sgx_undistort_points')
    return out


def undistort_stereo_rgbd_batch_dev(lib, batch, cap, d_keys, d_n, dist, cam, d_depth_u16, width, height, d_keys_un, d_uright, d_zdepth, stream=None):
    cs = camera_struct(cam, width, height); d = _dist_array(dist)
    lib.check(lib.dll.sgx_frame_undistort_stereo_rgbd_batch_dev(batch, cap, _vp(d_keys), _vp(d_n), _vp(d), len(d), C.byref(cs), _vp(d_depth_u16), width, height,
                                                                float(cam['depth_factor']), _vp(d_keys_un), _vp(d_uright), _vp(d_zdepth), _vp(stream)),
              'sgx_frame_undistort_stereo_rgbd_batch_dev')


def image_bounds(lib, width, height, cam, dist):
    import numpy as np
    K4 = np.array([cam['fx'], cam['fy'], cam['cx'], cam['cy']], 'f4'); d = _dist_array(dist)
    cs = camera_struct(cam, width, height)
    lib.check(lib.dll.sgx_frame_image_bounds(int(width), int(height), _vp(K4), _vp(d), len(d), C.byref(cs)), 'sgx_frame_image_bounds')
    return dict(min_x=cs.min_x, max_x=cs.max_x, min_y=cs.min_y, max_y=cs.max_y)
```

### sg_slam_amd/orb.py

```python
import ctypes as C
import numpy as np
from .capi import OrbConfig, KP_DTYPE, _vp
from ._lib import load


class ORBextractor:
    def __init__(self, nfeatures=1000, scaleFactor=1.2, nlevels=8, iniThFAST=20, minThFAST=7,
                 width=640, height=480, max_batch=1, lib=None):
        self.lib = lib if lib is not None else load()
        self.cfg = OrbConfig(nfeatures, scaleFactor, nlevels, iniThFAST, minThFAST, width, height, max_batch)
        h = C.c_void_p()
        self.lib.check(self.lib.dll.sgx_orb_create(C.byref(self.cfg), C.byref(h)), 'sgx_orb_create')
        self.h = h
        self.nlevels, self.nfeatures, self.width, self.height, self.max_batch = nlevels, nfeatures, width, height, max_batch
        self.capacity = self.lib.dll.sgx_orb_keypoint_capacity(self.h)
        t = [np.zeros(nlevels, 'f4') for _ in range(4)] + [np.zeros(nlevels, 'i4')]
        self.lib.check(self.lib.dll.sgx_orb_get_tables(self.h, *[_vp(a) for a in t]), 'sgx_orb_get_tables')
        self.mvScaleFactor, self.mvInvScaleFactor, self.mvLevelSigma2, self.mvInvLevelSigma2, self.mnFeaturesPerLevel = t

    def close(self):
        if getattr(self, 'h', None):
            self.lib.dll.sgx_orb_destroy(self.h)
            self.h = None

    def __del__(self):
        try:
            self.close()
        except Exception:
            pass

    def GetLevels(self): return self.nlevels
    def GetScaleFactor(self): return float(self.cfg.scale_factor)
    def GetScaleFactors(self): return self.mvScaleFactor
    def GetInverseScaleFactors(self): return self.mvInvScaleFactor
    def GetScaleSigmaSquares(self): return self.mvLevelSigma2
    def GetInverseScaleSigmaSquares(self): return self.mvInvLevelSigma2
    def GetnFeatures(self): return self.nfeatures

    def __call__(self, image, mask=None):
        img = np.ascontiguousarray(image, np.uint8)
        if img.size == 0:
            return np.zeros(0, KP_DTYPE), np.zeros((0, 32), np.uint8)
        assert img.shape == (self.height, self.width)
        kps = np.zeros(self.capacity, KP_DTYPE)
        desc = np.zeros((self.capacity, 32), np.uint8)
        n = C.c_int(0)
        self.lib.check(self.lib.dll.sgx_orb_extract(self.h, _vp(img), self.width, _vp(kps), _vp(desc), self.capacity, C.byref(n)),
                       'sgx_orb_extract')
        return kps[:n.value].copy(), desc[:n.value].copy()

    def extract_batch_dev(self, d_gray, pitch, batch, d_kps, d_desc, d_count, stream=None):
        self.lib.check(self.lib.dll.sgx_orb_extract_batch_dev(self.h, _vp(d_gray), pitch, batch, _vp(d_kps), _vp(d_desc),
                                                              _vp(d_count), self.capacity, _vp(stream)), 'sgx_orb_extract_batch_dev')

    def last_status(self, stream=None):
        self.lib.check(self.lib.dll.sgx_orb_last_status(self.h, _vp(stream)), 'sgx_orb_last_status')

    def debug_level(self, frame, level):
        w, h, s = C.c_int32(), C.c_int32(), C.c_int32()
        self.lib.check(self.lib.tap('sgx_orb_debug_level_geometry')(self.h, level, C.byref(w), C.byref(h), C.byref(s)))
        out = np.zeros((h.value, w.value), np.uint8)
        self.lib.check(self.lib.tap('sgx_orb_debug_read_level')(self.h, frame, level, _vp(out)), 'debug_read_level')
        return out

    def debug_candidates(self, frame, level, cap=8192):
        x = np.zeros(cap, 'i4'); y = np.zeros(cap, 'i4'); s = np.zeros(cap, 'i4'); n = C.c_int(0)
        self.lib.check(self.lib.tap('sgx_orb_debug_read_candidates')(self.h, frame, level, _vp(x), _vp(y), _vp(s), cap, C.byref(n)))
        return x[:n.value].copy(), y[:n.value].copy(), s[:n.value].copy()

    def debug_run_octree(self, level, x, y, score):
        packed = (np.asarray(x, np.uint32) | (np.asarray(y, np.uint32) << 12) | (np.asarray(score, np.uint32) << 24)).astype(np.uint32)
        packed = np.ascontiguousarray(packed)
        out = np.zeros(2048, np.uint32); n = C.c_int(0)
        self.lib.check(self.lib.tap('sgx_orb_debug_run_octree')(self.h, level, _vp(packed), len(packed), _vp(out), 2048, C.byref(n)), 'debug_run_octree')
        o = out[:n.value]
        return (o & 0xFFF).astype('i4'), ((o >> 12) & 0xFFF).astype('i4'), (o >> 24).astype('i4')
```

### sg_slam_amd/tracker_native.py

```python
import ctypes as C
import numpy as np
from .capi import TrackerConfig, _vp
from .matcher import camera_struct


class TrackerNative:
    def __init__(self, lib, streams, cam, width=640, height=480, nfeatures=1000, th=15.0, pipelined=True, local_map=True, dynamic_mask=True, max_boxes=8, detector=None, dist=None):
        self.lib, self.S, self.W, self.H = lib, int(streams), int(width), int(height)
        cfg = TrackerConfig()
        cfg.streams, cfg.width, cfg.height = self.S, width, height
        cfg.nfeatures, cfg.scale_factor, cfg.nlevels, cfg.ini_th_fast, cfg.min_th_fast = nfeatures, 1.2, 8, 20, 7
        cfg.cam = camera_struct(cam, width, height); cfg.depth_map_factor = float(cam['depth_factor']); cfg.th_projection = float(th)
        cfg.local_map, cfg.dynamic_mask, cfg.max_boxes, cfg.pipelined = int(local_map), int(dynamic_mask), int(max_boxes), int(pipelined)
        self.detector = detector
        h = C.c_void_p()
        lib.check(lib.dll.sgx_tracker_create(C.byref(cfg), None if detector is None else detector.h, C.byref(h)), 'sgx_tracker_create')
        self.h = h
        self.cap = lib.dll.sgx_tracker_keypoint_capacity(h)
        self.rec_bytes = lib.dll.sgx_tracker_record_bytes(h)
        self.max_boxes = int(max_boxes)
        self.frame_idx = 0
        out = camera_struct(cam, width, height)
        if dist is not None:
            d = np.ascontiguousarray(dist, 'f4').reshape(-1)
            lib.check(lib.dll.sgx_tracker_set_distortion(h, _vp(d), len(d), C.byref(out)), 'sgx_tracker_set_distortion')
        self.bounds = dict(min_x=out.min_x, max_x=out.max_x, min_y=out.min_y, max_y=out.max_y)

    def close(self):
        if getattr(self, 'h', None):
            self.lib.dll.sgx_tracker_destroy(self.h); self.h = None

    def __del__(self):
        try: self.close()
        except Exception: pass

    def set_initial_pose(self, Tcw_host):
        T = np.ascontiguousarray(Tcw_host, 'f4').reshape(self.S, 16)
        self.lib.check(self.lib.dll.sgx_tracker_set_initial_pose(self.h, _vp(T)))

    def step(self, d_gray, d_depth, d_bgr=None, gray_pitch=None, bgr_pitch=None, stream=None):
        self.lib.check(self.lib.dll.sgx_tracker_step_dev(self.h, _vp(d_gray), gray_pitch or self.W, _vp(d_depth), _vp(d_bgr), bgr_pitch or 3 * self.W,
                                                         None if stream is None else C.c_void_p(stream)), 'sgx_tracker_step_dev')
        self.frame_idx += 1

    def host_buffers(self, slot):
        b, d, p = C.c_void_p(), C.c_void_p(), C.c_int()
        self.lib.check(self.lib.dll.sgx_tracker_host_buffers(self.h, slot, C.byref(b), C.byref(p), C.byref(d)), 'sgx_tracker_host_buffers')
        bgr = np.ctypeslib.as_array(C.cast(b, C.POINTER(C.c_uint8)), shape=(self.S, self.H, p.value))
        dep = np.ctypeslib.as_array(C.cast(d, C.POINTER(C.c_uint16)), shape=(self.S, self.H, self.W))
        return bgr, dep

    def step_host(self, slot, rgb_order=True):
        self.lib.check(self.lib.dll.sgx_tracker_step_host(self.h, slot, int(rgb_order)), 'sgx_tracker_step_host')
        self.frame_idx += 1

    def synchronize(self):
        self.lib.check(self.lib.dll.sgx_tracker_sync(self.h))

    def wait_inputs(self, steps_back=0):
        self.lib.check(self.lib.dll.sgx_tracker_wait_inputs(self.h, steps_back), 'sgx_tracker_wait_inputs')

    def read(self):
        S = self.S
        out = dict(Tcw=np.zeros((S, 16), 'f4'), nkeys=np.zeros(S, 'i4'), nmatch=np.zeros(S, 'i4'), ninl=np.zeros(S, 'i4'), nmatch_local=np.zeros(S, 'i4'), ninl2=np.zeros(S, 'i4'),
                   nkeys_raw=np.zeros(S, 'i4'), f_ok=np.zeros(S, 'i4'), f_stats=np.zeros((S, 4), 'i4'))
        self.lib.check(self.lib.dll.sgx_tracker_read(self.h, *[_vp(out[k]) for k in ('Tcw', 'nkeys', 'nmatch', 'ninl', 'nmatch_local', 'ninl2', 'nkeys_raw', 'f_ok', 'f_stats')]))
        return out

    def last_pose(self):
        return self.read()['Tcw'].reshape(self.S, 4, 4)

    def snapshot_pose(self, d_out):
        self.lib.check(self.lib.dll.sgx_tracker_snapshot_pose_dev(self.h, _vp(d_out)))

    def snapshot_boxes(self, stream_index, d_boxes, d_nboxes):
        self.lib.check(self.lib.dll.sgx_tracker_snapshot_boxes_dev(self.h, stream_index, _vp(d_boxes), _vp(d_nboxes)))

    def pack_records(self, d_records, stream=None):
        self.lib.check(self.lib.dll.sgx_tracker_pack_records_dev(self.h, _vp(d_records), None if stream is None else C.c_void_p(stream)))

    def frame_dev(self):
        p = [C.c_void_p() for _ in range(6)]
        self.lib.check(self.lib.dll.sgx_tracker_frame_dev(self.h, *[C.byref(x) for x in p]))
        return dict(zip(('n', 'keys', 'desc', 'Tcw', 'xw', 'has'), [x.value for x in p]))

    def frame_keys_un_dev(self):
        p = C.c_void_p()
        self.lib.check(self.lib.dll.sgx_tracker_frame_keys_un_dev(self.h, C.byref(p)))
        return p.value

    def last_status(self, stream=None):
        self.lib.check(self.lib.dll.sgx_orb_last_status(self.lib.dll.sgx_tracker_extractor(self.h), None if stream is None else C.c_void_p(stream)))


class TrackerGroups:

    def __init__(self, lib, streams, cam, groups, make_detector=None, **kw):
        assert streams % groups == 0, 'streams must divide into equal groups'
        self.lib, self.S, self.G, self.Sg = lib, int(streams), int(groups), int(streams) // int(groups)
        self.detectors = [make_detector(self.Sg) if make_detector else None for _ in range(self.G)]
        self.tr = [TrackerNative(lib, self.Sg, cam, detector=d, **kw) for d in self.detectors]
        self.cap, self.rec_bytes, self.max_boxes = self.tr[0].cap, self.tr[0].rec_bytes, self.tr[0].max_boxes
        self.W, self.H = self.tr[0].W, self.tr[0].H

    def _sl(self, g, a):
        if a is None: return None
        assert hasattr(a, 'shape') and len(a.shape) >= 1 and a.shape[0] == self.S, 'TrackerGroups takes tensors / arrays of shape (streams, ...), not raw pointers'
        contiguous = a.is_contiguous() if hasattr(a, 'is_contiguous') else a.flags['C_CONTIGUOUS']
        assert contiguous, 'TrackerGroups inputs must be contiguous'
        return a[g * self.Sg:(g + 1) * self.Sg]

    def set_initial_pose(self, Tcw_host):
        T = np.ascontiguousarray(Tcw_host, 'f4').reshape(self.S, 16)
        for g, t in enumerate(self.tr): t.set_initial_pose(T[g * self.Sg:(g + 1) * self.Sg])

    def step(self, d_gray, d_depth, d_bgr=None, stream=None, **kw):
        for g, t in enumerate(self.tr): t.step(self._sl(g, d_gray), self._sl(g, d_depth), d_bgr=self._sl(g, d_bgr), stream=stream, **kw)

    def synchronize(self):
        for t in self.tr: t.synchronize()

    def read(self):
        parts = [t.read() for t in self.tr]
        return {k: np.concatenate([p[k] for p in parts]) for k in parts[0]}

    def snapshot_pose(self, d_out):
        for g, t in enumerate(self.tr): t.snapshot_pose(self._sl(g, d_out))

    def snapshot_boxes(self, stream_index, d_boxes, d_nboxes):
        self.tr[stream_index // self.Sg].snapshot_boxes(stream_index % self.Sg, d_boxes, d_nboxes)

    def pack_records(self, d_records, stream=None):
        for g, t in enumerate(self.tr): t.pack_records(self._sl(g, d_records), stream=stream)

    def last_status(self, stream=None):
        for t in self.tr: t.last_status(stream=stream)

    def close(self):
        for t in self.tr: t.close()
```

Baseline: 30100.

## Defer ORB orientation and descriptors until after dynamic-keypoint masking

The tracker now runs only FAST detection and octree selection before optical flow, fundamental RANSAC and dynamic masking. Compaction then records each kept keypoint's source index, and blur plus orientation/descriptor computation runs only on the kept keypoints. This avoids computing and copying descriptors for keypoints that masking discards. The cost is an extra src index buffer, an extra launch boundary, and the blur now sitting later in the dependency chain. The old early-describe path stays available behind an environment/debug switch.

```diff
diff --git a/include/sgx.h b/include/sgx.h
--- a/include/sgx.h
+++ b/include/sgx.h
@@ -46,6 +46,9 @@
                        int32_t *features_per_level);
 int sgx_orb_extract_batch_dev(sgx_orb *h, const uint8_t *d_gray, int pitch, int batch,
                               sgx_keypoint *d_kps, uint8_t *d_desc, int32_t *d_count, int cap, void *stream);
+int sgx_orb_detect_batch_dev(sgx_orb *h, const uint8_t *d_gray, int pitch, int batch, sgx_keypoint *d_kps, int32_t *d_count, int cap, void *stream);
+int sgx_orb_describe_batch_dev(sgx_orb *h, const uint8_t *d_gray, int pitch, int batch, const int32_t *d_src, const int32_t *d_n_kept,
+                               sgx_keypoint *d_kps, uint8_t *d_desc, int cap, void *stream);
 int sgx_orb_extract(sgx_orb *h, const uint8_t *gray, int stride, sgx_keypoint *kps, uint8_t *desc, int cap, int *n);
 int sgx_orb_last_status(sgx_orb *h, void *stream);
 
@@ -296,6 +299,8 @@
                                const float *d_boxes, const int32_t *d_nboxes, int max_boxes, uint8_t *d_keep, void *stream);
 int sgx_frame_compact_keys_batch_dev(int batch, int cap, const sgx_keypoint *d_keys, const uint8_t *d_desc, const int32_t *d_n, const uint8_t *d_keep,
                                      const int32_t *d_have_dynamic, int nfeatures, sgx_keypoint *d_keys_out, uint8_t *d_desc_out, int32_t *d_n_out, void *stream);
+int sgx_frame_compact_keys_src_batch_dev(int batch, int cap, const sgx_keypoint *d_keys, const int32_t *d_n, const uint8_t *d_keep, const int32_t *d_have_dynamic,
+                                         int nfeatures, sgx_keypoint *d_keys_out, int32_t *d_src_out, int32_t *d_n_out, void *stream);
 
 
 typedef struct sgx_flow_config {
diff --git a/include/sgx_debug.h b/include/sgx_debug.h
--- a/include/sgx_debug.h
+++ b/include/sgx_debug.h
@@ -33,6 +33,8 @@
 int sgx_det_debug_time_ops(sgx_det *h, const uint8_t *d_img, int pitch, int batch, int reps, float *ms, int cap, int *nops);
 int sgx_det_debug_run_step(sgx_det *h, const uint8_t *d_img, int pitch, int batch, int step, int reps, void *stream);
 int sgx_orb_debug_run_octree(sgx_orb *h, int level, const uint32_t *packed, int n, uint32_t *out_sel, int cap, int *nsel);
+int sgx_tracker_debug_set_describe_early(int on);
+int sgx_tracker_debug_set_boxes(sgx_tracker *t, const float *boxes, const int32_t *nboxes, const int32_t *have_dynamic);
 
 #ifdef __cplusplus
 }
diff --git a/sg_slam_amd/capi.py b/sg_slam_amd/capi.py
--- a/sg_slam_amd/capi.py
+++ b/sg_slam_amd/capi.py
@@ -108,7 +108,7 @@
     'sgx_pnp_solver_get_estimate', 'sgx_pnp_solver_destroy', 'sgx_pnp_batch_create', 'sgx_pnp_batch_set_dev', 'sgx_pnp_batch_iterate_dev', 'sgx_pnp_batch_destroy',
     'sgx_obj3d_create', 'sgx_obj3d_destroy', 'sgx_obj3d_detect_batch_dev', 'sgx_obj3d_detect', 'sgx_objdb_create', 'sgx_objdb_destroy', 'sgx_objdb_add', 'sgx_objdb_size',
     'sgx_objdb_get', 'sgx_initializer_create', 'sgx_initializer_initialize', 'sgx_initializer_destroy', 'sgx_init_batch_create', 'sgx_init_batch_run_dev',
-    'sgx_init_batch_destroy',
+    'sgx_init_batch_destroy', 'sgx_orb_detect_batch_dev', 'sgx_orb_describe_batch_dev', 'sgx_frame_compact_keys_src_batch_dev',
 ]
 TAP_SYMBOLS = [
     'sgx_orb_debug_level_geometry', 'sgx_orb_debug_set_unfused_pyramid', 'sgx_orb_debug_read_level', 'sgx_orb_debug_read_candidates',
@@ -116,6 +116,7 @@
     'sgx_det_debug_detection_output', 'sgx_det_debug_continued', 'sgx_debug_flow_affine_batch_dev', 'sgx_det_debug_set_fusion', 'sgx_det_debug_set_legacy_kernels',
     'sgx_det_debug_set_block_fusion', 'sgx_det_debug_set_irb', 'sgx_det_debug_set_gemm', 'sgx_det_debug_time_ops', 'sgx_det_debug_run_step', 'sgx_flow_debug_read_level',
     'sgx_flow_debug_level_size', 'sgx_flow_debug_read_slot', 'sgx_debug_corun_bf16', 'sgx_pnp_debug_betas', 'sgx_obj3d_debug_read',
+    'sgx_tracker_debug_set_describe_early', 'sgx_tracker_debug_set_boxes',
 ]
 
 
@@ -144,6 +145,8 @@
         d.sgx_orb_get_tables.argtypes = [C.c_void_p] + [C.c_void_p] * 5
         d.sgx_orb_extract_batch_dev.argtypes = [C.c_void_p, C.c_void_p, C.c_int, C.c_int, C.c_void_p, C.c_void_p,
                                                 C.c_void_p, C.c_int, C.c_void_p]
+        d.sgx_orb_detect_batch_dev.argtypes = [C.c_void_p, C.c_void_p, C.c_int, C.c_int, C.c_void_p, C.c_void_p, C.c_int, C.c_void_p]
+        d.sgx_orb_describe_batch_dev.argtypes = [C.c_void_p, C.c_void_p, C.c_int, C.c_int, C.c_void_p, C.c_void_p, C.c_void_p, C.c_void_p, C.c_int, C.c_void_p]
         d.sgx_orb_extract.argtypes = [C.c_void_p, C.c_void_p, C.c_int, C.c_void_p, C.c_void_p, C.c_int, C.POINTER(C.c_int)]
         d.sgx_orb_last_status.argtypes = [C.c_void_p, C.c_void_p]
 
@@ -194,6 +197,7 @@
         d.sgx_dynamic_mask_batch_dev.argtypes = [C.c_int, C.c_int, vp, vp, vp, vp, vp, vp, C.c_int, vp, vp]
         d.sgx_frame_gray_from_color_batch_dev.argtypes = [C.c_int, C.c_int, C.c_int, vp, C.c_int, C.c_int, C.c_int, vp, C.c_int, vp]
         d.sgx_frame_compact_keys_batch_dev.argtypes = [C.c_int, C.c_int, vp, vp, vp, vp, vp, C.c_int, vp, vp, vp, vp]
+        d.sgx_frame_compact_keys_src_batch_dev.argtypes = [C.c_int, C.c_int, vp, vp, vp, vp, C.c_int, vp, vp, vp, vp]
         d.sgx_match_project_local.argtypes = [C.c_int] + [vp] * 5 + [C.c_int] + [vp] * 7 + [C.POINTER(Camera), vp, C.c_int, C.c_float, C.c_float, C.c_float, C.c_float, vp, vp, vp]
         d.sgx_match_project_local_batch_dev.argtypes = [C.c_int, C.c_int] + [vp] * 6 + [C.c_int] + [vp] * 8 + [C.POINTER(Camera), vp, C.c_int, C.c_float, C.c_float, C.c_float, C.c_float, vp, vp, vp, vp]
         d.sgx_undistort_points.argtypes = [C.c_int, vp, vp, vp, C.c_int, vp]
@@ -291,6 +295,8 @@
             d.sgx_obj3d_debug_read.argtypes = [vp, C.c_int, vp, vp, C.c_int, C.POINTER(C.c_int)]
             d.sgx_flow_debug_level_size.argtypes = [vp, C.c_int, C.POINTER(C.c_int32), C.POINTER(C.c_int32)]
             d.sgx_flow_debug_read_slot.argtypes = [vp, C.c_int, C.c_int, C.c_int, vp, C.POINTER(C.c_int32)]
+            d.sgx_tracker_debug_set_describe_early.argtypes = [C.c_int]
+            d.sgx_tracker_debug_set_boxes.argtypes = [vp, vp, vp, vp]
 
     def tap(self, name):
         if not self.has_taps:
diff --git a/sg_slam_amd/csrc/sgx_det.cpp b/sg_slam_amd/csrc/sgx_det.cpp
--- a/sg_slam_amd/csrc/sgx_det.cpp
+++ b/sg_slam_amd/csrc/sgx_det.cpp
@@ -1312,8 +1312,20 @@
     if (batch < 1 || cap < 1 || !d_keys || !d_desc || !d_n || !d_keep || !d_keys_out || !d_desc_out || !d_n_out || (const void *)d_keys == (const void *)d_keys_out) return SGX_ERR_INVALID;
     sgx_prof_begin(SGX_K_MASK, (sgx_stream_t)stream);
     SGX_LAUNCH(k_compact_keys, dim3(batch), dim3(256), (sgx_stream_t)stream, cap, (const uint8_t *)d_keys, d_desc, d_n, d_keep, d_have_dynamic, (float)nfeatures * 0.1f,
-               (uint8_t *)d_keys_out, d_desc_out, d_n_out);
+               (uint8_t *)d_keys_out, d_desc_out, d_n_out, (int *)nullptr);
     sgx_prof_end(SGX_K_MASK, (sgx_stream_t)stream);
     SGX_CHECK_HIP(hipGetLastError());
     return SGX_OK;
 }
+
+extern "C" int sgx_frame_compact_keys_src_batch_dev(int batch, int cap, const sgx_keypoint *d_keys, const int32_t *d_n, const uint8_t *d_keep, const int32_t *d_have_dynamic,
+                                                    int nfeatures, sgx_keypoint *d_keys_out, int32_t *d_src_out, int32_t *d_n_out, void *stream)
+{
+    if (batch < 1 || cap < 1 || !d_keys || !d_n || !d_keep || !d_keys_out || !d_src_out || !d_n_out || (const void *)d_keys == (const void *)d_keys_out) return SGX_ERR_INVALID;
+    sgx_prof_begin(SGX_K_MASK, (sgx_stream_t)stream);
+    SGX_LAUNCH(k_compact_keys, dim3(batch), dim3(256), (sgx_stream_t)stream, cap, (const uint8_t *)d_keys, (const uint8_t *)nullptr, d_n, d_keep, d_have_dynamic, (float)nfeatures * 0.1f,
+               (uint8_t *)d_keys_out, (uint8_t *)nullptr, d_n_out, d_src_out);
+    sgx_prof_end(SGX_K_MASK, (sgx_stream_t)stream);
+    SGX_CHECK_HIP(hipGetLastError());
+    return SGX_OK;
+}
diff --git a/sg_slam_amd/csrc/sgx_det_kernels.h b/sg_slam_amd/csrc/sgx_det_kernels.h
--- a/sg_slam_amd/csrc/sgx_det_kernels.h
+++ b/sg_slam_amd/csrc/sgx_det_kernels.h
@@ -906,7 +906,7 @@
 }
 
 SGX_KERNEL(256) k_compact_keys(int cap, const uint8_t *keys, const uint8_t *desc, const int *n, const uint8_t *keep, const int *have_dynamic, float restore_below,
-                               uint8_t *keys_out, uint8_t *desc_out, int *n_out)
+                               uint8_t *keys_out, uint8_t *desc_out, int *n_out, int *src_out)
 {
     SGX_LDS int scan[256];
     SGX_LDS int s_total;
@@ -926,12 +926,17 @@
     int pos = restore ? tid * CH : scan[tid];
     for (int i = tid * CH; i < min(N, (tid + 1) * CH); i++) {
         if (!restore && !keep[(size_t)f * cap + i]) continue;
-        const uint32_t *ks = (const uint32_t *)(keys + ((size_t)f * cap + i) * 28), *ds = (const uint32_t *)(desc + ((size_t)f * cap + i) * 32);
-        uint32_t *kd = (uint32_t *)(keys_out + ((size_t)f * cap + pos) * 28), *dd = (uint32_t *)(desc_out + ((size_t)f * cap + pos) * 32);
+        const uint32_t *ks = (const uint32_t *)(keys + ((size_t)f * cap + i) * 28);
+        uint32_t *kd = (uint32_t *)(keys_out + ((size_t)f * cap + pos) * 28);
 #pragma unroll
         for (int w = 0; w < 7; w++) kd[w] = ks[w];
-#pragma unroll
-        for (int w = 0; w < 8; w++) dd[w] = ds[w];
+        if (desc) {
+            const uint32_t *ds = (const uint32_t *)(desc + ((size_t)f * cap + i) * 32);
+            uint32_t *dd = (uint32_t *)(desc_out + ((size_t)f * cap + pos) * 32);
+#pragma unroll
+            for (int w = 0; w < 8; w++) dd[w] = ds[w];
+        }
+        if (src_out) src_out[(size_t)f * cap + pos] = i;
         pos++;
     }
     if (tid == 0) n_out[f] = restore ? N : s_total;
diff --git a/sg_slam_amd/csrc/sgx_orb.cpp b/sg_slam_amd/csrc/sgx_orb.cpp
--- a/sg_slam_amd/csrc/sgx_orb.cpp
+++ b/sg_slam_amd/csrc/sgx_orb.cpp
@@ -37,6 +37,7 @@
     uint32_t *d_status = nullptr;
     uint8_t *d_gray1 = nullptr; uint8_t *d_kps1 = nullptr; uint8_t *d_desc1 = nullptr; int *d_count1 = nullptr;
     int last_batch = 0;
+    int detected_batch = 0;
     int oct_maxlim = 0;
 };
 
@@ -345,12 +346,8 @@
     }
 }
 
-extern "C" int sgx_orb_extract_batch_dev(sgx_orb *h, const uint8_t *d_gray, int pitch, int batch,
-                                         sgx_keypoint *d_kps, uint8_t *d_desc, int32_t *d_count, int cap, void *stream_)
-{
-    if (!h || !d_gray || !d_kps || !d_desc || !d_count) return SGX_ERR_INVALID;
-    if (batch < 1 || batch > h->cfg.max_batch || pitch < h->g.W || (pitch & 3) || ((uintptr_t)d_gray & 3) || cap < h->g.kp_cap) return SGX_ERR_INVALID;
-    sgx_stream_t stream = (sgx_stream_t)stream_;
+static int launch_detect(sgx_orb *h, const uint8_t *d_gray, int pitch, int batch, sgx_stream_t stream, sgx_keypoint *d_kps = nullptr, int32_t *d_count = nullptr, int cap = 0)
+{
     const SgxOrbGeom &g = h->g;
     const int nl = g.nlevels;
     h->last_batch = batch;
@@ -373,10 +370,39 @@
     sgx_prof_end(SGX_K_FAST, stream);
     sgx_prof_begin(SGX_K_OCTREE, stream);
     launch_octree(h, batch, stream);
+    if (d_kps) SGX_LAUNCH(k_octree_keys, dim3((g.kp_cap + 255) / 256, batch), dim3(256), stream, g, h->d_sel, h->d_sel_count, (uint8_t *)d_kps, d_count, cap, h->d_status);
     sgx_prof_end(SGX_K_OCTREE, stream);
+    return SGX_OK;
+}
+
+static unsigned long long umax_packed_of(const sgx_orb *h)
+{
+    unsigned long long v = 0;
+    for (int i = 0; i < 16; i++) v |= (unsigned long long)(h->umax_h[i] & 15) << (4 * i);
+    return v;
+}
+
+static void launch_blur(sgx_orb *h, const uint8_t *d_gray, int pitch, int batch, sgx_stream_t stream)
+{
+    const SgxOrbGeom &g = h->g;
+    static const int blur_threads = sgx_getenv("SGX_TUNE_BLUR_THREADS") ? atoi(sgx_getenv("SGX_TUNE_BLUR_THREADS")) : 256;
+    const int blur_grid = sgx_getenv("SGX_TUNE_ORB_BLUR_GRID") ? atoi(sgx_getenv("SGX_TUNE_ORB_BLUR_GRID")) : 4096;
+    const int parts = std::min(g.nblur_tiles, std::max(1, blur_grid / batch));
+    SGX_LAUNCH(k_blur_levels, dim3(parts * batch), dim3(std::min(512, std::max(256, blur_threads))), stream, g, h->d_blur_tiles, d_gray, pitch, h->d_pyr, h->d_blur, batch);
+}
+
+extern "C" int sgx_orb_extract_batch_dev(sgx_orb *h, const uint8_t *d_gray, int pitch, int batch,
+                                         sgx_keypoint *d_kps, uint8_t *d_desc, int32_t *d_count, int cap, void *stream_)
+{
+    if (!h || !d_gray || !d_kps || !d_desc || !d_count) return SGX_ERR_INVALID;
+    if (batch < 1 || batch > h->cfg.max_batch || pitch < h->g.W || (pitch & 3) || ((uintptr_t)d_gray & 3) || cap < h->g.kp_cap) return SGX_ERR_INVALID;
+    sgx_stream_t stream = (sgx_stream_t)stream_;
+    const SgxOrbGeom &g = h->g;
+    h->detected_batch = 0;
+    { const int rc = launch_detect(h, d_gray, pitch, batch, stream); if (rc != SGX_OK) return rc; }
+    static const int e_extra = sgx_getenv("SGX_TUNE_E_EXTRA_LDS") ? atoi(sgx_getenv("SGX_TUNE_E_EXTRA_LDS")) : 0;
     sgx_prof_begin(SGX_K_ORIENT_DESC, stream);
-    unsigned long long umax_packed = 0;
-    for (int i = 0; i < 16; i++) umax_packed |= (unsigned long long)(h->umax_h[i] & 15) << (4 * i);
+    const unsigned long long umax_packed = umax_packed_of(h);
 #ifdef SGX_DEBUG_TAPS
     static const bool patch_blur = sgx_getenv("SGX_TUNE_ORB_PATCH_BLUR") != nullptr;
     if (patch_blur) {
@@ -385,12 +411,7 @@
     } else
 #endif
     {
-        static const int blur_threads = sgx_getenv("SGX_TUNE_BLUR_THREADS") ? atoi(sgx_getenv("SGX_TUNE_BLUR_THREADS")) : 256;
-        {
-            const int blur_grid = sgx_getenv("SGX_TUNE_ORB_BLUR_GRID") ? atoi(sgx_getenv("SGX_TUNE_ORB_BLUR_GRID")) : 4096;
-            const int parts = std::min(g.nblur_tiles, std::max(1, blur_grid / batch));
-            SGX_LAUNCH(k_blur_levels, dim3(parts * batch), dim3(std::min(512, std::max(256, blur_threads))), stream, g, h->d_blur_tiles, d_gray, pitch, h->d_pyr, h->d_blur, batch);
-        }
+        launch_blur(h, d_gray, pitch, batch, stream);
 #ifdef SGX_DEBUG_TAPS
         static const bool one_per_wave = sgx_getenv("SGX_TUNE_ORB_DESC_ONE_PER_WAVE") != nullptr;
         if (one_per_wave)
@@ -398,9 +419,36 @@
                        umax_packed, h->d_pattern, (uint8_t *)d_kps, d_desc, d_count, cap, batch, h->d_status);
         else
 #endif
-            SGX_LAUNCH(k_orient_desc4, dim3(((g.kp_cap + 3) / 4) * batch), dim3(64), stream, g, d_gray, pitch, h->d_pyr, h->d_blur, h->d_sel, h->d_sel_count,
-                       umax_packed, h->d_pattern, (uint8_t *)d_kps, d_desc, d_count, cap, batch, h->d_status);
-    }
+            SGX_LAUNCH(k_orient_desc4<false>, dim3(((g.kp_cap + 3) / 4) * batch), dim3(64), stream, g, d_gray, pitch, h->d_pyr, h->d_blur, h->d_sel, h->d_sel_count,
+                       umax_packed, h->d_pattern, (uint8_t *)d_kps, d_desc, d_count, cap, batch, h->d_status, (const int *)nullptr, (const int *)nullptr);
+    }
+    sgx_prof_end(SGX_K_ORIENT_DESC, stream);
+    SGX_CHECK_HIP(hipGetLastError());
+    return SGX_OK;
+}
+
+extern "C" int sgx_orb_detect_batch_dev(sgx_orb *h, const uint8_t *d_gray, int pitch, int batch, sgx_keypoint *d_kps, int32_t *d_count, int cap, void *stream_)
+{
+    if (!h || !d_gray || !d_kps || !d_count) return SGX_ERR_INVALID;
+    if (batch < 1 || batch > h->cfg.max_batch || pitch < h->g.W || (pitch & 3) || ((uintptr_t)d_gray & 3) || cap < h->g.kp_cap) return SGX_ERR_INVALID;
+    h->detected_batch = 0;
+    { const int rc = launch_detect(h, d_gray, pitch, batch, (sgx_stream_t)stream_, d_kps, d_count, cap); if (rc != SGX_OK) return rc; }
+    SGX_CHECK_HIP(hipGetLastError());
+    h->detected_batch = batch;
+    return SGX_OK;
+}
+
+extern "C" int sgx_orb_describe_batch_dev(sgx_orb *h, const uint8_t *d_gray, int pitch, int batch, const int32_t *d_src, const int32_t *d_n_kept,
+                                          sgx_keypoint *d_kps, uint8_t *d_desc, int cap, void *stream_)
+{
+    if (!h || !d_gray || !d_src || !d_n_kept || !d_kps || !d_desc) return SGX_ERR_INVALID;
+    if (batch < 1 || batch != h->detected_batch || pitch < h->g.W || (pitch & 3) || ((uintptr_t)d_gray & 3) || cap < h->g.kp_cap) return SGX_ERR_INVALID;
+    sgx_stream_t stream = (sgx_stream_t)stream_;
+    const SgxOrbGeom &g = h->g;
+    sgx_prof_begin(SGX_K_ORIENT_DESC, stream);
+    launch_blur(h, d_gray, pitch, batch, stream);
+    SGX_LAUNCH(k_orient_desc4<true>, dim3(((g.kp_cap + 3) / 4) * batch), dim3(64), stream, g, d_gray, pitch, h->d_pyr, h->d_blur, h->d_sel, h->d_sel_count,
+               umax_packed_of(h), h->d_pattern, (uint8_t *)d_kps, d_desc, (int *)nullptr, cap, batch, h->d_status, d_src, d_n_kept);
     sgx_prof_end(SGX_K_ORIENT_DESC, stream);
     SGX_CHECK_HIP(hipGetLastError());
     return SGX_OK;
diff --git a/sg_slam_amd/csrc/sgx_orb_kernels.h b/sg_slam_amd/csrc/sgx_orb_kernels.h
--- a/sg_slam_amd/csrc/sgx_orb_kernels.h
+++ b/sg_slam_amd/csrc/sgx_orb_kernels.h
@@ -1060,9 +1060,18 @@
 }
 #endif
 
+template <bool KEPT> SGX_DEV int sgx_desc_raw_slot(const int *src, int frame, int cap, int out, int n_kept)
+{
+    if (!KEPT) return out;
+    if (out >= n_kept) return cap;
+    const int s = src[(size_t)frame * cap + out];
+    return (unsigned)s < (unsigned)cap ? s : cap;
+}
+
+template <bool KEPT>
 SGX_KERNEL(64) k_orient_desc4(SgxOrbGeom g, const uint8_t *gray, int gray_pitch, const uint8_t *pyr, const uint8_t *blur,
                               const uint32_t *sel, const int *sel_count, unsigned long long umax_packed, const signed char *pattern,
-                              uint8_t *kps_raw, uint8_t *desc, int *count, int cap, int batch, uint32_t *status)
+                              uint8_t *kps_raw, uint8_t *desc, int *count, int cap, int batch, uint32_t *status, const int *src, const int *n_kept)
 {
     SGX_LDS uint32_t patch_dw[4][31 * SGX_MS / 4];
     SGX_LDS uint8_t bits[4][256];
@@ -1075,8 +1084,9 @@
         else { frame = n / kc; slot4 = n % kc; }
     }
     int total = 0;
-    for (int l = 0; l < g.nlevels; l++) total += sel_count[frame * g.nlevels + l];
-    if (slot4 == 0) {
+    if (KEPT) total = min(n_kept[frame], cap);
+    else for (int l = 0; l < g.nlevels; l++) total += sel_count[frame * g.nlevels + l];
+    if (!KEPT && slot4 == 0) {
         SGX_THREADS_BEGIN(tid)
         if (tid == 0) { count[frame] = total < cap ? total : cap; if (total > cap) sgx_atomic_or(status, SGX_ST_KP_OVERFLOW); }
         SGX_THREADS_END
@@ -1085,7 +1095,7 @@
 
     SGX_THREADS_BEGIN(tid)
     if (tid < 4) { s_m01[tid] = 0; s_m10[tid] = 0; }
-    const int grp = tid >> 4, l16 = tid & 15, slot = 4 * slot4 + grp;
+    const int grp = tid >> 4, l16 = tid & 15, out = 4 * slot4 + grp, slot = sgx_desc_raw_slot<KEPT>(src, frame, cap, out, total);
     int level = -1, base = 0, acc_ = 0;
     for (int l = 0; l < g.nlevels; l++) {
         const int n = sel_count[frame * g.nlevels + l];
@@ -1106,7 +1116,7 @@
     SGX_THREADS_END
     SGX_SYNC();
     SGX_THREADS_BEGIN(tid)
-    const int grp = tid >> 4, l16 = tid & 15, slot = 4 * slot4 + grp;
+    const int grp = tid >> 4, l16 = tid & 15, out = 4 * slot4 + grp, slot = sgx_desc_raw_slot<KEPT>(src, frame, cap, out, total);
     int level = -1, base = 0, acc_ = 0;
     for (int l = 0; l < g.nlevels; l++) {
         const int n = sel_count[frame * g.nlevels + l];
@@ -1135,7 +1145,7 @@
     SGX_THREADS_END
     SGX_SYNC();
     SGX_THREADS_BEGIN(tid)
-    const int grp = tid >> 4, l16 = tid & 15, slot = 4 * slot4 + grp;
+    const int grp = tid >> 4, l16 = tid & 15, out = 4 * slot4 + grp, slot = sgx_desc_raw_slot<KEPT>(src, frame, cap, out, total);
     int level = -1, base = 0, acc_ = 0;
     for (int l = 0; l < g.nlevels; l++) {
         const int n = sel_count[frame * g.nlevels + l];
@@ -1151,16 +1161,19 @@
         float sn, cs;
         sgx_sincosf(angle * factorPI, &sn, &cs);
         s_a[grp] = cs; s_b[grp] = sn;
-        float *kp = (float *)(kps_raw + ((size_t)frame * cap + slot) * 28);
+        float *kp = (float *)(kps_raw + ((size_t)frame * cap + out) * 28);
         float fx = (float)kx, fy = (float)ky;
         if (level != 0) { fx = fx * L.scale; fy = fy * L.scale; }
-        kp[0] = fx; kp[1] = fy; kp[2] = (float)L.patch_size; kp[3] = angle; kp[4] = (float)(e >> 24);
-        ((int *)kp)[5] = level; ((int *)kp)[6] = -1;
-    }
-    SGX_THREADS_END
-    SGX_SYNC();
-    SGX_THREADS_BEGIN(tid)
-    const int grp = tid >> 4, l16 = tid & 15, slot = 4 * slot4 + grp;
+        if (KEPT) kp[3] = angle;
+        else {
+            kp[0] = fx; kp[1] = fy; kp[2] = (float)L.patch_size; kp[3] = angle; kp[4] = (float)(e >> 24);
+            ((int *)kp)[5] = level; ((int *)kp)[6] = -1;
+        }
+    }
+    SGX_THREADS_END
+    SGX_SYNC();
+    SGX_THREADS_BEGIN(tid)
+    const int grp = tid >> 4, l16 = tid & 15, out = 4 * slot4 + grp, slot = sgx_desc_raw_slot<KEPT>(src, frame, cap, out, total);
     int level = -1, base = 0, acc_ = 0;
     for (int l = 0; l < g.nlevels; l++) {
         const int n = sel_count[frame * g.nlevels + l];
@@ -1186,16 +1199,42 @@
     SGX_THREADS_END
     SGX_SYNC();
     SGX_THREADS_BEGIN(tid)
-    const int grp = tid >> 4, l16 = tid & 15, slot = 4 * slot4 + grp;
-    if (slot < total && slot < cap) {
+    const int grp = tid >> 4, l16 = tid & 15, out = 4 * slot4 + grp;
+    if (out < total && out < cap) {
 #pragma unroll
         for (int h2 = 0; h2 < 2; h2++) {
             const int byte = 2 * l16 + h2;
             int v = 0;
 #pragma unroll
             for (int j = 0; j < 8; j++) v |= bits[grp][8 * byte + j] << j;
-            desc[((size_t)frame * cap + slot) * 32 + byte] = (uint8_t)v;
-        }
-    }
-    SGX_THREADS_END
-}
+            desc[((size_t)frame * cap + out) * 32 + byte] = (uint8_t)v;
+        }
+    }
+    SGX_THREADS_END
+}
+
+#define SGX_KP_ANGLE_PENDING (-1.0f)
+SGX_KERNEL(256) k_octree_keys(SgxOrbGeom g, const uint32_t *sel, const int *sel_count, uint8_t *kps_raw, int *count, int cap, uint32_t *status)
+{
+    const int frame = (int)blockIdx.y;
+    SGX_THREADS_BEGIN(tid)
+    const int slot = (int)blockIdx.x * 256 + tid;
+    int level = -1, base = 0, total = 0;
+    for (int l = 0; l < g.nlevels; l++) {
+        const int n = sel_count[frame * g.nlevels + l];
+        if (level < 0 && slot < total + n) { level = l; base = total; }
+        total += n;
+    }
+    if (slot == 0) { count[frame] = total < cap ? total : cap; if (total > cap) sgx_atomic_or(status, SGX_ST_KP_OVERFLOW); }
+    if (level >= 0 && slot < cap) {
+        const SgxLevel L = g.lv[level];
+        const uint32_t e = sel[((size_t)frame * g.nlevels + level) * SGX_OCT_MAXN + (slot - base)];
+        const int kx = (int)(e & 0xFFF) + SGX_BORDER, ky = (int)((e >> 12) & 0xFFF) + SGX_BORDER;
+        float *kp = (float *)(kps_raw + ((size_t)frame * cap + slot) * 28);
+        float fx = (float)kx, fy = (float)ky;
+        if (level != 0) { fx = fx * L.scale; fy = fy * L.scale; }
+        kp[0] = fx; kp[1] = fy; kp[2] = (float)L.patch_size; kp[3] = SGX_KP_ANGLE_PENDING; kp[4] = (float)(e >> 24);
+        ((int *)kp)[5] = level; ((int *)kp)[6] = -1;
+    }
+    SGX_THREADS_END
+}
diff --git a/sg_slam_amd/csrc/sgx_tracker.cpp b/sg_slam_amd/csrc/sgx_tracker.cpp
--- a/sg_slam_amd/csrc/sgx_tracker.cpp
+++ b/sg_slam_amd/csrc/sgx_tracker.cpp
@@ -69,7 +69,9 @@
     int32_t *match, *nmatch, *ninl, *zero_i4; uint8_t *outlier, *zero_u8, *vel_valid;
     float *lm_xw, *lm_normal, *lm_min, *lm_max; uint8_t *lm_desc, *lm_skip; int32_t *lm_obs, *lm_n;
     int32_t *match_local, *nmatch_local, *merged, *cur_mp_obs, *ninl2; uint8_t *in_view, *outlier2; float *xw_all;
-    sgx_keypoint *rkeys; uint8_t *rdesc, *keep, *lk_status; int32_t *rn; float *prev_xy; double *F; int32_t *f_ok, *f_stats;
+    sgx_keypoint *rkeys; uint8_t *keep, *lk_status; int32_t *rn, *src; float *prev_xy; double *F; int32_t *f_ok, *f_stats;
+    uint8_t *rdesc = nullptr;
+    bool describe_early = false;
     float *pre_boxes; int32_t *pre_nboxes, *pre_have;
     float *no_boxes; int32_t *no_nboxes, *no_have;
     sgx_det_result *det_res[2]; float *det_boxes[2]; int32_t *det_nb[2], *det_have[2];
@@ -94,6 +96,9 @@
     }
 };
 
+static thread_local int g_trk_describe_early = -1;
+SGX_TAP int sgx_tracker_debug_set_describe_early(int on) { g_trk_describe_early = on < 0 ? -1 : (on ? 1 : 0); return SGX_OK; }
+
 extern "C" void sgx_tracker_destroy(sgx_tracker *t)
 {
     if (!t) return;
@@ -143,7 +148,12 @@
         if (hipMemcpy(t->lm_skip, ones.data(), ones.size(), hipMemcpyHostToDevice) != hipSuccess || hipMemcpy(t->lm_obs, one.data(), one.size() * 4, hipMemcpyHostToDevice) != hipSuccess ||
             hipMemcpy(t->lm_n, full.data(), full.size() * 4, hipMemcpyHostToDevice) != hipSuccess) FAIL(SGX_ERR_DEVICE);
     }
-    if (t->alloc(&t->rkeys, (size_t)S * cap) || t->alloc(&t->rdesc, (size_t)S * cap * 32) || t->alloc(&t->keep, (size_t)S * cap) || t->alloc(&t->lk_status, (size_t)S * cap) ||
+    {
+        static const bool env_early = sgx_getenv("SGX_TRK_DESCRIBE_EARLY") != nullptr;
+        t->describe_early = g_trk_describe_early < 0 ? env_early : g_trk_describe_early != 0;
+        if (t->describe_early && t->alloc(&t->rdesc, (size_t)S * cap * 32)) FAIL(SGX_ERR_NOMEM);
+    }
+    if (t->alloc(&t->rkeys, (size_t)S * cap) || t->alloc(&t->src, (size_t)S * cap) || t->alloc(&t->keep, (size_t)S * cap) || t->alloc(&t->lk_status, (size_t)S * cap) ||
         t->alloc(&t->rn, S) || t->alloc(&t->prev_xy, (size_t)S * cap * 2) || t->alloc(&t->F, (size_t)S * 9) || t->alloc(&t->f_ok, S) || t->alloc(&t->f_stats, (size_t)S * 4) ||
         t->alloc(&t->pre_boxes, (size_t)S * MB * 4) || t->alloc(&t->pre_nboxes, S) || t->alloc(&t->pre_have, S) || t->alloc(&t->no_boxes, (size_t)S * MB * 4) ||
         t->alloc(&t->no_nboxes, S) || t->alloc(&t->no_have, S)) FAIL(SGX_ERR_NOMEM);
@@ -229,12 +239,17 @@
             TRK_CHECK(sgx_orb_extract_batch_dev(t->ex, d_gray, gray_pitch, S, t->keys[c], t->desc[c], t->n[c], cap, sE));
             TRK_CHECK(sgx_flow_lk_batch_dev(t->flow, d_gray, gray_pitch, S, nullptr, nullptr, cap, nullptr, nullptr, nullptr, sE));
         } else {
-            TRK_CHECK(sgx_orb_extract_batch_dev(t->ex, d_gray, gray_pitch, S, t->rkeys, t->rdesc, t->rn, cap, sE));
+            if (t->describe_early) TRK_CHECK(sgx_orb_extract_batch_dev(t->ex, d_gray, gray_pitch, S, t->rkeys, t->rdesc, t->rn, cap, sE));
+            else TRK_CHECK(sgx_orb_detect_batch_dev(t->ex, d_gray, gray_pitch, S, t->rkeys, t->rn, cap, sE));
             TRK_CHECK(sgx_flow_lk_batch_dev(t->flow, d_gray, gray_pitch, S, t->rkeys, t->rn, cap, t->prev_xy, t->lk_status, nullptr, sE));
             TRK_CHECK(sgx_fundamental_ransac_batch_dev(S, cap, t->rkeys, t->rn, t->prev_xy, t->pre_have, t->pre_boxes, t->pre_nboxes, MB, 1.0, 0.99, t->F, t->f_ok, t->f_stats, sE));
             if (with_det && t->pipelined) st_wait(sE, t->ev_det[b]);
             TRK_CHECK(sgx_dynamic_mask_batch_dev(S, cap, t->rkeys, t->rn, t->prev_xy, t->F, boxes, nboxes, MB, t->keep, sE));
-            TRK_CHECK(sgx_frame_compact_keys_batch_dev(S, cap, t->rkeys, t->rdesc, t->rn, t->keep, have, cf.nfeatures, t->keys[c], t->desc[c], t->n[c], sE));
+            if (t->describe_early) TRK_CHECK(sgx_frame_compact_keys_batch_dev(S, cap, t->rkeys, t->rdesc, t->rn, t->keep, have, cf.nfeatures, t->keys[c], t->desc[c], t->n[c], sE));
+            else {
+                TRK_CHECK(sgx_frame_compact_keys_src_batch_dev(S, cap, t->rkeys, t->rn, t->keep, have, cf.nfeatures, t->keys[c], t->src, t->n[c], sE));
+                TRK_CHECK(sgx_orb_describe_batch_dev(t->ex, d_gray, gray_pitch, S, t->src, t->n[c], t->keys[c], t->desc[c], cap, sE));
+            }
             TRK_HIP(hipMemcpyAsync(t->pre_boxes, boxes, (size_t)S * MB * 16, hipMemcpyDeviceToDevice, sE));
             TRK_HIP(hipMemcpyAsync(t->pre_nboxes, nboxes, (size_t)S * 4, hipMemcpyDeviceToDevice, sE));
             TRK_HIP(hipMemcpyAsync(t->pre_have, have, (size_t)S * 4, hipMemcpyDeviceToDevice, sE));
@@ -392,4 +407,14 @@
     return SGX_OK;
 }
 
+SGX_TAP int sgx_tracker_debug_set_boxes(sgx_tracker *t, const float *boxes, const int32_t *nboxes, const int32_t *have_dynamic)
+{
+    if (!t || !boxes || !nboxes || !have_dynamic) return SGX_ERR_INVALID;
+    TRK_CHECK(sgx_tracker_sync(t));
+    TRK_HIP(hipMemcpy(t->no_boxes, boxes, (size_t)t->S * t->MB * 16, hipMemcpyHostToDevice));
+    TRK_HIP(hipMemcpy(t->no_nboxes, nboxes, (size_t)t->S * 4, hipMemcpyHostToDevice));
+    TRK_HIP(hipMemcpy(t->no_have, have_dynamic, (size_t)t->S * 4, hipMemcpyHostToDevice));
+    return SGX_OK;
+}
+
 extern "C" sgx_orb *sgx_tracker_extractor(sgx_tracker *t) { return t ? t->ex : nullptr; }
diff --git a/sg_slam_amd/frame.py b/sg_slam_amd/frame.py
--- a/sg_slam_amd/frame.py
+++ b/sg_slam_amd/frame.py
@@ -36,6 +36,11 @@
                                                        _vp(d_keys_out), _vp(d_desc_out), _vp(d_n_out), _vp(stream)), 'sgx_frame_compact_keys_batch_dev')
 
 
+def compact_keys_src_batch(lib, batch, cap, d_keys, d_n, d_keep, d_have_dynamic, nfeatures, d_keys_out, d_src_out, d_n_out, stream=None):
+    lib.check(lib.dll.sgx_frame_compact_keys_src_batch_dev(batch, cap, _vp(d_keys), _vp(d_n), _vp(d_keep), _vp(d_have_dynamic), int(nfeatures),
+                                                           _vp(d_keys_out), _vp(d_src_out), _vp(d_n_out), _vp(stream)), 'sgx_frame_compact_keys_src_batch_dev')
+
+
 def gray_from_color_batch(lib, batch, width, height, d_src, src_pitch, channels, blue_first, d_gray, gray_pitch, stream=None):
     lib.check(lib.dll.sgx_frame_gray_from_color_batch_dev(batch, width, height, _vp(d_src), src_pitch, channels, 1 if blue_first else 0, _vp(d_gray), gray_pitch, _vp(stream)),
               'sgx_frame_gray_from_color_batch_dev')
diff --git a/sg_slam_amd/orb.py b/sg_slam_amd/orb.py
--- a/sg_slam_amd/orb.py
+++ b/sg_slam_amd/orb.py
@@ -53,6 +53,14 @@
         self.lib.check(self.lib.dll.sgx_orb_extract_batch_dev(self.h, _vp(d_gray), pitch, batch, _vp(d_kps), _vp(d_desc),
                                                               _vp(d_count), self.capacity, _vp(stream)), 'sgx_orb_extract_batch_dev')
 
+    def detect_batch_dev(self, d_gray, pitch, batch, d_kps, d_count, stream=None):
+        self.lib.check(self.lib.dll.sgx_orb_detect_batch_dev(self.h, _vp(d_gray), pitch, batch, _vp(d_kps), _vp(d_count), self.capacity, _vp(stream)),
+                       'sgx_orb_detect_batch_dev')
+
+    def describe_batch_dev(self, d_gray, pitch, batch, d_src, d_n_kept, d_kps, d_desc, stream=None):
+        self.lib.check(self.lib.dll.sgx_orb_describe_batch_dev(self.h, _vp(d_gray), pitch, batch, _vp(d_src), _vp(d_n_kept), _vp(d_kps), _vp(d_desc),
+                                                               self.capacity, _vp(stream)), 'sgx_orb_describe_batch_dev')
+
     def last_status(self, stream=None):
         self.lib.check(self.lib.dll.sgx_orb_last_status(self.h, _vp(stream)), 'sgx_orb_last_status')
 
diff --git a/sg_slam_amd/tracker_native.py b/sg_slam_amd/tracker_native.py
--- a/sg_slam_amd/tracker_native.py
+++ b/sg_slam_amd/tracker_native.py
@@ -5,7 +5,8 @@
 
 
 class TrackerNative:
-    def __init__(self, lib, streams, cam, width=640, height=480, nfeatures=1000, th=15.0, pipelined=True, local_map=True, dynamic_mask=True, max_boxes=8, detector=None, dist=None):
+    def __init__(self, lib, streams, cam, width=640, height=480, nfeatures=1000, th=15.0, pipelined=True, local_map=True, dynamic_mask=True, max_boxes=8, detector=None, dist=None,
+                 describe_early=None):
         self.lib, self.S, self.W, self.H = lib, int(streams), int(width), int(height)
         cfg = TrackerConfig()
         cfg.streams, cfg.width, cfg.height = self.S, width, height
@@ -14,7 +15,12 @@
         cfg.local_map, cfg.dynamic_mask, cfg.max_boxes, cfg.pipelined = int(local_map), int(dynamic_mask), int(max_boxes), int(pipelined)
         self.detector = detector
         h = C.c_void_p()
-        lib.check(lib.dll.sgx_tracker_create(C.byref(cfg), None if detector is None else detector.h, C.byref(h)), 'sgx_tracker_create')
+        if describe_early is not None:
+            lib.check(lib.tap('sgx_tracker_debug_set_describe_early')(int(bool(describe_early))))
+        try:
+            lib.check(lib.dll.sgx_tracker_create(C.byref(cfg), None if detector is None else detector.h, C.byref(h)), 'sgx_tracker_create')
+        finally:
+            if describe_early is not None: lib.tap('sgx_tracker_debug_set_describe_early')(-1)
         self.h = h
         self.cap = lib.dll.sgx_tracker_keypoint_capacity(h)
         self.rec_bytes = lib.dll.sgx_tracker_record_bytes(h)
@@ -89,6 +95,11 @@
         self.lib.check(self.lib.dll.sgx_tracker_frame_keys_un_dev(self.h, C.byref(p)))
         return p.value
 
+    def debug_set_boxes(self, boxes, nboxes, have_dynamic):
+        b = np.ascontiguousarray(boxes, 'f4').reshape(self.S, self.max_boxes, 4); nb = np.ascontiguousarray(nboxes, 'i4').reshape(self.S)
+        hv = np.ascontiguousarray(have_dynamic, 'i4').reshape(self.S)
+        self.lib.check(self.lib.tap('sgx_tracker_debug_set_boxes')(self.h, _vp(b), _vp(nb), _vp(hv)), 'sgx_tracker_debug_set_boxes')
+
     def last_status(self, stream=None):
         self.lib.check(self.lib.dll.sgx_orb_last_status(self.lib.dll.sgx_tracker_extractor(self.h), None if stream is None else C.c_void_p(stream)))
 
```

Result: faster. 30520, median of 6 (+1.4%).
